# ndming/GS-2M

Measured on AMD Instinct MI355X. Metric: train views/s (fwd+bwd raster) at 1M Gaussians 1080p, higher is better.
Workload: dtype f32; 1 GPU; BASELINE configs[2] (c3): 1000000 synthetic Gaussians (SH deg 3), 1 camera 1920x1080 per GPU, feature_count=9, fwd+bwd at the op boundary; gaussians=1000000, visible=844909, num_rendered=2709460, width=1920, height=1080, feature_count=9, parallelism=view-parallel x1, views_per_rank=1

## Files before the change

gs-2m_amd/csrc/api.hip:

```cpp
#include "common.h"
#include <atomic>
#include <mutex>
#include <chrono>
#include <dlfcn.h>

#define HIP_TRY(expr)                          \
    do {                                       \
        hipError_t e_ = (expr);                \
        if (e_ != hipSuccess) return GS2M_ERR_HIP; \
    } while (0)

namespace {

uint32_t higher_msb(uint32_t n) {
    uint32_t msb = sizeof(n) * 4;
    uint32_t step = msb;
    while (step > 1) {
        step /= 2;
        if (n >> msb) msb += step; else msb -= step;
    }
    if (n >> msb) msb++;
    return msb;
}

constexpr int kLandSlots = 64, kLandWords = 16;
struct LandRing {
    uint32_t* host = nullptr;
    uint32_t* dev = nullptr;
    std::atomic<uint32_t> next{0};
    std::atomic<uint32_t> gen[kLandSlots];
};
LandRing g_land[64];
std::mutex g_land_mutex;
thread_local uint64_t t_last_token = 0;
thread_local long long t_rows_hint = -1;
thread_local long long t_units_hint = -1, t_units_from_token = -1;

static_assert(GS2M_NUM_STAGES == 10, "stage table");
enum Stage { ST_PREPROCESS = 0, ST_UNUSED1, ST_SCAN, ST_EMIT, ST_TILE_SORT, ST_LISTS, ST_BLEND_FWD, ST_UNUSED7,
             ST_BLEND_BWD, ST_GAUSSIAN_BWD, ST_COUNT };
constexpr int kMaxRecords = 8192;
struct Prof {
    std::atomic<int> mode{0};
    int n = 0;
    hipEvent_t ev[kMaxRecords][2];
    int stage[kMaxRecords];
    int created = 0;
    int every = 1;
    int seen3 = 0;
};
Prof g_prof;
std::mutex g_prof_mutex;
std::atomic<int> g_reference_binning{0};
std::atomic<int> g_spin_wait{1};
std::atomic<int> g_debug{0};
std::atomic<int> g_markers{0};

const char* const kStageNames[ST_COUNT] = {"preprocess", "-", "scan", "emit", "tile_sort", "depth_order+quad_lists", "blend_fwd", "-", "blend_bwd", "gaussian_bwd"};

struct Roctx {
    int (*push)(const char*) = nullptr;
    int (*pop)() = nullptr;
    bool tried = false;
    void load() {
        if (tried) return;
        tried = true;
        void* h = dlopen("libroctx64.so", RTLD_NOW | RTLD_GLOBAL);
        if (!h) h = dlopen("libroctx64.so.4", RTLD_NOW | RTLD_GLOBAL);
        if (!h) return;
        push = (int (*)(const char*))dlsym(h, "roctxRangePushA");
        pop = (int (*)())dlsym(h, "roctxRangePop");
    }
};
Roctx g_roctx;

struct StageTimer {
    hipStream_t s;
    int slot = -1;
    int stage;
    int* failed;
    bool marked = false;
    StageTimer(int stage_, hipStream_t s_, int* failed_ = nullptr) : s(s_), stage(stage_), failed(failed_) {
        if (g_markers.load(std::memory_order_relaxed)) {
            g_roctx.load();
            if (g_roctx.push) { g_roctx.push(kStageNames[stage]); marked = true; }
        }
        const bool blend = stage == ST_BLEND_FWD || stage == ST_BLEND_BWD;
        if (g_prof.mode.load(std::memory_order_relaxed) == 0) return;
        {
            std::lock_guard<std::mutex> lock(g_prof_mutex);
            if (g_prof.mode == 0 || (g_prof.mode == 1 && !blend) || (g_prof.mode == 3 && stage != ST_BLEND_BWD) || g_prof.n >= kMaxRecords) return;
            if (g_prof.mode == 3 && (g_prof.seen3++ % g_prof.every) != 0) return;
            slot = g_prof.n++;
            if (slot >= g_prof.created) {
                (void)hipEventCreate(&g_prof.ev[slot][0]);
                (void)hipEventCreate(&g_prof.ev[slot][1]);
                g_prof.created = slot + 1;
            }
            g_prof.stage[slot] = stage;
        }
        (void)hipEventRecord(g_prof.ev[slot][0], s);
    }
    ~StageTimer() {
        if (slot >= 0) (void)hipEventRecord(g_prof.ev[slot][1], s);
        if (failed && g_debug.load(std::memory_order_relaxed) && *failed == 0) {
            hipError_t e = hipGetLastError();
            if (e == hipSuccess) e = hipStreamSynchronize(s);
            if (e != hipSuccess) *failed = stage + 1;
        }
        if (marked && g_roctx.pop) g_roctx.pop();
    }
};
#define DEBUG_CHECK()                                        \
    do {                                                     \
        if (failed_stage) return GS2M_ERR_STAGE(failed_stage - 1); \
    } while (0)

}

extern "C" {

char* gs2m_prealloc_alloc(size_t bytes, void* user) {
    gs2m_prealloc* p = static_cast<gs2m_prealloc*>(user);
    if (!p) return nullptr;
    p->requested = bytes;
    if (p->ptr && bytes <= p->capacity) return p->ptr;
    p->used_fallback = 1;
    return p->fallback ? p->fallback(bytes, p->fallback_user) : nullptr;
}

const char* gs2m_version(void) { return "gs2m_raster 0.5 (gfx950, round 5)"; }

static int forward_impl(gs2m_alloc_fn geometry_alloc, void* geometry_user, gs2m_alloc_fn binning_alloc,
                        void* binning_user, gs2m_alloc_fn image_alloc, void* image_user, int P, int D, int M,
                        const float* background, int width, int height, const float* means3D, const float* shs, const float* shs_rest,
                        const float* colors_precomp, const float* opacities, const float* scales, float scale_modifier,
                        const float* rotations, const float* cov3D_precomp, const float* features,
                        const float* viewmatrix, const float* projmatrix, const float* cam_pos, float tan_fovx,
                        float tan_fovy, int prefiltered, int feature_count, float* out_color, int* out_radii,
                        int* out_observe, float* out_buffer, void* stream_) {
    hipStream_t s = (hipStream_t)stream_;
    const int reference_binning = g_reference_binning.load(), spin_wait = g_spin_wait.load();
    int failed_stage = 0;
    if (P < 0 || width <= 0 || height <= 0 || feature_count < 0 || feature_count > GS2M_NUM_FEATURES) return GS2M_ERR_INVALID_ARG;
    if (!geometry_alloc || !binning_alloc || !image_alloc || !out_color || !out_buffer || !background) return GS2M_ERR_INVALID_ARG;
    if (P > 0 && (!means3D || !opacities || !out_radii || !out_observe || !viewmatrix || !projmatrix)) return GS2M_ERR_INVALID_ARG;
    if (P > 0 && ((shs == nullptr) == (colors_precomp == nullptr))) return GS2M_ERR_INVALID_ARG;
    if (P > 0 && (((scales == nullptr) || (rotations == nullptr)) == (cov3D_precomp == nullptr))) return GS2M_ERR_INVALID_ARG;
    if (P > 0 && shs && (D < 0 || D > 3 || M < (D + 1) * (D + 1) || !cam_pos)) return GS2M_ERR_INVALID_ARG;
    if (shs_rest && (!shs || M != 16 || (((uintptr_t)shs_rest) & 15))) return GS2M_ERR_UNSUPPORTED;
    if (P > 0 && feature_count > 0 && !features) return GS2M_ERR_INVALID_ARG;
    if (width > 16 * 65535 || height > 16 * 65535) return GS2M_ERR_UNSUPPORTED;
    if ((size_t)((width + GS2M_TILE - 1) / GS2M_TILE) * (size_t)((height + GS2M_TILE - 1) / GS2M_TILE) > ((size_t)1 << 28)) return GS2M_ERR_UNSUPPORTED;
    if (P >= (1 << GS2M_GID_BITS)) return GS2M_ERR_UNSUPPORTED;

    const int tiles_x = (width + GS2M_TILE - 1) / GS2M_TILE, tiles_y = (height + GS2M_TILE - 1) / GS2M_TILE;
    const size_t tiles = (size_t)tiles_x * tiles_y, N = (size_t)width * height;
    const float focal_y = height / (2.0f * tan_fovy);
    const float focal_x = width / (2.0f * tan_fovx);

    const size_t Pn = P > 0 ? (size_t)P : 1;
    GeomState gsz = gs2m_carve_geom(nullptr, Pn);
    char* gbase = geometry_alloc(gsz.total_bytes, geometry_user);
    if (!gbase) return GS2M_ERR_ALLOC;
    GeomState g = gs2m_carve_geom(gbase, Pn);

    ImageState isz = gs2m_carve_image(nullptr, N, tiles);
    char* ibase = image_alloc(isz.total_bytes, image_user);
    if (!ibase) return GS2M_ERR_ALLOC;
    ImageState im = gs2m_carve_image(ibase, N, tiles);

    int dev_id = 0;
    HIP_TRY(hipGetDevice(&dev_id));
    if (dev_id < 0 || dev_id >= 64) return GS2M_ERR_UNSUPPORTED;
    LandRing& ring = g_land[dev_id];
    if (!ring.host) {
        std::lock_guard<std::mutex> lock(g_land_mutex);
        if (!ring.host) {
            uint32_t* h = nullptr;
            HIP_TRY(hipHostMalloc((void**)&h, kLandSlots * kLandWords * sizeof(uint32_t), hipHostMallocMapped | hipHostMallocPortable));
            HIP_TRY(hipHostGetDevicePointer((void**)&ring.dev, h, 0));
            for (int k = 0; k < kLandSlots; k++) ring.gen[k] = 0;
            ring.host = h;
        }
    }
    const uint32_t seq = ring.next.fetch_add(1), slot = seq % kLandSlots;
    const uint32_t generation = ring.gen[slot].fetch_add(1) + 1;
    volatile uint32_t* land = ring.host + slot * kLandWords;
    uint32_t* land_dev = ring.dev + slot * kLandWords;
    land[GS2M_LAND_R] = 0xFFFFFFFFu;
    land[GS2M_LAND_HUNITS] = 0xFFFFFFFFu;
    land[GS2M_LAND_PREFILTERED] = 0u;
    land[GS2M_LAND_ROWS] = 0u;
    t_last_token = ((uint64_t)(dev_id + 1) << 40) | ((uint64_t)(generation & 0xFFFFFFFFu) << 8) | slot;

    int R = 0;
    uint32_t U = 0, crowded = GS2M_CROWDED_WAVE;
    if (P > 0) {
        {
            StageTimer t(ST_PREPROCESS, s, &failed_stage);
            ZeroJobs zj = {{g.tile_hist, nullptr, nullptr}, {(size_t)GS2M_HIST_COPIES * GS2M_HIST_COPY_WORDS, 0, 0}};
            gs2m_launch_preprocess(P, D, M, means3D, scales, scale_modifier, rotations, opacities, shs, shs_rest, cov3D_precomp,
                                   colors_precomp, features, viewmatrix, projmatrix, cam_pos, width, height, tan_fovx,
                                   tan_fovy, focal_x, focal_y, tiles_x, tiles_y, out_radii, out_observe, g,
                                   reference_binning ? 0 : 1, zj, s);
        }
        if (prefiltered) gs2m_launch_prefiltered_check(P, means3D, viewmatrix, land_dev + GS2M_LAND_PREFILTERED, s);
        {
            StageTimer t(ST_SCAN, s, &failed_stage);
            gs2m_launch_blockscan(P, g, land_dev, s);
        }
        HIP_TRY(hipGetLastError());
        DEBUG_CHECK();
        if (spin_wait) {
            const auto t0 = std::chrono::steady_clock::now();
            uint32_t spins = 0;
            while (land[GS2M_LAND_R] == 0xFFFFFFFFu || land[GS2M_LAND_HUNITS] == 0xFFFFFFFFu) {
                __builtin_ia32_pause();
                if ((++spins & 0xFFFFu) == 0u && std::chrono::steady_clock::now() - t0 > std::chrono::seconds(2)) break;
            }
        }
        if (land[GS2M_LAND_R] == 0xFFFFFFFFu || land[GS2M_LAND_HUNITS] == 0xFFFFFFFFu) HIP_TRY(hipStreamSynchronize(s));
        if (prefiltered && land[GS2M_LAND_PREFILTERED] != 0u) {
            HIP_TRY(hipStreamSynchronize(s));
            return GS2M_ERR_PREFILTERED;
        }
        if (land[GS2M_LAND_R] >= (1u << 29)) return GS2M_ERR_UNSUPPORTED;
        R = (int)land[GS2M_LAND_R];
        U = land[GS2M_LAND_HUNITS];
        if ((size_t)U * 4 * GS2M_UNIT > (size_t)6 * (size_t)R + 65536) {
            crowded = GS2M_CROWDED_OFF;
            land[GS2M_LAND_R] = 0xFFFFFFFFu;
            land[GS2M_LAND_HUNITS] = 0xFFFFFFFFu;
            gs2m_launch_recount_heavy(P, g, s);
            gs2m_launch_blockscan(P, g, land_dev, s);
            HIP_TRY(hipGetLastError());
            HIP_TRY(hipStreamSynchronize(s));
            if (land[GS2M_LAND_R] != (uint32_t)R) return GS2M_ERR_STAGE(ST_SCAN);
            U = land[GS2M_LAND_HUNITS];
        }
        if (U >= (1u << 22)) return GS2M_ERR_UNSUPPORTED;
    }

    const int tile_bits = (int)higher_msb((uint32_t)tiles);
    const size_t Rn = R > 0 ? (size_t)R : 1;
    const size_t btemp = gs2m_binning_temp_bytes(Rn, tile_bits);
    BinningState bsz = gs2m_carve_binning(nullptr, Rn, btemp, U);
    char* bbase = binning_alloc(bsz.total_bytes, binning_user);
    if (!bbase) return GS2M_ERR_ALLOC;
    BinningState b = gs2m_carve_binning(bbase, Rn, btemp, U);

    if (R > 0) {
        {
            StageTimer t(ST_EMIT, s, &failed_stage);
            ZeroJobs zj = {{nullptr, im.ranges_raw, nullptr}, {0, tiles * 2, 0}};
            gs2m_radix_zero_region(b.temp, (size_t)R, tile_bits, &zj.p[0], &zj.words[0]);
            gs2m_launch_emit(P, width, height, tiles_x, tile_bits, g, b, U, crowded, land_dev, zj, s);
        }
        if (g_debug.load(std::memory_order_relaxed)) {
            uint32_t total = 0;
            HIP_TRY(hipStreamSynchronize(s));
            HIP_TRY(hipMemcpy(&total, g.counters, sizeof(total), hipMemcpyDeviceToHost));
            if (total != (uint32_t)R) return GS2M_ERR_STAGE(ST_EMIT);
        }
        {
            StageTimer t(ST_TILE_SORT, s, &failed_stage);
            HIP_TRY(gs2m_radix_sort_pairs(b.temp, b.temp_bytes, b.keys_unsorted, nullptr, b.sort_keyA, b.sort_valA, b.tile_keys, b.slot_sorted,
                                          (size_t)R, tile_bits, true, s, im.ranges_raw, g.tile_hist));
        }
    } else {
        HIP_TRY(gs2m_zero_async(im.ranges_raw, tiles * 2 * sizeof(uint32_t), s));
        land[GS2M_LAND_ROWS] = 1u;
        if (land[GS2M_LAND_HUNITS] == 0xFFFFFFFFu) land[GS2M_LAND_HUNITS] = 0u;
    }
    DEBUG_CHECK();
    {
        StageTimer t(ST_LISTS, s, &failed_stage);
        gs2m_launch_tile_sort(tiles, tiles_x, tiles_y, (size_t)(R > 0 ? R : 0), b, im, g, s);
    }
    {
        StageTimer t(ST_BLEND_FWD, s, &failed_stage);
        gs2m_launch_blend_fwd_q(width, height, tiles_x, tiles_y, feature_count, background, g, b, im, out_color, out_buffer, out_observe, s);
    }
    DEBUG_CHECK();
    HIP_TRY(hipGetLastError());
    return R;
}

static int backward_impl(int P, int D, int M, int R, const float* background, int width, int height,
                         const float* means3D, const float* shs, const float* shs_rest, const float* colors_precomp, const float* scales,
                         float scale_modifier, const float* rotations, const float* cov3D_precomp,
                         const float* features, const float* viewmatrix, const float* projmatrix, const float* campos,
                         float tan_fovx, float tan_fovy, const int* radii, const float* buffer, char* geom_buffer,
                         char* binning_buffer, char* image_buffer, int feature_count, const float* grad_colors,
                         const float* grad_buffer, float* dL_dmeans2D, float* dL_dconics, float* dL_dopacities,
                         float* dL_dcolors, float* dL_dmeans3D, float* dL_dcov3D, float* dL_dshs, float* dL_dshs_rest, float* dL_dscales,
                         float* dL_drots, float* dL_dfeatures, gs2m_alloc_fn scratch_alloc, void* scratch_user,
                         void* stream_) {
    (void)buffer; (void)features;
    hipStream_t s = (hipStream_t)stream_;
    int failed_stage = 0;
    if (P == 0) return GS2M_OK;
    if (P >= (1 << GS2M_GID_BITS)) return GS2M_ERR_UNSUPPORTED;
    if (P < 0 || R < 0 || width <= 0 || height <= 0 || feature_count < 0 || feature_count > GS2M_NUM_FEATURES) return GS2M_ERR_INVALID_ARG;
    if (!geom_buffer || !binning_buffer || !image_buffer || !scratch_alloc || !grad_colors || !radii) return GS2M_ERR_INVALID_ARG;
    if (feature_count > 0 && !grad_buffer) return GS2M_ERR_INVALID_ARG;
    if (!dL_dmeans2D || !dL_dopacities || !dL_dmeans3D || !dL_dscales || !dL_drots || !dL_dfeatures) return GS2M_ERR_INVALID_ARG;
    if ((colors_precomp && !dL_dcolors) || (cov3D_precomp && !dL_dcov3D)) return GS2M_ERR_INVALID_ARG;
    if (shs_rest && (M != 16 || ((dL_dshs == nullptr) != (dL_dshs_rest == nullptr)) || ((((uintptr_t)shs_rest) | ((uintptr_t)dL_dshs_rest)) & 15))) return GS2M_ERR_UNSUPPORTED;

    const int tiles_x = (width + GS2M_TILE - 1) / GS2M_TILE, tiles_y = (height + GS2M_TILE - 1) / GS2M_TILE;
    const size_t tiles = (size_t)tiles_x * tiles_y, N = (size_t)width * height;
    const size_t Rn = R > 0 ? (size_t)R : 1;
    GeomState g = gs2m_carve_geom(geom_buffer, (size_t)P);
    BinningState b = gs2m_carve_binning(binning_buffer, Rn, gs2m_binning_temp_bytes(Rn, (int)higher_msb((uint32_t)tiles)), 0);
    ImageState im = gs2m_carve_image(image_buffer, N, tiles);

    const int rowf = gs2m_row_floats(feature_count);
    const long long hint = t_rows_hint;
    long long units = hint >= 0 ? t_units_hint : -1;
    t_rows_hint = -1;
    t_units_hint = -1;
    size_t nrows = 0;
    if (hint >= 0 && (size_t)hint <= Rn * 10 + 256) {
        nrows = (size_t)hint;
    } else if (R > 0) {
        uint32_t c[2] = {0u, 0u};
        HIP_TRY(hipStreamSynchronize(s));
        HIP_TRY(hipMemcpy(c, g.counters + GS2M_CNT_ROWS, sizeof(c), hipMemcpyDeviceToHost));
        nrows = c[0];
        units = c[1];
    }
    const size_t rows_bytes = gs2m_align_up((nrows > 0 ? nrows : 1) * (size_t)rowf * sizeof(float));
    char* sbase = scratch_alloc(rows_bytes + 2 * GS2M_ALIGN, scratch_user);
    if (!sbase) return GS2M_ERR_ALLOC;
    float* rows = (float*)gs2m_align_up((size_t)(uintptr_t)sbase);

    if (R > 0) {
        StageTimer t(ST_BLEND_BWD, s, &failed_stage);
        gs2m_launch_blend_bwd_q(width, height, tiles_x, tiles_y, feature_count, background, g, b, im, grad_colors,
                                grad_buffer, rows, s);
    }
    DEBUG_CHECK();
    {
        StageTimer tg(ST_GAUSSIAN_BWD, s, &failed_stage);
        if (R > 0) gs2m_launch_heavy_reduce(rows, rowf, b, g, units, s);
        gs2m_launch_gaussian_bwd(P, D, M, means3D, shs, shs_rest, colors_precomp, scales, scale_modifier, rotations, cov3D_precomp,
                                 viewmatrix, projmatrix, campos, width, height, tan_fovx, tan_fovy, radii, feature_count, g,
                                 rows, rowf, R > 0, dL_dmeans2D, dL_dconics, dL_dopacities, dL_dcolors, dL_dmeans3D,
                                 dL_dcov3D, dL_dshs, dL_dshs_rest, dL_dscales, dL_drots, dL_dfeatures, s);
    }
    DEBUG_CHECK();
    HIP_TRY(hipGetLastError());
    return GS2M_OK;
}

int gs2m_raster_forward(gs2m_alloc_fn geometry_alloc, void* geometry_user, gs2m_alloc_fn binning_alloc,
                        void* binning_user, gs2m_alloc_fn image_alloc, void* image_user, int P, int D, int M,
                        const float* background, int width, int height, const float* means3D, const float* shs,
                        const float* colors_precomp, const float* opacities, const float* scales, float scale_modifier,
                        const float* rotations, const float* cov3D_precomp, const float* features,
                        const float* viewmatrix, const float* projmatrix, const float* cam_pos, float tan_fovx,
                        float tan_fovy, int prefiltered, int feature_count, float* out_color, int* out_radii,
                        int* out_observe, float* out_buffer, void* stream_) {
    return forward_impl(geometry_alloc, geometry_user, binning_alloc, binning_user, image_alloc, image_user, P, D, M, background, width, height, means3D, shs, nullptr, colors_precomp, opacities, scales, scale_modifier, rotations, cov3D_precomp, features, viewmatrix, projmatrix, cam_pos, tan_fovx, tan_fovy, prefiltered, feature_count, out_color, out_radii, out_observe, out_buffer, stream_);
}

int gs2m_raster_forward_split_sh(gs2m_alloc_fn geometry_alloc, void* geometry_user, gs2m_alloc_fn binning_alloc,
                        void* binning_user, gs2m_alloc_fn image_alloc, void* image_user, int P, int D, int M,
                        const float* background, int width, int height, const float* means3D, const float* sh_dc, const float* sh_rest,
                        const float* colors_precomp, const float* opacities, const float* scales, float scale_modifier,
                        const float* rotations, const float* cov3D_precomp, const float* features,
                        const float* viewmatrix, const float* projmatrix, const float* cam_pos, float tan_fovx,
                        float tan_fovy, int prefiltered, int feature_count, float* out_color, int* out_radii,
                        int* out_observe, float* out_buffer, void* stream_) {
    if (!sh_dc || !sh_rest) return GS2M_ERR_INVALID_ARG;
    return forward_impl(geometry_alloc, geometry_user, binning_alloc, binning_user, image_alloc, image_user, P, D, M, background, width, height, means3D, sh_dc, sh_rest, colors_precomp, opacities, scales, scale_modifier, rotations, cov3D_precomp, features, viewmatrix, projmatrix, cam_pos, tan_fovx, tan_fovy, prefiltered, feature_count, out_color, out_radii, out_observe, out_buffer, stream_);
}

int gs2m_raster_backward(int P, int D, int M, int R, const float* background, int width, int height,
                         const float* means3D, const float* shs, const float* colors_precomp, const float* scales,
                         float scale_modifier, const float* rotations, const float* cov3D_precomp,
                         const float* features, const float* viewmatrix, const float* projmatrix, const float* campos,
                         float tan_fovx, float tan_fovy, const int* radii, const float* buffer, char* geom_buffer,
                         char* binning_buffer, char* image_buffer, int feature_count, const float* grad_colors,
                         const float* grad_buffer, float* dL_dmeans2D, float* dL_dconics, float* dL_dopacities,
                         float* dL_dcolors, float* dL_dmeans3D, float* dL_dcov3D, float* dL_dshs, float* dL_dscales,
                         float* dL_drots, float* dL_dfeatures, gs2m_alloc_fn scratch_alloc, void* scratch_user,
                         void* stream_) {
    return backward_impl(P, D, M, R, background, width, height, means3D, shs, nullptr, colors_precomp, scales, scale_modifier, rotations, cov3D_precomp, features, viewmatrix, projmatrix, campos, tan_fovx, tan_fovy, radii, buffer, geom_buffer, binning_buffer, image_buffer, feature_count, grad_colors, grad_buffer, dL_dmeans2D, dL_dconics, dL_dopacities, dL_dcolors, dL_dmeans3D, dL_dcov3D, dL_dshs, nullptr, dL_dscales, dL_drots, dL_dfeatures, scratch_alloc, scratch_user, stream_);
}

int gs2m_raster_backward_split_sh(int P, int D, int M, int R, const float* background, int width, int height,
                         const float* means3D, const float* sh_dc, const float* sh_rest, const float* colors_precomp, const float* scales,
                         float scale_modifier, const float* rotations, const float* cov3D_precomp,
                         const float* features, const float* viewmatrix, const float* projmatrix, const float* campos,
                         float tan_fovx, float tan_fovy, const int* radii, const float* buffer, char* geom_buffer,
                         char* binning_buffer, char* image_buffer, int feature_count, const float* grad_colors,
                         const float* grad_buffer, float* dL_dmeans2D, float* dL_dconics, float* dL_dopacities,
                         float* dL_dcolors, float* dL_dmeans3D, float* dL_dcov3D, float* dL_dsh_dc, float* dL_dsh_rest, float* dL_dscales,
                         float* dL_drots, float* dL_dfeatures, gs2m_alloc_fn scratch_alloc, void* scratch_user,
                         void* stream_) {
    if (!sh_dc || !sh_rest) return GS2M_ERR_INVALID_ARG;
    return backward_impl(P, D, M, R, background, width, height, means3D, sh_dc, sh_rest, colors_precomp, scales, scale_modifier, rotations, cov3D_precomp, features, viewmatrix, projmatrix, campos, tan_fovx, tan_fovy, radii, buffer, geom_buffer, binning_buffer, image_buffer, feature_count, grad_colors, grad_buffer, dL_dmeans2D, dL_dconics, dL_dopacities, dL_dcolors, dL_dmeans3D, dL_dcov3D, dL_dsh_dc, dL_dsh_rest, dL_dscales, dL_drots, dL_dfeatures, scratch_alloc, scratch_user, stream_);
}

int gs2m_raster_mark_visible(int P, const float* means3D, const float* viewmatrix, const float* projmatrix,
                             uint8_t* present, void* stream_) {
    (void)projmatrix;
    if (P < 0) return GS2M_ERR_INVALID_ARG;
    if (P == 0) return GS2M_OK;
    if (!means3D || !viewmatrix || !present) return GS2M_ERR_INVALID_ARG;
    gs2m_launch_mark_visible(P, means3D, viewmatrix, present, (hipStream_t)stream_);
    HIP_TRY(hipGetLastError());
    return GS2M_OK;
}

int gs2m_set_reference_binning(int on) {
    g_reference_binning = on ? 1 : 0;
    return GS2M_OK;
}

int gs2m_set_tile_sort_policy(int policy) {
    if (policy < 0 || policy > 3) return GS2M_ERR_INVALID_ARG;
    gs2m_set_tile_sort_policy_impl(policy);
    return GS2M_OK;
}

int gs2m_set_debug(int on) {
    g_debug = on ? 1 : 0;
    return GS2M_OK;
}

int gs2m_set_markers(int on) {
    g_markers = on ? 1 : 0;
    if (on) {
        g_roctx.load();
        if (!g_roctx.push || !g_roctx.pop) return GS2M_ERR_UNSUPPORTED;
    }
    return GS2M_OK;
}

const char* gs2m_stage_name(int stage) { return stage >= 0 && stage < ST_COUNT ? kStageNames[stage] : "?"; }

int gs2m_set_spin_wait(int on) {
    g_spin_wait = on ? 1 : 0;
    return GS2M_OK;
}

int gs2m_profile_mode(int mode) {
    if (mode < 0 || mode > 3) return GS2M_ERR_INVALID_ARG;
    std::lock_guard<std::mutex> lock(g_prof_mutex);
    g_prof.mode = mode;
    g_prof.n = 0;
    g_prof.seen3 = 0;
    return GS2M_OK;
}

int gs2m_profile_sampling(int every) {
    if (every < 1) return GS2M_ERR_INVALID_ARG;
    std::lock_guard<std::mutex> lock(g_prof_mutex);
    g_prof.every = every;
    return GS2M_OK;
}

int gs2m_profile_collect(float* stage_ms, int* stage_count, int n_stages) {
    if (!stage_ms || !stage_count || n_stages < GS2M_NUM_STAGES) return GS2M_ERR_INVALID_ARG;
    std::lock_guard<std::mutex> lock(g_prof_mutex);
    for (int i = 0; i < n_stages; i++) { stage_ms[i] = 0.f; stage_count[i] = 0; }
    for (int r = 0; r < g_prof.n; r++) {
        float ms = 0.f;
        HIP_TRY(hipEventSynchronize(g_prof.ev[r][1]));
        HIP_TRY(hipEventElapsedTime(&ms, g_prof.ev[r][0], g_prof.ev[r][1]));
        stage_ms[g_prof.stage[r]] += ms;
        stage_count[g_prof.stage[r]] += 1;
    }
    g_prof.n = 0;
    return GS2M_OK;
}

int gs2m_debug_layout(int P, int R, int width, int height, gs2m_layout* out) {
    if (!out || P < 0 || R < 0 || width <= 0 || height <= 0) return GS2M_ERR_INVALID_ARG;
    const int tiles_x = (width + GS2M_TILE - 1) / GS2M_TILE, tiles_y = (height + GS2M_TILE - 1) / GS2M_TILE;
    const size_t tiles = (size_t)tiles_x * tiles_y, N = (size_t)width * height;
    const size_t Pn = P > 0 ? (size_t)P : 1, Rn = R > 0 ? (size_t)R : 1;
    GeomState g = gs2m_carve_geom(nullptr, Pn);
    BinningState b = gs2m_carve_binning(nullptr, Rn, gs2m_binning_temp_bytes(Rn, (int)higher_msb((uint32_t)tiles)), 0);
    ImageState im = gs2m_carve_image(nullptr, N, tiles);
    out->geom_bytes = g.total_bytes;
    out->rec = (uint64_t)(uintptr_t)g.rec;
    out->tiles_touched = (uint64_t)(uintptr_t)g.tiles_touched;
    out->depth_key = (uint64_t)(uintptr_t)g.depth_key;
    out->rect = (uint64_t)(uintptr_t)g.rect;
    out->gauss_rows = (uint64_t)(uintptr_t)g.gauss_rows;
    out->clamped = (uint64_t)(uintptr_t)g.clamped;
    out->wave_rowbase = (uint64_t)(uintptr_t)g.wave_rowbase;
    out->counters = (uint64_t)(uintptr_t)g.counters;
    out->binning_bytes = b.total_bytes;
    out->point_list = (uint64_t)(uintptr_t)b.point_list;
    out->tile_keys = (uint64_t)(uintptr_t)b.tile_keys;
    out->qlist = (uint64_t)(uintptr_t)b.qlist;
    out->qrow = (uint64_t)(uintptr_t)b.qrow;
    out->image_bytes = im.total_bytes;
    out->final_T = (uint64_t)(uintptr_t)im.final_T;
    out->n_contrib = (uint64_t)(uintptr_t)im.n_contrib;
    out->ranges = (uint64_t)(uintptr_t)im.ranges;
    out->qcount = (uint64_t)(uintptr_t)im.qcount;
    return GS2M_OK;
}

unsigned long long gs2m_raster_forward_token(void) { return (unsigned long long)t_last_token; }

long long gs2m_raster_dense_rows(unsigned long long token) {
    if (token == 0ull) return -1;
    const int dev = (int)(token >> 40) - 1;
    const uint32_t slot = (uint32_t)(token & 0xFFull), generation = (uint32_t)((token >> 8) & 0xFFFFFFFFull);
    if (dev < 0 || dev >= 64 || slot >= (uint32_t)kLandSlots || !g_land[dev].host) return -1;
    LandRing& ring = g_land[dev];
    volatile uint32_t* land = ring.host + slot * kLandWords;
    const auto t0 = std::chrono::steady_clock::now();
    uint32_t spins = 0;
    for (;;) {
        if (ring.gen[slot].load() != generation) return -1;
        const uint32_t v = land[GS2M_LAND_ROWS];
        if (v != 0u) {
            t_units_from_token = (long long)land[GS2M_LAND_HUNITS];
            return ring.gen[slot].load() == generation ? (long long)v - 1 : -1;
        }
        __builtin_ia32_pause();
        if ((++spins & 0xFFFFu) == 0u && std::chrono::steady_clock::now() - t0 > std::chrono::seconds(2)) return -1;
    }
}

int gs2m_raster_backward_rows_hint(long long dense_rows) {
    t_rows_hint = dense_rows;
    t_units_hint = dense_rows >= 0 ? t_units_from_token : -1;
    t_units_from_token = -1;
    return GS2M_OK;
}

int gs2m_debug_tile_sort(int tiles, const unsigned* ranges_raw, unsigned* ranges, const unsigned* slot_sorted, const unsigned* e_rec,
                         const unsigned* wave_rowbase, unsigned* point_list, unsigned* row_tmp, unsigned* qlist,
                         unsigned* qrow, unsigned* qcount, void* stream_) {
    if (tiles < 0 || !ranges_raw || !ranges || !slot_sorted || !e_rec || !wave_rowbase || !point_list || !row_tmp || !qlist || !qrow || !qcount) return GS2M_ERR_INVALID_ARG;
    BinningState b = {};
    b.slot_sorted = const_cast<uint32_t*>(slot_sorted); b.e_rec = reinterpret_cast<uint4*>(const_cast<unsigned*>(e_rec));
    b.point_list = point_list; b.sort_valA = row_tmp; b.qlist = reinterpret_cast<uint2*>(qlist); b.qrow = qrow;
    ImageState im = {};
    im.ranges_raw = const_cast<uint32_t*>(ranges_raw);
    im.ranges = reinterpret_cast<uint2*>(ranges);
    im.qcount = qcount;
    GeomState g = {};
    g.wave_rowbase = const_cast<uint32_t*>(wave_rowbase);
    static uint32_t* dbg_counters[64] = {nullptr};
    int dev = 0;
    HIP_TRY(hipGetDevice(&dev));
    if (dev < 0 || dev >= 64) return GS2M_ERR_UNSUPPORTED;
    if (dbg_counters[dev] == nullptr) HIP_TRY(hipMalloc(&dbg_counters[dev], 64 * sizeof(uint32_t)));
    HIP_TRY(hipMemsetAsync(dbg_counters[dev], 0, 64 * sizeof(uint32_t), (hipStream_t)stream_));
    g.counters = dbg_counters[dev];
    gs2m_launch_tile_sort((size_t)tiles, tiles, 1, SIZE_MAX, b, im, g, (hipStream_t)stream_);
    HIP_TRY(hipGetLastError());
    return GS2M_OK;
}

int gs2m_debug_radix_temp_bytes(long long n, int total_bits, unsigned long long* bytes) {
    if (n < 0 || !bytes) return GS2M_ERR_INVALID_ARG;
    *bytes = (unsigned long long)gs2m_radix_temp_bytes((size_t)n, total_bits);
    return GS2M_OK;
}

int gs2m_debug_radix_plan(int total_bits, int* npass, int* bits4, int* shift4) {
    if (!npass || !bits4 || !shift4) return GS2M_ERR_INVALID_ARG;
    gs2m_radix_plan(total_bits, npass, bits4, shift4);
    return GS2M_OK;
}

int gs2m_debug_radix_sort(long long n, int total_bits, const unsigned* kin, const unsigned* vin, unsigned* kA, unsigned* vA, unsigned* kB,
                          unsigned* vB, void* temp, unsigned long long temp_bytes, int prezeroed, unsigned* range_raw, const unsigned* ext_hist,
                          void* stream_) {
    if (n < 0 || (n > 0 && (!kin || !kA || !vA || !kB || !vB || !temp))) return GS2M_ERR_INVALID_ARG;
    const hipError_t e = gs2m_radix_sort_pairs(temp, (size_t)temp_bytes, kin, vin, kA, vA, kB, vB, (size_t)n, total_bits, prezeroed != 0,
                                               (hipStream_t)stream_, range_raw, ext_hist);
    return e == hipErrorInvalidValue ? GS2M_ERR_INVALID_ARG : gs2m_status(e);
}

int gs2m_debug_block_scans(long long n_blocks, const unsigned* block_tt, const unsigned* block_hu, unsigned* block_pref, unsigned* block_hupref,
                           long long n_waves, const unsigned* wave_rows, unsigned* wave_rowbase, unsigned* counters, unsigned* landing_out,
                           void* stream_) {
    if (n_blocks < 1 || n_blocks > 0x7FFFFFFF / 256 || n_waves < 1 || n_waves > 0x7FFFFFFF / 64) return GS2M_ERR_INVALID_ARG;
    if (!block_tt || !block_hu || !block_pref || !block_hupref || !wave_rows || !wave_rowbase || !counters || !landing_out) return GS2M_ERR_INVALID_ARG;
    if ((uintptr_t)landing_out & 7) return GS2M_ERR_INVALID_ARG;
    GeomState g = {};
    g.block_tt = const_cast<uint32_t*>(block_tt); g.block_hu = const_cast<uint32_t*>(block_hu);
    g.block_pref = block_pref; g.block_hupref = block_hupref;
    g.wave_rows = const_cast<uint32_t*>(wave_rows); g.wave_rowbase = wave_rowbase;
    g.counters = counters;
    gs2m_launch_blockscan((int)(n_blocks * 256), g, landing_out, (hipStream_t)stream_);
    gs2m_launch_rowscan((int)(n_waves * 64), g, landing_out, (hipStream_t)stream_);
    HIP_TRY(hipGetLastError());
    return GS2M_OK;
}

int gs2m_debug_blend_forward(int W, int H, int fc, const float* bg, const unsigned* ranges, const unsigned* qlist, const unsigned* qcount,
                             const float* rec, float* out_color, float* out_buffer, float* final_T, unsigned* n_contrib, int* observe,
                             unsigned* qlast, void* stream_) {
    if (W < 1 || H < 1 || fc < 0 || fc > GS2M_NUM_FEATURES) return GS2M_ERR_INVALID_ARG;
    if (!bg || !ranges || !qlist || !qcount || !rec || !out_color || !out_buffer || !final_T || !n_contrib || !observe || !qlast) return GS2M_ERR_INVALID_ARG;
    GeomState g = {};
    g.rec = reinterpret_cast<float4*>(const_cast<float*>(rec));
    BinningState b = {};
    b.qlist = reinterpret_cast<uint2*>(const_cast<unsigned*>(qlist));
    ImageState im = {};
    im.ranges = reinterpret_cast<uint2*>(const_cast<unsigned*>(ranges));
    im.qcount = const_cast<uint32_t*>(qcount);
    im.final_T = final_T; im.n_contrib = n_contrib; im.qlast = qlast;
    gs2m_launch_blend_fwd_q(W, H, (W + GS2M_TILE - 1) / GS2M_TILE, (H + GS2M_TILE - 1) / GS2M_TILE, fc, bg, g, b, im, out_color, out_buffer, observe,
                            (hipStream_t)stream_);
    HIP_TRY(hipGetLastError());
    return GS2M_OK;
}

int gs2m_debug_blend_backward(int W, int H, int fc, const float* bg, const unsigned* ranges, const unsigned* qlist, const unsigned* qcount,
                              const unsigned* qrow, const unsigned* qlast, const float* rec, const float* final_T, const unsigned* n_contrib,
                              const float* grad_color, const float* grad_buffer, float* rows, void* stream_) {
    if (W < 1 || H < 1 || fc < 0 || fc > GS2M_NUM_FEATURES) return GS2M_ERR_INVALID_ARG;
    if (!bg || !ranges || !qlist || !qcount || !qrow || !qlast || !rec || !final_T || !n_contrib || !grad_color || !grad_buffer || !rows) return GS2M_ERR_INVALID_ARG;
    GeomState g = {};
    g.rec = reinterpret_cast<float4*>(const_cast<float*>(rec));
    BinningState b = {};
    b.qlist = reinterpret_cast<uint2*>(const_cast<unsigned*>(qlist));
    b.qrow = const_cast<uint32_t*>(qrow);
    ImageState im = {};
    im.ranges = reinterpret_cast<uint2*>(const_cast<unsigned*>(ranges));
    im.qcount = const_cast<uint32_t*>(qcount);
    im.qlast = const_cast<uint32_t*>(qlast);
    im.final_T = const_cast<float*>(final_T); im.n_contrib = const_cast<uint32_t*>(n_contrib);
    gs2m_launch_blend_bwd_q(W, H, (W + GS2M_TILE - 1) / GS2M_TILE, (H + GS2M_TILE - 1) / GS2M_TILE, fc, bg, g, b, im, grad_color, grad_buffer, rows,
                            (hipStream_t)stream_);
    HIP_TRY(hipGetLastError());
    return GS2M_OK;
}

int gs2m_debug_row_floats(int fc) {
    if (fc < 0 || fc > GS2M_NUM_FEATURES) return GS2M_ERR_INVALID_ARG;
    return gs2m_row_floats(fc);
}

}
```

gs-2m_amd/csrc/binning.hip:

```cpp
#include "common.h"

GeomState gs2m_carve_geom(char* base, size_t P) {
    GeomState g;
    size_t off = base ? (gs2m_align_up((size_t)(uintptr_t)base) - (size_t)(uintptr_t)base) : 0;
    auto take = [&](size_t bytes) {
        char* p = (char*)((uintptr_t)base + off);
        off = gs2m_align_up(off + bytes);
        return p;
    };
    const size_t nb = (P + 255) / 256 + 1, nw = (P + 63) / 64 + 1;
    g.rec = (float4*)take(P * REC_Q * sizeof(float4));
    g.tiles_touched = (uint32_t*)take(P * 4);
    g.rect = (uint2*)take(P * sizeof(uint2));
    g.depth_key = (uint32_t*)take(P * 4);
    g.clamped = (uint8_t*)take(P);
    g.sh_dir = (float*)take(P * 9 * sizeof(float));
    g.counters = (uint32_t*)take(64 * 4);
    g.gauss_rows = (uint32_t*)take(P * 4);
    g.block_tt = (uint32_t*)take(nb * 4);
    g.block_pref = (uint32_t*)take(nb * 4);
    g.block_hu = (uint32_t*)take(nb * 4);
    g.block_hupref = (uint32_t*)take(nb * 4);
    g.wave_rows = (uint32_t*)take(nw * 4);
    g.wave_rowbase = (uint32_t*)take(nw * 4);
    g.tile_hist = (uint32_t*)take(GS2M_HIST_COPIES * GS2M_HIST_COPY_WORDS * 4);
    g.total_bytes = off + GS2M_ALIGN;
    return g;
}

BinningState gs2m_carve_binning(char* base, size_t R, size_t temp_bytes, size_t heavy_units) {
    BinningState b;
    size_t off = base ? (gs2m_align_up((size_t)(uintptr_t)base) - (size_t)(uintptr_t)base) : 0;
    auto take = [&](size_t bytes) {
        char* p = (char*)((uintptr_t)base + off);
        off = gs2m_align_up(off + bytes);
        return p;
    };
    b.keys_unsorted = (uint32_t*)take(R * 4);
    b.e_rec = (uint4*)take(R * sizeof(uint4));
    b.sort_keyA = (uint32_t*)take(R * 4);
    b.sort_valA = (uint32_t*)take(R * 4);
    b.tile_keys = (uint32_t*)take(R * 4);
    b.slot_sorted = (uint32_t*)take(R * 4);
    b.point_list = (uint32_t*)take(R * 4);
    b.qlist = (uint2*)take(R * 4 * sizeof(uint2));
    b.qrow = (uint32_t*)take(R * 4 * 4);
    b.temp = take(temp_bytes);
    b.temp_bytes = temp_bytes;
    b.hrec = (HeavyUnit*)take(heavy_units * sizeof(HeavyUnit));
    b.total_bytes = off + GS2M_ALIGN;
    return b;
}

size_t gs2m_binning_temp_bytes(size_t R, int tile_bits) { return gs2m_align_up(gs2m_radix_temp_bytes(R, tile_bits)) + GS2M_ALIGN; }

ImageState gs2m_carve_image(char* base, size_t N, size_t tiles) {
    ImageState im;
    size_t off = base ? (gs2m_align_up((size_t)(uintptr_t)base) - (size_t)(uintptr_t)base) : 0;
    auto take = [&](size_t bytes) {
        char* p = (char*)((uintptr_t)base + off);
        off = gs2m_align_up(off + bytes);
        return p;
    };
    im.final_T = (float*)take(N * 4);
    im.n_contrib = (uint32_t*)take(N * 4);
    im.ranges = (uint2*)take(tiles * sizeof(uint2));
    im.ranges_raw = (uint32_t*)take(tiles * 2 * sizeof(uint32_t));
    im.qcount = (uint32_t*)take(tiles * 4 * sizeof(uint32_t));
    im.qlast = (uint32_t*)take(tiles * 4 * sizeof(uint32_t));
    im.total_bytes = off + GS2M_ALIGN;
    return im;
}

namespace {

__device__ __forceinline__ void publish(uint32_t* landing, int word, uint32_t v) {
    __hip_atomic_store(landing + word, v, __ATOMIC_RELAXED, __HIP_MEMORY_SCOPE_SYSTEM);
}

__device__ __forceinline__ unsigned long long block_sum_u64(unsigned long long v, unsigned long long* s_part ) {
    const int lane = threadIdx.x & 63, wave = threadIdx.x >> 6, nw = blockDim.x >> 6;
#pragma unroll
    for (int d = 32; d > 0; d >>= 1) v += __shfl_xor(v, d, 64);
    gs2m_sync();
    if (lane == 0) s_part[wave] = v;
    gs2m_sync();
    unsigned long long t = 0;
    for (int w = 0; w < nw; w++) t += s_part[w];
    return t;
}

template <typename F>
__device__ __forceinline__ unsigned long long scan_1024_per_block(const uint32_t* __restrict__ in, size_t n, uint32_t* s_w ,
                                                                  unsigned long long* s_part , F emit) {
    const size_t first = (size_t)blockIdx.x * 1024;
    unsigned long long before = 0;
    for (size_t base = 0; base < first; base += 16 * 1024) {
        uint32_t v[16];
#pragma unroll
        for (int k = 0; k < 16; k++) {
            const size_t i = base + (size_t)k * 1024 + threadIdx.x;
            v[k] = i < first ? in[i] : 0u;
        }
#pragma unroll
        for (int k = 0; k < 16; k++) before += v[k];
    }
    const size_t i = first + threadIdx.x;
    const uint32_t mine = i < n ? in[i] : 0u;
    before = block_sum_u64(before, s_part);
    const int lane = threadIdx.x & 63, wave = threadIdx.x >> 6;
    const uint32_t incl = wave_inclusive_scan_u32(mine, lane);
    if (lane == 63) s_w[wave] = incl;
    gs2m_sync();
    uint32_t run = incl - mine, total = 0;
    for (int w = 0; w < 16; w++) {
        if (w < wave) run += s_w[w];
        total += s_w[w];
    }
    if (i < n) emit(i, (uint32_t)before + run, mine);
    return before + total;
}

template <typename F>
__device__ __forceinline__ void scan2_1024_per_block(const uint32_t* __restrict__ in0, const uint32_t* __restrict__ in1, size_t n, uint32_t* s_w ,
                                                     unsigned long long* s_part , F emit, unsigned long long& total0, unsigned long long& total1) {
    const size_t first = (size_t)blockIdx.x * 1024;
    unsigned long long b0 = 0, b1 = 0;
    for (size_t base = 0; base < first; base += 8 * 1024) {
        uint32_t v[8], w[8];
#pragma unroll
        for (int k = 0; k < 8; k++) {
            const size_t i = base + (size_t)k * 1024 + threadIdx.x;
            v[k] = i < first ? in0[i] : 0u;
            w[k] = i < first ? in1[i] : 0u;
        }
#pragma unroll
        for (int k = 0; k < 8; k++) { b0 += v[k]; b1 += w[k]; }
    }
    const size_t i = first + threadIdx.x;
    const uint32_t m0 = i < n ? in0[i] : 0u, m1 = i < n ? in1[i] : 0u;
    const int lane = threadIdx.x & 63, wave = threadIdx.x >> 6;
#pragma unroll
    for (int d = 32; d > 0; d >>= 1) { b0 += __shfl_xor(b0, d, 64); b1 += __shfl_xor(b1, d, 64); }
    const uint32_t i0 = wave_inclusive_scan_u32(m0, lane), i1 = wave_inclusive_scan_u32(m1, lane);
    if (lane == 0) { s_part[wave] = b0; s_part[16 + wave] = b1; }
    if (lane == 63) { s_w[wave] = i0; s_w[16 + wave] = i1; }
    gs2m_sync();
    unsigned long long f0 = 0, f1 = 0;
    uint32_t r0 = i0 - m0, r1 = i1 - m1, t0 = 0, t1 = 0;
    for (int w = 0; w < 16; w++) {
        f0 += s_part[w]; f1 += s_part[16 + w];
        if (w < wave) { r0 += s_w[w]; r1 += s_w[16 + w]; }
        t0 += s_w[w]; t1 += s_w[16 + w];
    }
    if (i < n) emit(i, (uint32_t)f0 + r0, (uint32_t)f1 + r1);
    total0 = f0 + t0;
    total1 = f1 + t1;
}

__global__ void __launch_bounds__(1024) blockscan_kernel(const uint32_t* __restrict__ block_tt, const uint32_t* __restrict__ block_hu, size_t nblocks,
                                                         uint32_t* __restrict__ block_pref, uint32_t* __restrict__ block_hupref,
                                                         uint32_t* __restrict__ counters, uint32_t* landing) {
    __shared__ uint32_t s_w[32];
    __shared__ unsigned long long s_part[32];
    unsigned long long t = 0, u = 0;
    scan2_1024_per_block(block_tt, block_hu, nblocks, s_w, s_part, [&](size_t b, uint32_t e0, uint32_t e1) { block_pref[b] = e0; block_hupref[b] = e1; }, t, u);
    if (blockIdx.x == gridDim.x - 1 && threadIdx.x == 0) {
        const uint32_t r32 = t > 0xFFFFFFFEull ? 0xFFFFFFFEu : (uint32_t)t, u32 = u > 0xFFFFFFFEull ? 0xFFFFFFFEu : (uint32_t)u;
        __hip_atomic_store(reinterpret_cast<unsigned long long*>(landing + GS2M_LAND_R), (unsigned long long)r32 | ((unsigned long long)u32 << 32),
                           __ATOMIC_RELAXED, __HIP_MEMORY_SCOPE_SYSTEM);
        counters[1] = r32;
        counters[GS2M_CNT_HUNITS] = u32;
        counters[GS2M_CNT_SPAN_MID] = 0u;
        counters[GS2M_CNT_SPAN_LONG] = 0u;
    }
}

__global__ void __launch_bounds__(1024) rowscan_kernel(const uint32_t* __restrict__ wave_rows, size_t nwaves, uint32_t* __restrict__ wave_rowbase,
                                                       uint32_t* __restrict__ counters, uint32_t* landing) {
    __shared__ uint32_t s_w[16];
    __shared__ unsigned long long s_part[16];
    const uint32_t heavy_rows = 4u * GS2M_UNIT * counters[GS2M_CNT_HUNITS];
    const unsigned long long total = heavy_rows + scan_1024_per_block(wave_rows, nwaves, s_w, s_part, [&](size_t w, uint32_t excl, uint32_t) { wave_rowbase[w] = heavy_rows + excl; });
    if (blockIdx.x == gridDim.x - 1 && threadIdx.x == 0) {
        counters[GS2M_CNT_ROWS] = (uint32_t)total;
        publish(landing, GS2M_LAND_ROWS, (uint32_t)total + 1u);
    }
}


__device__ __forceinline__ uint2 expand_instance(uint32_t rmin, uint32_t rwid, uint32_t t, const float4 a , const float2 ct ,
                                                 int W, int H, int tiles_x) {
    const uint32_t ry = t / rwid, rx = t - ry * rwid;
    const uint32_t tx = (rmin & 0xFFFFu) + rx, ty = (rmin >> 16) + ry;
    const int px0 = (int)tx * GS2M_TILE, py0 = (int)ty * GS2M_TILE;
    uint32_t mask = gs2m_reaches_quads(a.x, a.y, a.z, a.w, ct.x, ct.y, (float)px0, (float)py0);
    if (px0 + 8 >= W) mask &= 0x5u;
    if (py0 + 8 >= H) mask &= 0x3u;
    return make_uint2(ty * (uint32_t)tiles_x + tx, mask);
}

__global__ void __launch_bounds__(256) emit_kernel(int P, int W, int H, int tiles_x, const uint2* __restrict__ rect,
                                                   const uint32_t* __restrict__ block_pref, const uint32_t* __restrict__ block_hupref,
                                                   const float4* __restrict__ rec,
                                                   const uint32_t* __restrict__ depth_key, uint32_t* __restrict__ keys_out, uint4* __restrict__ e_rec,
                                                   HeavyUnit* __restrict__ hrec,
                                                   uint32_t* __restrict__ gauss_rows, uint32_t* __restrict__ wave_rows,
                                                   uint32_t* __restrict__ counters, uint32_t* __restrict__ tile_hist, int npass, int4 hbits,
                                                   int4 hshift, uint32_t crowded, ZeroJobs zero) {
    __shared__ uint32_t s_th[4][256];
    __shared__ uint32_t s_pref[4][GS2M_WAVE];
    __shared__ uint32_t s_rmin[4][GS2M_WAVE];
    __shared__ uint32_t s_rw[4][GS2M_WAVE];
    __shared__ uint32_t s_off[4][GS2M_WAVE];
    __shared__ uint32_t s_depth[4][GS2M_WAVE];
    __shared__ float4 s_geo[4][GS2M_WAVE];
    __shared__ float2 s_ct[4][GS2M_WAVE];
    __shared__ uint32_t s_rc[4][GS2M_WAVE];
    __shared__ uint32_t s_wtot[4], s_whu[4];
    const int i = blockIdx.x * 256 + threadIdx.x;
    const int wave = threadIdx.x >> 6, lane = threadIdx.x & 63;
    gs2m_zero_jobs(zero, (size_t)i, (size_t)gridDim.x * 256);
#pragma unroll
    for (int p = 0; p < 4; p++) s_th[p][threadIdx.x] = 0u;
    const int hb[4] = {hbits.x, hbits.y, hbits.z, hbits.w}, hs[4] = {hshift.x, hshift.y, hshift.z, hshift.w};
    uint32_t cnt = 0, rmin = 0, rw = 1;
    if (i < P) {
        const uint2 r = rect[i];
        rmin = r.x;
        rw = r.y & 0xFFFFu;
        cnt = rw * (r.y >> 16);
        if (rw == 0u) rw = 1u;
    }
    const bool heavy = gs2m_heavy(cnt, crowded);
    const uint32_t hu = heavy ? (cnt + GS2M_UNIT - 1u) / GS2M_UNIT : 0u;
    const uint32_t incl_all = wave_inclusive_scan_u32(cnt, lane), incl_hu = wave_inclusive_scan_u32(hu, lane);
    if (lane == 63) { s_wtot[wave] = incl_all; s_whu[wave] = incl_hu; }
    const uint32_t lcnt = heavy ? 0u : cnt;
    if (lcnt > 0) {
        const float4* r = rec + (size_t)i * REC_Q;
        s_geo[wave][lane] = r[REC_GEO0];
        s_ct[wave][lane] = make_float2(r[REC_GEO1].x, r[REC_BIN].w);
        s_depth[wave][lane] = depth_key[i];
    }
    const uint32_t incl = wave_inclusive_scan_u32(lcnt, lane);
    const uint32_t total = __shfl(incl, 63, 64);
    s_pref[wave][lane] = incl - lcnt;
    s_rmin[wave][lane] = rmin;
    s_rw[wave][lane] = rw;
    s_rc[wave][lane] = 0u;
    gs2m_sync();
    uint32_t off = block_pref[blockIdx.x], ustart = block_hupref[blockIdx.x];
#pragma unroll
    for (int w = 0; w < 4; w++)
        if (w < wave) { off += s_wtot[w]; ustart += s_whu[w]; }
    off += incl_all - cnt;
    ustart += incl_hu - hu;
    s_off[wave][lane] = off;
    if (blockIdx.x == gridDim.x - 1 && threadIdx.x == 255) counters[0] = off + cnt;
    if (heavy) {
        gauss_rows[i] = GS2M_ROWS_BIG | ustart;
        for (uint32_t j = 0; j < hu; j++) {
            hrec[ustart + j].gid = (uint32_t)i;
            hrec[ustart + j].off = off;
        }
    }
    const uint32_t gid0 = (uint32_t)blockIdx.x * 256u;
    uint32_t rows_run = 0;
    for (uint32_t k = 0; k < total; k += GS2M_WAVE) {
        const uint32_t j = k + lane;
        uint32_t pc = 0, slot = 0, mask = 0;
        int lo = 0;
        if (j < total) {
#pragma unroll
            for (int step = 32; step > 0; step >>= 1)
                if (s_pref[wave][lo + step] <= j) lo += step;
            const uint32_t t = j - s_pref[wave][lo];
            slot = s_off[wave][lo] + t;
            const uint2 km = expand_instance(s_rmin[wave][lo], s_rw[wave][lo], t, s_geo[wave][lo], s_ct[wave][lo], W, H, tiles_x);
            mask = km.y;
            keys_out[slot] = km.x;
            for (int p = 0; p < npass; p++) atomicAdd(&s_th[p][(km.x >> hs[p]) & ((1u << hb[p]) - 1u)], 1u);
            pc = (uint32_t)__popc(mask);
            if (pc) atomicAdd(&s_rc[wave][lo], pc);
        }
        const uint32_t pin = wave_inclusive_scan_u32(pc, lane);
        if (j < total) e_rec[slot] = make_uint4((gid0 + (uint32_t)(wave * GS2M_WAVE + lo)) | (mask << GS2M_GID_BITS), rows_run + pin - pc, s_depth[wave][lo], 0u);
        rows_run += __shfl(pin, 63, 64);
    }
    if (i < P && !heavy) gauss_rows[i] = s_rc[wave][lane];
    const size_t wave_id = (size_t)blockIdx.x * 4 + wave;
    if (lane == 0 && (size_t)wave_id * GS2M_WAVE < (size_t)P) wave_rows[wave_id] = rows_run;
    gs2m_sync();
    uint32_t* dst = tile_hist + (blockIdx.x & (GS2M_HIST_COPIES - 1)) * GS2M_HIST_COPY_WORDS;
    for (int p = 0; p < npass; p++) {
        const uint32_t c = s_th[p][threadIdx.x];
        if (c) atomicAdd(&dst[p * 256 + threadIdx.x], c);
    }
}

__global__ void __launch_bounds__(256) recount_heavy_kernel(int P, const uint2* __restrict__ rect, uint32_t* __restrict__ block_hu) {
    __shared__ uint32_t s_hu[4];
    const int i = blockIdx.x * 256 + threadIdx.x;
    uint32_t cnt = 0;
    if (i < P) {
        const uint2 r = rect[i];
        cnt = (r.y & 0xFFFFu) * (r.y >> 16);
    }
    uint32_t hu = gs2m_heavy(cnt, GS2M_CROWDED_OFF) ? (cnt + GS2M_UNIT - 1u) / GS2M_UNIT : 0u;
#pragma unroll
    for (int d = 32; d > 0; d >>= 1) hu += (uint32_t)__shfl_xor((int)hu, d, 64);
    if ((threadIdx.x & 63) == 0) s_hu[threadIdx.x >> 6] = hu;
    gs2m_sync();
    if (threadIdx.x == 0) block_hu[blockIdx.x] = s_hu[0] + s_hu[1] + s_hu[2] + s_hu[3];
}

__global__ void __launch_bounds__(256) emit_heavy_kernel(uint32_t units, int W, int H, int tiles_x, const uint2* __restrict__ rect, const float4* __restrict__ rec,
                                                         const uint32_t* __restrict__ depth_key, const uint32_t* __restrict__ gauss_rows,
                                                         uint32_t* __restrict__ keys_out, uint4* __restrict__ e_rec, HeavyUnit* __restrict__ hrec,
                                                         uint32_t* __restrict__ tile_hist, int npass, int4 hbits, int4 hshift) {
    __shared__ uint32_t s_th[4][256];
#pragma unroll
    for (int p = 0; p < 4; p++) s_th[p][threadIdx.x] = 0u;
    gs2m_sync();
    const int hb[4] = {hbits.x, hbits.y, hbits.z, hbits.w}, hs[4] = {hshift.x, hshift.y, hshift.z, hshift.w};
    const int wave = threadIdx.x >> 6, lane = threadIdx.x & 63;
    const uint32_t u = blockIdx.x * 4u + (uint32_t)wave;
    if (u < units) {
        const uint32_t gid = hrec[u].gid, off = hrec[u].off;
        const uint32_t ustart = gauss_rows[gid] & ~GS2M_ROWS_BIG;
        const uint2 r = rect[gid];
        const uint32_t rw = r.y & 0xFFFFu, cnt = rw * (r.y >> 16);
        const float4* rq = rec + (size_t)gid * REC_Q;
        const float4 geo = rq[REC_GEO0];
        const float2 ct = make_float2(rq[REC_GEO1].x, rq[REC_BIN].w);
        const uint32_t dk = depth_key[gid];
        const uint32_t t = (u - ustart) * GS2M_UNIT + (uint32_t)lane;
        uint32_t pc = 0;
        if (t < cnt) {
            const uint2 km = expand_instance(r.x, rw, t, geo, ct, W, H, tiles_x);
            keys_out[off + t] = km.x;
            for (int p = 0; p < npass; p++) atomicAdd(&s_th[p][(km.x >> hs[p]) & ((1u << hb[p]) - 1u)], 1u);
            e_rec[off + t] = make_uint4(gid | (km.y << GS2M_GID_BITS), GS2M_ROWS_BIG | (4u * (u * GS2M_UNIT + (uint32_t)lane)), dk, 0u);
            pc = (uint32_t)__popc(km.y);
        }
        hrec[u].pop[lane] = (uint8_t)pc;
    }
    gs2m_sync();
    uint32_t* dst = tile_hist + (blockIdx.x & (GS2M_HIST_COPIES - 1)) * GS2M_HIST_COPY_WORDS;
    for (int p = 0; p < npass; p++) {
        const uint32_t c = s_th[p][threadIdx.x];
        if (c) atomicAdd(&dst[p * 256 + threadIdx.x], c);
    }
}

}

void gs2m_launch_blockscan(int P, const GeomState& g, uint32_t* landing, hipStream_t s) {
    const size_t nb = (size_t)(P + 255) / 256;
    blockscan_kernel<<<(unsigned)((nb + 1023) / 1024 > 0 ? (nb + 1023) / 1024 : 1), 1024, 0, s>>>(g.block_tt, g.block_hu, nb, g.block_pref, g.block_hupref, g.counters,
                                                                                                  landing);
}

void gs2m_launch_recount_heavy(int P, const GeomState& g, hipStream_t s) {
    recount_heavy_kernel<<<(P + 255) / 256, 256, 0, s>>>(P, g.rect, g.block_hu);
}

void gs2m_launch_emit(int P, int W, int H, int tiles_x, int tile_bits, const GeomState& g, const BinningState& b, uint32_t heavy_units, uint32_t crowded,
                      uint32_t* landing, const ZeroJobs& zero, hipStream_t s) {
    int npass = 0, bits[4], shift[4];
    gs2m_radix_plan(tile_bits, &npass, bits, shift);
    const int4 hbits = make_int4(bits[0], bits[1], bits[2], bits[3]), hshift = make_int4(shift[0], shift[1], shift[2], shift[3]);
    emit_kernel<<<(P + 255) / 256, 256, 0, s>>>(P, W, H, tiles_x, g.rect, g.block_pref, g.block_hupref, g.rec, g.depth_key, b.keys_unsorted, b.e_rec, b.hrec,
                                                g.gauss_rows, g.wave_rows, g.counters, g.tile_hist, npass, hbits, hshift, crowded, zero);
    if (heavy_units > 0u)
        emit_heavy_kernel<<<(heavy_units + 3u) / 4u, 256, 0, s>>>(heavy_units, W, H, tiles_x, g.rect, g.rec, g.depth_key, g.gauss_rows, b.keys_unsorted, b.e_rec,
                                                                  b.hrec, g.tile_hist, npass, hbits, hshift);
    gs2m_launch_rowscan(P, g, landing, s);
}

void gs2m_launch_rowscan(int P, const GeomState& g, uint32_t* landing, hipStream_t s) {
    const size_t nw = (size_t)(P + 63) / 64;
    rowscan_kernel<<<(unsigned)((nw + 1023) / 1024 > 0 ? (nw + 1023) / 1024 : 1), 1024, 0, s>>>(g.wave_rows, nw, g.wave_rowbase, g.counters, landing);
}

__global__ void zero_kernel(uint32_t* __restrict__ p, size_t words) {
    const size_t i = (size_t)blockIdx.x * blockDim.x + threadIdx.x;
    const size_t head = (4 - (((uintptr_t)p >> 2) & 3)) & 3;
    const size_t quads = words > head ? (words - head) >> 2 : 0;
    if (i < quads) reinterpret_cast<uint4*>(p + head)[i] = make_uint4(0u, 0u, 0u, 0u);
    if (i < head && i < words) p[i] = 0u;
    const size_t tail = head + 4 * quads;
    if (i < words - min(words, tail)) p[tail + i] = 0u;
}
hipError_t gs2m_zero_async(void* p, size_t bytes, hipStream_t s) {
    if (bytes == 0) return hipSuccess;
    if ((bytes & 3) || ((uintptr_t)p & 3)) return hipMemsetAsync(p, 0, bytes, s);
    const size_t words = bytes >> 2, threads = (words >> 2) + 4;
    zero_kernel<<<(unsigned)((threads + 255) / 256), 256, 0, s>>>((uint32_t*)p, words);
    return hipGetLastError();
}
```

gs-2m_amd/csrc/common.h:

```cpp
#pragma once
#include <hip/hip_runtime.h>
#include <stdint.h>
#include <stddef.h>
#include "../../include/gs2m_raster.h"

typedef float gs2m_v4f __attribute__((ext_vector_type(4)));
template <typename T> __device__ __forceinline__ T gs2m_ldnt(const T* p) { return __builtin_nontemporal_load(p); }
__device__ __forceinline__ float4 gs2m_ldnt(const float4* p) {
    const gs2m_v4f t = __builtin_nontemporal_load(reinterpret_cast<const gs2m_v4f*>(p));
    return make_float4(t.x, t.y, t.z, t.w);
}
template <typename T> __device__ __forceinline__ void gs2m_stnt(T* p, T v) { __builtin_nontemporal_store(v, p); }
__device__ __forceinline__ void gs2m_stnt(float4* p, float4 v) {
    const gs2m_v4f t = {v.x, v.y, v.z, v.w};
    __builtin_nontemporal_store(t, reinterpret_cast<gs2m_v4f*>(p));
}

#define GS2M_ALIGN 256
#define GS2M_WAVE 64

#define REC_Q 8
#define REC_GEO0 0
#define REC_GEO1 1
#define REC_BIN 2
#define REC_CH 3
#define REC_AUX 7
#define GS2M_GID_BITS 28
#define GS2M_GID_MASK 0x0FFFFFFFu
#define GS2M_HEAVY_TILES 40u
#define GS2M_HEAVY_TILES_CROWDED 8u
#define GS2M_CROWDED_WAVE 320u
#define GS2M_ROWS_BIG 0x80000000u
#define GS2M_UNIT 64u
struct HeavyUnit {
    uint32_t gid;
    uint32_t off;
    uint32_t pad[2];
    uint8_t pop[GS2M_UNIT];
};

#define ROW_GEOM 8
#define ROW_COL 8
#define ROW_FEAT 11

static inline size_t gs2m_align_up(size_t x, size_t a = GS2M_ALIGN) { return (x + a - 1) & ~(a - 1); }
static inline int gs2m_status(hipError_t e) { return e == hipSuccess ? GS2M_OK : GS2M_ERR_HIP; }

struct GeomState {
    float4* rec;
    uint32_t* tiles_touched;
    uint2* rect;
    uint32_t* depth_key;
    uint8_t* clamped;
    float* sh_dir;
    uint32_t* counters;
    uint32_t* gauss_rows;
    uint32_t* block_tt;
    uint32_t* block_pref;
    uint32_t* block_hu;
    uint32_t* block_hupref;
    uint32_t* wave_rows;
    uint32_t* wave_rowbase;
    uint32_t* tile_hist;
    size_t total_bytes;
};
struct BinningState {
    uint32_t* keys_unsorted;
    uint4* e_rec;
    uint32_t* sort_keyA;
    uint32_t* sort_valA;
    uint32_t* tile_keys;
    uint32_t* slot_sorted;
    uint32_t* point_list;
    uint2* qlist;
    uint32_t* qrow;
    char* temp;
    size_t temp_bytes;
    HeavyUnit* hrec;
    size_t total_bytes;
};
struct ImageState {
    float* final_T;
    uint32_t* n_contrib;
    uint2* ranges;
    uint32_t* ranges_raw;
    uint32_t* qcount;
    uint32_t* qlast;
    size_t total_bytes;
};

struct ZeroJobs {
    uint32_t* p[3];
    size_t words[3];
};
#ifdef __HIPCC__
__device__ __forceinline__ void gs2m_zero_jobs(const ZeroJobs& z, size_t thread, size_t threads) {
#pragma unroll
    for (int k = 0; k < 3; k++)
        for (size_t i = thread; i < z.words[k]; i += threads) z.p[k][i] = 0u;
}
#endif

#ifdef __HIPCC__
__device__ __forceinline__ void gs2m_stage_sh(const float* __restrict__ shs, const float* __restrict__ rest, int P,
                                              float* __restrict__ s_sh) {
    const int tid = threadIdx.x;
    if (rest == nullptr) {
        const size_t base4 = (size_t)blockIdx.x * 256 * 12, lim4 = (size_t)P * 12;
        const float4* g4 = reinterpret_cast<const float4*>(shs);
        float4 t[12];
#pragma unroll
        for (int i = 0; i < 12; i++) {
            const size_t k = base4 + tid + 256 * i;
            t[i] = k < lim4 ? gs2m_ldnt(g4 + k) : make_float4(0.f, 0.f, 0.f, 0.f);
        }
#pragma unroll
        for (int i = 0; i < 12; i++) {
            const int e = 4 * (tid + 256 * i);
            const int row = e / 48, col = e - row * 48;
            float* d = s_sh + row * 49 + col;
            d[0] = t[i].x; d[1] = t[i].y; d[2] = t[i].z; d[3] = t[i].w;
        }
    } else {
        const size_t dbase = (size_t)blockIdx.x * 768, dlim = (size_t)P * 3;
#pragma unroll
        for (int i = 0; i < 3; i++) {
            const int e = tid + 256 * i;
            const float v = dbase + e < dlim ? shs[dbase + e] : 0.f;
            s_sh[(e / 3) * 49 + (e % 3)] = v;
        }
        const size_t rbase = (size_t)blockIdx.x * 11520, rlim = (size_t)P * 45;
        const bool full = rbase + 11520 <= rlim;
        float4 t[12];
        if (full) {
            const float4* g4 = reinterpret_cast<const float4*>(rest + rbase);
#pragma unroll
            for (int i = 0; i < 11; i++) t[i] = gs2m_ldnt(g4 + tid + 256 * i);
            t[11] = tid < 64 ? gs2m_ldnt(g4 + tid + 2816) : make_float4(0.f, 0.f, 0.f, 0.f);
        } else {
#pragma unroll
            for (int i = 0; i < 12; i++) {
                const int k4 = tid + 256 * i;
                const size_t ge = rbase + 4 * (size_t)k4;
                t[i] = make_float4(0.f, 0.f, 0.f, 0.f);
                if (k4 < 2880) {
                    if (ge + 3 < rlim) {
                        t[i] = *reinterpret_cast<const float4*>(rest + ge);
                    } else {
                        if (ge < rlim) t[i].x = rest[ge];
                        if (ge + 1 < rlim) t[i].y = rest[ge + 1];
                        if (ge + 2 < rlim) t[i].z = rest[ge + 2];
                    }
                }
            }
        }
        int row = (4 * tid) / 45, col = 4 * tid - 45 * row;
#pragma unroll
        for (int i = 0; i < 12; i++) {
            if (i < 11 || tid < 64) {
                const float v[4] = {t[i].x, t[i].y, t[i].z, t[i].w};
                int a = row * 49 + 3 + col, left = 45 - col;
#pragma unroll
                for (int c = 0; c < 4; c++) s_sh[a + c + (c >= left ? 4 : 0)] = v[c];
            }
            row += 22; col += 34;
            if (col >= 45) { col -= 45; row += 1; }
        }
    }
}
#endif

GeomState gs2m_carve_geom(char* base, size_t P);
BinningState gs2m_carve_binning(char* base, size_t R, size_t temp_bytes, size_t heavy_units);
size_t gs2m_binning_temp_bytes(size_t R, int tile_bits);
ImageState gs2m_carve_image(char* base, size_t N, size_t tiles);

size_t gs2m_radix_temp_bytes(size_t n, int total_bits);
hipError_t gs2m_radix_sort_pairs(void* temp, size_t temp_bytes, const uint32_t* kin, const uint32_t* vin, uint32_t* kA,
                                 uint32_t* vA, uint32_t* kB, uint32_t* vB, size_t n, int total_bits, bool prezeroed, hipStream_t s,
                                 uint32_t* range_raw = nullptr, const uint32_t* ext_hist = nullptr);
#define GS2M_HIST_COPIES 8
#define GS2M_HIST_COPY_WORDS 1024
void gs2m_radix_plan(int total_bits, int* npass, int bits[4], int shift[4]);
void gs2m_radix_zero_region(void* temp, size_t n, int total_bits, uint32_t** ptr, size_t* words);

#define GS2M_LAND_R 0
#define GS2M_LAND_HUNITS 1
#define GS2M_LAND_PREFILTERED 2
#define GS2M_LAND_ROWS 3
#define GS2M_CNT_ROWS 2
#define GS2M_CNT_HUNITS 3
#define GS2M_CNT_SPAN_MID 4
#define GS2M_CNT_SPAN_LONG 5

void gs2m_launch_preprocess(int P, int D, int M, const float* means3D, const float* scales, float scale_modifier,
                            const float* rotations, const float* opacities, const float* shs, const float* shs_rest,
                            const float* cov3D_precomp, const float* colors_precomp, const float* features,
                            const float* viewmatrix, const float* projmatrix, const float* cam_pos, int W, int H,
                            float tan_fovx, float tan_fovy, float focal_x, float focal_y, int tiles_x, int tiles_y,
                            int* radii, int* observe_zero, const GeomState& g, int shrink, const ZeroJobs& zero, hipStream_t s);
void gs2m_launch_blockscan(int P, const GeomState& g, uint32_t* landing, hipStream_t s);
void gs2m_launch_rowscan(int P, const GeomState& g, uint32_t* landing, hipStream_t s);
void gs2m_launch_emit(int P, int W, int H, int tiles_x, int tile_bits, const GeomState& g, const BinningState& b, uint32_t heavy_units,
                      uint32_t crowded, uint32_t* landing, const ZeroJobs& zero, hipStream_t s);
void gs2m_launch_recount_heavy(int P, const GeomState& g, hipStream_t s);
void gs2m_launch_heavy_reduce(float* rows, int rowf, const BinningState& b, const GeomState& g, long long heavy_units, hipStream_t s);
void gs2m_set_tile_sort_policy_impl(int policy);
void gs2m_launch_tile_sort(size_t tiles, int tiles_x, int tiles_y, size_t R, const BinningState& b, const ImageState& im, const GeomState& g, hipStream_t s);
hipError_t gs2m_zero_async(void* p, size_t bytes, hipStream_t s);

void gs2m_launch_blend_fwd_q(int W, int H, int tiles_x, int tiles_y, int fc, const float* bg, const GeomState& g,
                             const BinningState& b, const ImageState& im, float* out_color, float* out_buffer,
                             int* out_observe, hipStream_t s);
void gs2m_launch_blend_bwd_q(int W, int H, int tiles_x, int tiles_y, int fc, const float* bg, const GeomState& g,
                             const BinningState& b, const ImageState& im, const float* grad_color,
                             const float* grad_buffer, float* rows, hipStream_t s);
int gs2m_row_floats(int fc);
void gs2m_launch_gaussian_bwd(int P, int D, int M, const float* means3D, const float* shs, const float* shs_rest,
                              const float* colors_precomp,
                              const float* scales, float scale_modifier, const float* rotations,
                              const float* cov3D_precomp, const float* viewmatrix, const float* projmatrix,
                              const float* campos, int W, int H, float tan_fovx, float tan_fovy, const int* radii,
                              int fc, const GeomState& g, const float* rows, int rowf, bool have_rows,
                              float* dL_dmeans2D, float* dL_dconics, float* dL_dopacities, float* dL_dcolors,
                              float* dL_dmeans3D, float* dL_dcov3D, float* dL_dshs, float* dL_dshs_rest, float* dL_dscales,
                              float* dL_drots, float* dL_dfeatures, hipStream_t s);
void gs2m_launch_prefiltered_check(int P, const float* means3D, const float* viewmatrix, uint32_t* flag, hipStream_t s);
void gs2m_launch_mark_visible(int P, const float* means3D, const float* viewmatrix, uint8_t* present, hipStream_t s);

#ifdef __HIPCC__
__device__ __forceinline__ float u2f(uint32_t u) { return __uint_as_float(u); }
__device__ __forceinline__ uint32_t f2u(float f) { return __float_as_uint(f); }

#define DPP_QUAD_PERM(a, b, c, d) ((a) | ((b) << 2) | ((c) << 4) | ((d) << 6))
#define DPP_ROW_HALF_MIRROR 0x141
#define DPP_ROW_MIRROR 0x140

__device__ __forceinline__ void gs2m_sync() {
    asm volatile("s_waitcnt lgkmcnt(0)" ::: "memory");
    __syncthreads();
}
__device__ __forceinline__ int gs2m_sync_or(bool pred) {
    asm volatile("s_waitcnt lgkmcnt(0)" ::: "memory");
    return __syncthreads_or(pred);
}

#define GS2M_CROWDED_OFF 0xFFFFFFFFu
__device__ __forceinline__ bool gs2m_heavy(uint32_t cnt, uint32_t crowded) {
    uint32_t light = cnt < GS2M_HEAVY_TILES ? cnt : 0u;
#pragma unroll
    for (int d = 32; d > 0; d >>= 1) light += (uint32_t)__shfl_xor((int)light, d, 64);
    return cnt >= (light > crowded ? GS2M_HEAVY_TILES_CROWDED : GS2M_HEAVY_TILES) && cnt < (1u << 29);
}

template <typename T>
__device__ __forceinline__ T gs2m_wave_inclusive_scan(T v, int lane) {
#pragma unroll
    for (int d = 1; d < 64; d <<= 1) {
        const T t = __shfl_up(v, d, 64);
        if (lane >= d) v += t;
    }
    return v;
}
__device__ __forceinline__ uint32_t wave_inclusive_scan_u32(uint32_t v, int lane) { return gs2m_wave_inclusive_scan(v, lane); }

template <typename T>
__device__ __forceinline__ T gs2m_wg_exclusive_scan(T v, T* s_w, T* total) {
    const int lane = threadIdx.x & 63, w = threadIdx.x >> 6;
    const T inc = gs2m_wave_inclusive_scan(v, lane);
    if (lane == 63) s_w[w] = inc;
    __syncthreads();
    T off = 0, tot = 0;
#pragma unroll
    for (int k = 0; k < 4; k++) {
        const T x = s_w[k];
        off += k < w ? x : T(0);
        tot += x;
    }
    __syncthreads();
    *total = tot;
    return off + inc - v;
}

#define GS2M_LOG2E 1.4426950408889634f
__device__ __forceinline__ float gs2m_power(float dx, float dy, float A, float B, float C) {
    const float t1 = (A * dx) * dx;
    const float t2 = (C * dy) * dy;
    const float t3 = (B * dx) * dy;
    return (-0.5f * (t1 + t2)) - t3;
}
__device__ __forceinline__ uint32_t gs2m_reaches_quads(float gx, float gy, float A, float B, float C, float t2, float x0, float y0) {
    const float b2 = B + B;
    const float nhrC = -0.5f * __builtin_amdgcn_rcpf(C), nhrA = -0.5f * __builtin_amdgcn_rcpf(A);
    float xl[4], yl[4], blx[4], bly[4], basex[4], basey[4], mx[4], my[4];
#pragma unroll
    for (int i = 0; i < 4; i++) {
        const float o = (float)((i >> 1) * 8 + (i & 1) * 7);
        xl[i] = (x0 + o) - gx; yl[i] = (y0 + o) - gy;
        blx[i] = b2 * xl[i]; bly[i] = b2 * yl[i];
        basex[i] = (A * xl[i]) * xl[i]; basey[i] = (C * yl[i]) * yl[i];
        mx[i] = blx[i] * nhrC;
        my[i] = bly[i] * nhrA;
    }
    uint32_t mask = 0;
#pragma unroll
    for (int q = 0; q < 4; q++) {
        const int qx = q & 1, qy = q >> 1;
        const float lx = xl[2 * qx], ux = xl[2 * qx + 1], ly = yl[2 * qy], uy = yl[2 * qy + 1];
        const bool inside = lx <= 0.f && ux >= 0.f && ly <= 0.f && uy >= 0.f;
        float qe[2];
#pragma unroll
        for (int e = 0; e < 2; e++) {
            const int i = 2 * qx + e;
            const float fm = __builtin_amdgcn_fmed3f(mx[i], ly, uy);
            qe[e] = __builtin_fmaf(__builtin_fmaf(C, fm, blx[i]), fm, basex[i]);
        }
        const float qv = fminf(qe[0], qe[1]);
#pragma unroll
        for (int e = 0; e < 2; e++) {
            const int k = 2 * qy + e;
            const float fm = __builtin_amdgcn_fmed3f(my[k], lx, ux);
            qe[e] = __builtin_fmaf(__builtin_fmaf(A, fm, bly[k]), fm, basey[k]);
        }
        const float qmin = fminf(qv, fminf(qe[0], qe[1]));
        const bool hit = !(t2 < 3.0e38f) || inside || qmin <= __builtin_fmaf(1.0e-3f, fabsf(qmin), t2);
        mask |= hit ? (1u << q) : 0u;
    }
    return mask;
}

__device__ __forceinline__ float gs2m_exp(float x) { return __builtin_amdgcn_exp2f(x * GS2M_LOG2E); }
#endif
```

gs-2m_amd/csrc/radix_sort.hip:

```cpp
#include "common.h"
#include <stdlib.h>
#include <atomic>

static std::atomic<int> g_sort_tickets{0};
extern "C" int gs2m_set_sort_tickets(int on) {
    g_sort_tickets = on ? 1 : 0;
    return GS2M_OK;
}

namespace {
constexpr int RS_LB2_WIN = 16;
constexpr int RS_THREADS = 256;
constexpr int RS_ITEMS = 16;
constexpr int RS_TILE = RS_THREADS * RS_ITEMS;
constexpr int RS_MAXPASS = 4;
int resident_tiles() {
    static int cached[64] = {0};
    int dev = 0;
    if (hipGetDevice(&dev) != hipSuccess || dev < 0 || dev >= 64) return 0;
    if (cached[dev] == 0) {
        int cus = 0;
        cached[dev] = hipDeviceGetAttribute(&cus, hipDeviceAttributeMultiprocessorCount, dev) == hipSuccess && cus > 0 ? 4 * cus : -1;
    }
    return cached[dev] > 0 ? cached[dev] : 0;
}
constexpr uint32_t FLAG_AGG = 1u << 30, FLAG_PFX = 2u << 30, VAL_MASK = (1u << 30) - 1;

struct SortPlan {
    int npass;
    int bits[RS_MAXPASS];
    int shift[RS_MAXPASS];
};

SortPlan make_plan(int total_bits) {
    SortPlan p;
    if (total_bits < 1) total_bits = 1;
    p.npass = total_bits <= 16 ? 2 : 4;
    const int per = (total_bits + p.npass - 1) / p.npass;
    int s = 0;
    for (int i = 0; i < p.npass; i++) {
        int b = total_bits - s;
        if (b > per) b = per;
        if (b < 0) b = 0;
        p.bits[i] = b;
        p.shift[i] = s;
        s += b;
    }
    return p;
}

constexpr int RS_HIST_WGS = 512;
constexpr int RS_HIST_REP = 16;
__global__ void __launch_bounds__(RS_THREADS) rs_hist_kernel(const uint32_t* __restrict__ keys, uint32_t n, int npass,
                                                             int4 bits, int4 shift, uint32_t* __restrict__ ghist, int tiles,
                                                             int workers) {
    __shared__ uint32_t s_h[RS_MAXPASS][256][RS_HIST_REP];
    const int tid = threadIdx.x, lane = tid & 63;
    for (int i = tid; i < RS_MAXPASS * 256 * RS_HIST_REP; i += RS_THREADS) (&s_h[0][0][0])[i] = 0;
    gs2m_sync();
    const int b[4] = {bits.x, bits.y, bits.z, bits.w}, sh[4] = {shift.x, shift.y, shift.z, shift.w};
    const int rep = lane & (RS_HIST_REP - 1);
    for (int tile = blockIdx.x; tile < tiles; tile += workers) {
        const uint32_t base = (uint32_t)tile * RS_TILE;
        uint32_t key[RS_ITEMS];
#pragma unroll
        for (int k = 0; k < RS_ITEMS; k++) {
            const uint32_t i = base + k * RS_THREADS + tid;
            key[k] = i < n ? keys[i] : 0u;
        }
#pragma unroll
        for (int k = 0; k < RS_ITEMS; k++) {
            const uint32_t i = base + k * RS_THREADS + tid;
            if (i < n)
                for (int p = 0; p < npass; p++) atomicAdd(&s_h[p][(key[k] >> sh[p]) & ((1u << b[p]) - 1u)][rep], 1u);
        }
    }
    gs2m_sync();
    for (int p = 0; p < npass; p++) {
        const uint4* r4 = reinterpret_cast<const uint4*>(&s_h[p][tid][0]);
        uint32_t c = 0;
#pragma unroll
        for (int q = 0; q < RS_HIST_REP / 4; q++) {
            const uint4 v = r4[q];
            c += v.x + v.y + v.z + v.w;
        }
        if (c) atomicAdd(&ghist[p * 256 + tid], c);
    }
}

template <int BITS>
__global__ void __launch_bounds__(RS_THREADS) rs_onesweep_kernel(
    const uint32_t* __restrict__ keys_in, const uint32_t* __restrict__ vals_in, uint32_t* __restrict__ keys_out,
    uint32_t* __restrict__ vals_out, uint32_t n, int shift, const uint32_t* __restrict__ ghist, uint32_t* ticket,
    uint32_t* status , uint32_t* range_raw, int hist_copies ) {
    constexpr int BINS = 1 << BITS;
    __shared__ uint32_t s_cnt[4][BINS];
    __shared__ uint32_t s_gbase[256];
    __shared__ uint32_t s_w[2][4];
    __shared__ uint32_t s_tile;
    __shared__ uint32_t s_key[RS_TILE], s_val[RS_TILE];
    const int tid = threadIdx.x, wave = tid >> 6, lane = tid & 63;
    if (tid == 0) s_tile = ticket != nullptr ? atomicAdd(ticket, 1u) : blockIdx.x;
    for (int i = tid; i < 4 * BINS; i += RS_THREADS) (&s_cnt[0][0])[i] = 0;
    gs2m_sync();
    const uint32_t tile = s_tile;
    const uint32_t tile_base = tile * RS_TILE;
    const uint32_t tile_count = min((uint32_t)RS_TILE, n - tile_base);
    const uint32_t segbase = tile_base + wave * (64 * RS_ITEMS);

    uint32_t key[RS_ITEMS], val[RS_ITEMS], rank[RS_ITEMS];
#pragma unroll
    for (int k = 0; k < RS_ITEMS; k++) {
        const uint32_t i = segbase + k * 64 + lane;
        key[k] = i < n ? keys_in[i] : 0xFFFFFFFFu;
        val[k] = i < n ? (vals_in ? vals_in[i] : i) : 0u;
    }
    const unsigned long long lt = (1ull << lane) - 1ull;
    [[maybe_unused]] uint32_t run0 = 0;
#pragma unroll
    for (int k = 0; k < RS_ITEMS; k++) {
        const bool valid = segbase + k * 64 + lane < n;
        const uint32_t d = (key[k] >> shift) & (BINS - 1);
        unsigned long long peers = __builtin_amdgcn_ballot_w64(valid);
#pragma unroll
        for (int b = 0; b < BITS; b++) {
            const bool bit = (d >> b) & 1u;
            const unsigned long long bal = __builtin_amdgcn_ballot_w64(bit);
            peers &= bit ? bal : ~bal;
        }
        const unsigned long long below = peers & lt;
        if constexpr (BITS == 0) {
            rank[k] = run0 + (uint32_t)__popcll(below);
            run0 += (uint32_t)__popcll(peers);
        } else {
            const uint32_t old = s_cnt[wave][d];
            rank[k] = old + (uint32_t)__popcll(below);
            if (valid && below == 0ull) s_cnt[wave][d] = old + (uint32_t)__popcll(peers);
        }
    }
    if (BITS == 0 && lane == 0) s_cnt[wave][0] = run0;
    gs2m_sync();

    uint32_t tot = 0, c0 = 0, c1 = 0, c2 = 0, gh = 0;
    if (tid < BINS) {
        c0 = s_cnt[0][tid]; c1 = s_cnt[1][tid]; c2 = s_cnt[2][tid];
        tot = c0 + c1 + c2 + s_cnt[3][tid];
        for (int c = 0; c < hist_copies; c++) gh += ghist[c * GS2M_HIST_COPY_WORDS + tid];
    }
    const uint32_t inclA = wave_inclusive_scan_u32(tot, lane), inclB = wave_inclusive_scan_u32(gh, lane);
    if (lane == 63) {
        s_w[0][wave] = inclA;
        s_w[1][wave] = inclB;
    }
    gs2m_sync();
    uint32_t tile_excl = inclA - tot, digit_base = inclB - gh;
#pragma unroll
    for (int w = 0; w < 4; w++)
        if (w < wave) {
            tile_excl += s_w[0][w];
            digit_base += s_w[1][w];
        }
    if (tid < BINS) {
        __hip_atomic_store(status + (size_t)tile * 256 + tid, FLAG_AGG | tot, __ATOMIC_RELAXED, __HIP_MEMORY_SCOPE_AGENT);
        s_cnt[0][tid] = tile_excl;
        s_cnt[1][tid] = tile_excl + c0;
        s_cnt[2][tid] = tile_excl + c0 + c1;
        s_cnt[3][tid] = tile_excl + c0 + c1 + c2;
    }
    gs2m_sync();
#pragma unroll
    for (int k = 0; k < RS_ITEMS; k++) {
        if (segbase + k * 64 + lane < n) {
            const uint32_t d = (key[k] >> shift) & (BINS - 1);
            const uint32_t lp = s_cnt[wave][d] + rank[k];
            s_key[lp] = key[k];
            s_val[lp] = val[k];
        }
    }
    if (tid < BINS) {
        const uint32_t grp = tile >> 5, r = tile & 31u;
        uint32_t* const lvl2 = status + (size_t)gridDim.x * 256;
        const bool leader = r == 31u;
        uint32_t insum = 0;
#pragma unroll
        for (int h = 0; h < 2; h++) {
            uint32_t w[16];
#pragma unroll
            for (int k = 0; k < 16; k++) {
                const uint32_t back = (uint32_t)(16 * h + k) + 1u;
                w[k] = back <= r ? __hip_atomic_load(status + (size_t)(tile - back) * 256 + tid, __ATOMIC_RELAXED, __HIP_MEMORY_SCOPE_AGENT) : FLAG_AGG;
            }
#pragma unroll
            for (int k = 0; k < 16; k++) {
                const uint32_t back = (uint32_t)(16 * h + k) + 1u;
                while ((w[k] & ~VAL_MASK) == 0u) {
                    __builtin_amdgcn_s_sleep(1);
                    w[k] = __hip_atomic_load(status + (size_t)(tile - back) * 256 + tid, __ATOMIC_RELAXED, __HIP_MEMORY_SCOPE_AGENT);
                }
                insum += w[k] & VAL_MASK;
            }
        }
        uint32_t* const my2 = lvl2 + (size_t)grp * 256 + tid;
        const uint32_t gagg = insum + tot;
        if (leader) __hip_atomic_store(my2, (grp == 0 ? FLAG_PFX : FLAG_AGG) | gagg, __ATOMIC_RELAXED, __HIP_MEMORY_SCOPE_AGENT);
        uint32_t excl2 = 0;
        {
            int p = (int)grp - 1;
            bool found = p < 0;
            while (!found) {
                uint32_t w[RS_LB2_WIN];
#pragma unroll
                for (int k = 0; k < RS_LB2_WIN; k++)
                    w[k] = p - k >= 0 ? __hip_atomic_load(lvl2 + (size_t)(p - k) * 256 + tid, __ATOMIC_RELAXED, __HIP_MEMORY_SCOPE_AGENT)
                                      : FLAG_PFX;
                bool stalled = false;
#pragma unroll
                for (int k = 0; k < RS_LB2_WIN; k++) {
                    const uint32_t f = w[k] & ~VAL_MASK;
                    if (!found && !stalled) {
                        if (f == 0u) {
                            stalled = true;
                        } else {
                            excl2 += w[k] & VAL_MASK;
                            p--;
                            found = f == FLAG_PFX;
                        }
                    }
                }
                if (stalled) __builtin_amdgcn_s_sleep(1);
            }
        }
        if (leader && grp > 0) __hip_atomic_store(my2, FLAG_PFX | (excl2 + gagg), __ATOMIC_RELAXED, __HIP_MEMORY_SCOPE_AGENT);
        const uint32_t excl = excl2 + insum;
        s_gbase[tid] = digit_base + excl - tile_excl;
    }
    gs2m_sync();
#pragma unroll
    for (int k = 0; k < RS_ITEMS; k++) {
        const uint32_t i = k * RS_THREADS + tid;
        if (i < tile_count) {
            const uint32_t kk = s_key[i];
            const uint32_t pos = s_gbase[(kk >> shift) & (BINS - 1)] + i;
            keys_out[pos] = kk;
            vals_out[pos] = s_val[i];
            if (range_raw != nullptr) {
                if (i == 0 || s_key[i - 1] != kk) atomicMax(&range_raw[2 * kk], ~pos);
                if (i + 1 == tile_count || s_key[i + 1] != kk) atomicMax(&range_raw[2 * kk + 1], pos + 1u);
            }
        }
    }
}

template <int BITS>
void launch_pass(const uint32_t* ki, const uint32_t* vi, uint32_t* ko, uint32_t* vo, uint32_t n, int shift,
                 const uint32_t* ghist, uint32_t* ticket, uint32_t* status, int tiles, hipStream_t s, uint32_t* range_raw, int hist_copies) {
    static const bool env_tickets = getenv("GS2M_SORT_TICKETS") && atoi(getenv("GS2M_SORT_TICKETS")) != 0;
    const bool force_tickets = env_tickets || g_sort_tickets.load(std::memory_order_relaxed) != 0;
    rs_onesweep_kernel<BITS><<<tiles, RS_THREADS, 0, s>>>(ki, vi, ko, vo, n, shift, ghist,
                                                          (!force_tickets && tiles <= resident_tiles()) ? nullptr : ticket, status, range_raw, hist_copies);
}

}

void gs2m_radix_plan(int total_bits, int* npass, int bits[4], int shift[4]) {
    const SortPlan p = make_plan(total_bits);
    *npass = p.npass;
    for (int i = 0; i < RS_MAXPASS; i++) { bits[i] = i < p.npass ? p.bits[i] : 0; shift[i] = i < p.npass ? p.shift[i] : 0; }
}

static size_t status_rows(size_t tiles) { return tiles + (tiles + 31) / 32; }
size_t gs2m_radix_temp_bytes(size_t n, int total_bits) {
    const SortPlan p = make_plan(total_bits);
    const size_t tiles = (n + RS_TILE - 1) / RS_TILE;
    return gs2m_align_up(RS_MAXPASS * 256 * 4) + GS2M_ALIGN + (size_t)p.npass * status_rows(tiles) * 256 * 4 + 2 * GS2M_ALIGN;
}

void gs2m_radix_zero_region(void* temp, size_t n, int total_bits, uint32_t** ptr, size_t* words) {
    const SortPlan p = make_plan(total_bits);
    const size_t tiles = (n + RS_TILE - 1) / RS_TILE;
    *ptr = (uint32_t*)gs2m_align_up((size_t)(uintptr_t)temp);
    *words = (gs2m_align_up(RS_MAXPASS * 256 * 4) + GS2M_ALIGN + (size_t)p.npass * status_rows(tiles) * 256 * 4) / 4;
}

hipError_t gs2m_radix_sort_pairs(void* temp, size_t temp_bytes, const uint32_t* kin, const uint32_t* vin, uint32_t* kA,
                                 uint32_t* vA, uint32_t* kB, uint32_t* vB, size_t n, int total_bits, bool prezeroed, hipStream_t s,
                                 uint32_t* range_raw, const uint32_t* ext_hist) {
    if (n == 0) return hipSuccess;
    if (n > (size_t)VAL_MASK) return hipErrorInvalidValue;
    const SortPlan p = make_plan(total_bits);
    const int tiles = (int)((n + RS_TILE - 1) / RS_TILE);
    if (temp_bytes < gs2m_radix_temp_bytes(n, total_bits)) return hipErrorInvalidValue;
    char* base = (char*)gs2m_align_up((size_t)(uintptr_t)temp);
    uint32_t* ghist = (uint32_t*)base;
    uint32_t* tickets = (uint32_t*)(base + gs2m_align_up(RS_MAXPASS * 256 * 4));
    uint32_t* status = (uint32_t*)(base + gs2m_align_up(RS_MAXPASS * 256 * 4) + GS2M_ALIGN);
    const size_t zero_bytes = gs2m_align_up(RS_MAXPASS * 256 * 4) + GS2M_ALIGN + (size_t)p.npass * status_rows((size_t)tiles) * 256 * 4;
    hipError_t e = prezeroed ? hipSuccess : gs2m_zero_async(base, zero_bytes, s);
    if (e != hipSuccess) return e;
    const int workers = tiles < RS_HIST_WGS ? tiles : RS_HIST_WGS;
    if (ext_hist == nullptr)
        rs_hist_kernel<<<workers, RS_THREADS, 0, s>>>(kin, (uint32_t)n, p.npass, make_int4(p.bits[0], p.bits[1], p.bits[2], p.bits[3]),
                                                      make_int4(p.shift[0], p.shift[1], p.shift[2], p.shift[3]), ghist, tiles, workers);
    const uint32_t *ki = kin, *vi = vin;
    for (int i = 0; i < p.npass; i++) {
        uint32_t* ko = (i & 1) ? kB : kA;
        uint32_t* vo = (i & 1) ? vB : vA;
        uint32_t* st = status + (size_t)i * status_rows((size_t)tiles) * 256;
        const uint32_t* gh = (ext_hist ? ext_hist : ghist) + i * 256;
        const int hc = ext_hist ? GS2M_HIST_COPIES : 1;
        uint32_t* const rr = i == p.npass - 1 ? range_raw : nullptr;
        switch (p.bits[i]) {
#define RS_CASE(B) case B: launch_pass<B>(ki, vi, ko, vo, (uint32_t)n, p.shift[i], gh, tickets + i, st, tiles, s, rr, hc); break;
            RS_CASE(0) RS_CASE(1) RS_CASE(2) RS_CASE(3) RS_CASE(4) RS_CASE(5) RS_CASE(6) RS_CASE(7) RS_CASE(8)
#undef RS_CASE
            default: return hipErrorInvalidValue;
        }
        ki = ko;
        vi = vo;
    }
    return hipGetLastError();
}
```

gs-2m_amd/csrc/tile_sort.hip:

```cpp
#include "common.h"
#include <atomic>
#include <cstdlib>
#include <type_traits>

namespace {

template <int CTRL, int ROW_MASK = 0xF, int BANK_MASK = 0xF>
__device__ __forceinline__ uint32_t dpp_u32(uint32_t old, uint32_t v) {
    return (uint32_t)__builtin_amdgcn_update_dpp((int)old, (int)v, CTRL, ROW_MASK, BANK_MASK, false);
}
template <int CTRL>
__device__ __forceinline__ uint32_t dpp_perm(uint32_t v) {
    return (uint32_t)__builtin_amdgcn_update_dpp(0, (int)v, CTRL, 0xF, 0xF, true);
}
template <int B>
__device__ __forceinline__ uint32_t lane_xor(uint32_t v, int lane) {
    if constexpr (B == 0) return dpp_perm<DPP_QUAD_PERM(1, 0, 3, 2)>(v);
    else if constexpr (B == 1) return dpp_perm<DPP_QUAD_PERM(2, 3, 0, 1)>(v);
    else if constexpr (B == 2) {
        const uint32_t t = dpp_u32<0x104 , 0xF, 0x5>(v, v);
        return dpp_u32<0x114 , 0xF, 0xA>(t, v);
    } else if constexpr (B == 3) return dpp_perm<0x128 >(v);
    else return (uint32_t)__builtin_amdgcn_ds_bpermute((lane ^ (1 << B)) << 2, (int)v);
}
template <int T>
__device__ __forceinline__ uint32_t lane_flip(uint32_t v, int lane) {
    if constexpr (T == 1) return dpp_perm<DPP_QUAD_PERM(1, 0, 3, 2)>(v);
    else if constexpr (T == 2) return dpp_perm<DPP_QUAD_PERM(3, 2, 1, 0)>(v);
    else if constexpr (T == 3) return dpp_perm<DPP_ROW_HALF_MIRROR>(v);
    else if constexpr (T == 4) return dpp_perm<DPP_ROW_MIRROR>(v);
    else return (uint32_t)__builtin_amdgcn_ds_bpermute((lane ^ ((1 << T) - 1)) << 2, (int)v);
}

template <int I, int N, typename F>
__device__ __forceinline__ void static_for(F&& f) {
    if constexpr (I < N) {
        f(std::integral_constant<int, I>{});
        static_for<I + 1, N>(f);
    }
}
template <int E, int a, int b>
__device__ __forceinline__ void ce(uint32_t (&k)[E], uint32_t (&x)[E]) {
    const bool sw = k[b] < k[a];
    const uint32_t mn = min(k[a], k[b]), mx = max(k[a], k[b]);
    const uint32_t xa = sw ? x[b] : x[a], xb = sw ? x[a] : x[b];
    k[a] = mn; k[b] = mx; x[a] = xa; x[b] = xb;
}
template <int E, int KB>
__device__ __forceinline__ void inlane_flip(uint32_t (&k)[E], uint32_t (&x)[E]) {
    static_for<0, E>([&](auto ec) {
        constexpr int e = decltype(ec)::value;
        if constexpr (((e >> (KB - 1)) & 1) == 0) ce<E, e, (e ^ ((1 << KB) - 1))>(k, x);
    });
}
template <int E, int JB>
__device__ __forceinline__ void inlane_xor(uint32_t (&k)[E], uint32_t (&x)[E]) {
    static_for<0, E>([&](auto ec) {
        constexpr int e = decltype(ec)::value;
        if constexpr (((e >> JB) & 1) == 0) ce<E, e, (e | (1 << JB))>(k, x);
    });
}
template <int E, int T>
__device__ __forceinline__ void cross_flip(uint32_t (&k)[E], uint32_t (&x)[E], int lane) {
    const bool lower = ((lane >> (T - 1)) & 1) == 0;
    uint32_t nk[E], nx[E];
#pragma unroll
    for (int e = 0; e < E; e++) {
        const uint32_t ok = lane_flip<T>(k[E - 1 - e], lane), ox = lane_flip<T>(x[E - 1 - e], lane);
        const uint32_t mn = min(k[e], ok), mx = max(k[e], ok);
        nk[e] = lower ? mn : mx;
        nx[e] = nk[e] == k[e] ? x[e] : ox;
    }
#pragma unroll
    for (int e = 0; e < E; e++) { k[e] = nk[e]; x[e] = nx[e]; }
}
template <int E, int B>
__device__ __forceinline__ void cross_xor(uint32_t (&k)[E], uint32_t (&x)[E], int lane) {
    const bool lower = ((lane >> B) & 1) == 0;
#pragma unroll
    for (int e = 0; e < E; e++) {
        const uint32_t ok = lane_xor<B>(k[e], lane), ox = lane_xor<B>(x[e], lane);
        const uint32_t mn = min(k[e], ok), mx = max(k[e], ok);
        const uint32_t nk = lower ? mn : mx;
        x[e] = nk == k[e] ? x[e] : ox;
        k[e] = nk;
    }
}
template <int E, int LE, int JB>
__device__ __forceinline__ void xor_steps(uint32_t (&k)[E], uint32_t (&x)[E], int lane) {
    if constexpr (JB >= 0) {
        if constexpr (JB >= LE) cross_xor<E, JB - LE>(k, x, lane);
        else inlane_xor<E, JB>(k, x);
        xor_steps<E, LE, JB - 1>(k, x, lane);
    }
}
template <int E, int LE, int KB>
__device__ __forceinline__ void levels(uint32_t (&k)[E], uint32_t (&x)[E], int lane, uint32_t n) {
    if constexpr (KB <= LE + 6) {
        if (n > (1u << (KB - 1))) {
            if constexpr (KB <= LE) inlane_flip<E, KB>(k, x);
            else cross_flip<E, KB - LE>(k, x, lane);
            xor_steps<E, LE, KB - 2>(k, x, lane);
        }
        levels<E, LE, KB + 1>(k, x, lane, n);
    }
}

__device__ __forceinline__ int skew(int p) { return p + (p >> 5); }

template <int E>
__device__ __forceinline__ void tie_positions(const uint32_t (&key)[E], const uint32_t (&idx)[E], uint32_t (&pos)[E], const int t, const uint32_t n,
                                              const uint32_t* s_k, const uint32_t* s_i) {
#pragma unroll
    for (int e = 0; e < E; e++) {
        const uint32_t i = (uint32_t)(t * E + e);
        pos[e] = i;
        if (i >= n) continue;
        const uint32_t K = key[e], X = idx[e];
        uint32_t a = i, cnt = 0;
        for (uint32_t j = i; j > 0u;) {
            j--;
            if (s_k[skew((int)j)] != K) break;
            a = j;
            cnt += s_i[skew((int)j)] < X ? 1u : 0u;
        }
        for (uint32_t j = i + 1u; j < n; j++) {
            if (s_k[skew((int)j)] != K) break;
            cnt += s_i[skew((int)j)] < X ? 1u : 0u;
        }
        pos[e] = a + cnt;
    }
}

template <int E, int LE>
__device__ __forceinline__ void sort_tile_wave(const int tile, const uint32_t start, const uint32_t n, const uint32_t* __restrict__ slot_sorted,
                                               const uint4* __restrict__ e_rec, const uint32_t* __restrict__ wave_rowbase,
                                               uint32_t* __restrict__ point_list, uint2* __restrict__ qlist, uint32_t* __restrict__ qrow,
                                               uint32_t* __restrict__ qcount, uint32_t* s_v, uint32_t* s_r, const int lane) {
    uint32_t key[E], idx[E], rb[E];
    static_for<0, E / 8>([&](auto bc) {
        constexpr int e0 = 8 * decltype(bc)::value;
        uint32_t slot[8];
#pragma unroll
        for (int e = 0; e < 8; e++) {
            const uint32_t p = (uint32_t)((e0 + e) * GS2M_WAVE + lane);
            slot[e] = p < n ? slot_sorted[start + p] : 0u;
        }
        uint4 rc[8];
#pragma unroll
        for (int e = 0; e < 8; e++) rc[e] = (uint32_t)((e0 + e) * GS2M_WAVE + lane) < n ? e_rec[slot[e]] : make_uint4(0u, 0u, 0xFFFFFFFFu, 0u);
        static_for<0, 8>([&](auto ec) {
            constexpr int e = decltype(ec)::value;
            const uint32_t p = (uint32_t)((e0 + e) * GS2M_WAVE + lane);
            key[e0 + e] = rc[e].z;
            idx[e0 + e] = p;
            s_v[skew((int)p)] = rc[e].x;
            s_r[skew((int)p)] = rc[e].y & ~GS2M_ROWS_BIG;
            rb[e0 + e] = p < n && (rc[e].y & GS2M_ROWS_BIG) == 0u ? wave_rowbase[(rc[e].x & GS2M_GID_MASK) >> 6] : 0u;
        });
        asm volatile("" ::: "memory");
    });
    levels<E, LE, 1>(key, idx, lane, 0xFFFFFFFFu);
#pragma unroll
    for (int e = 0; e < E; e++) s_r[skew(e * GS2M_WAVE + lane)] += rb[e];
    asm volatile("s_waitcnt lgkmcnt(0)" ::: "memory");
    uint32_t sv[E], sr[E];
    auto pick_up = [&]() {
#pragma unroll
        for (int e = 0; e < E; e++) {
            const bool real = (uint32_t)(lane * E + e) < n;
            sv[e] = real ? s_v[skew((int)idx[e])] : 0u;
            sr[e] = real ? s_r[skew((int)idx[e])] : 0u;
        }
        asm volatile("s_waitcnt lgkmcnt(0)" ::: "memory");
    };
    auto park = [&]() {
#pragma unroll
        for (int e = 0; e < E; e++) {
            s_v[skew(lane * E + e)] = sv[e];
            s_r[skew(lane * E + e)] = sr[e];
        }
    };
    pick_up();
    bool tie = false;
#pragma unroll
    for (int e = 0; e + 1 < E; e++) tie |= (uint32_t)(lane * E + e + 1) < n && key[e] == key[e + 1];
    {
        const uint32_t nxt = (uint32_t)__shfl_down((int)key[0], 1, 64);
        tie |= lane < 63 && (uint32_t)(lane * E + E) < n && key[E - 1] == nxt;
    }
    if (__builtin_amdgcn_ballot_w64(tie) != 0ull) {
#pragma unroll
        for (int e = 0; e < E; e++) {
            s_v[skew(lane * E + e)] = key[e];
            s_r[skew(lane * E + e)] = idx[e];
        }
        asm volatile("s_waitcnt lgkmcnt(0)" ::: "memory");
        uint32_t pos[E];
        tie_positions<E>(key, idx, pos, lane, n, s_v, s_r);
        asm volatile("s_waitcnt lgkmcnt(0)" ::: "memory");
#pragma unroll
        for (int e = 0; e < E; e++) {
            s_v[skew((int)pos[e])] = sv[e];
            s_r[skew((int)pos[e])] = sr[e];
        }
    } else {
        park();
    }
    asm volatile("s_waitcnt lgkmcnt(0)" ::: "memory");
    uint2* out = qlist + (size_t)4 * start;
    uint32_t* orow = qrow + (size_t)4 * start;
    uint32_t run[4] = {0u, 0u, 0u, 0u};
    const unsigned long long lt = lane == 0 ? 0ull : (~0ull >> (64 - lane));
    for (uint32_t base = 0; base < n; base += GS2M_WAVE) {
        const uint32_t k = base + (uint32_t)lane;
        uint32_t v = 0, r = 0;
        if (k < n) {
            v = s_v[skew((int)k)];
            r = s_r[skew((int)k)];
            point_list[start + k] = v;
        }
        const uint32_t mask = v >> GS2M_GID_BITS;
#pragma unroll
        for (int q = 0; q < 4; q++) {
            const bool hit = ((mask >> q) & 1u) != 0u;
            const unsigned long long m = __builtin_amdgcn_ballot_w64(hit);
            if (hit) {
                const size_t o = (size_t)q * n + run[q] + (uint32_t)__popcll(m & lt);
                out[o] = make_uint2(v, k);
                orow[o] = r + (uint32_t)__popc(mask & ((1u << q) - 1u));
            }
            run[q] += (uint32_t)__popcll(m);
        }
    }
    if (lane < 4) qcount[tile * 4 + lane] = lane == 0 ? run[0] : (lane == 1 ? run[1] : (lane == 2 ? run[2] : run[3]));
    asm volatile("s_waitcnt lgkmcnt(0)" ::: "memory");
}

#ifndef GS2M_TS_SUPER_LOG
#define GS2M_TS_SUPER_LOG 2
#endif
__device__ __forceinline__ int tile_of_block(int b, int tiles_x, int tiles_y) {
    constexpr int L = GS2M_TS_SUPER_LOG, SIDE = 1 << L, PER = SIDE * SIDE;
    const int xcd = b & 7, j = b >> 3, sub = j & (PER - 1);
    const int stx = (tiles_x + SIDE - 1) >> L, nsuper = stx * ((tiles_y + SIDE - 1) >> L);
    const int S = (j >> (2 * L)) * 8 + xcd;
    if (S >= nsuper) return -1;
    const int tx = SIDE * (S % stx) + (sub & (SIDE - 1)), ty = SIDE * (S / stx) + (sub >> L);
    if (tx >= tiles_x || ty >= tiles_y) return -1;
    return ty * tiles_x + tx;
}
__host__ __device__ inline unsigned tile_grid(int tiles_x, int tiles_y) {
    constexpr int L = GS2M_TS_SUPER_LOG, SIDE = 1 << L;
    const size_t nsuper = (size_t)((tiles_x + SIDE - 1) >> L) * ((tiles_y + SIDE - 1) >> L);
    return (unsigned)(((nsuper + 7) / 8) * 8 * SIDE * SIDE);
}

__device__ __forceinline__ uint2 tile_range(const uint32_t* __restrict__ ranges_raw, uint2* __restrict__ ranges, int tile, int lane) {
    const uint2 raw = reinterpret_cast<const uint2*>(ranges_raw)[tile];
    const uint2 range = raw.y != 0u ? make_uint2(~raw.x, raw.y) : make_uint2(0u, 0u);
    if (lane == 0) ranges[tile] = range;
    return range;
}

__global__ void __launch_bounds__(64) tile_sort_wave_kernel(const uint32_t* __restrict__ ranges_raw, uint2* __restrict__ ranges,
                                                            const uint32_t* __restrict__ slot_sorted, const uint4* __restrict__ e_rec,
                                                            const uint32_t* __restrict__ wave_rowbase,
                                                            uint32_t* __restrict__ point_list, uint2* __restrict__ qlist,
                                                            uint32_t* __restrict__ qrow, uint32_t* __restrict__ qcount, int tiles_x, int tiles_y,
                                                            uint32_t wave_max , uint32_t* __restrict__ counters) {
    constexpr int M = 64 * 8;
    __shared__ uint32_t s_v[M + M / 32], s_r[M + M / 32];
    const int lane = threadIdx.x;
    const int tile = tile_of_block(blockIdx.x, tiles_x, tiles_y);
    if (tile < 0) return;
    const uint2 range = tile_range(ranges_raw, ranges, tile, lane);
    const uint32_t n = range.y - range.x;
    if (n == 0u) {
        if (lane < 4) qcount[tile * 4 + lane] = 0u;
    } else if (n <= wave_max) {
        sort_tile_wave<8, 3>(tile, range.x, n, slot_sorted, e_rec, wave_rowbase, point_list, qlist, qrow, qcount, s_v, s_r, lane);
    } else if (lane == 0) {
        counters[n <= 1024u ? GS2M_CNT_SPAN_MID : GS2M_CNT_SPAN_LONG] = 1u;
    }
}

__global__ void __launch_bounds__(64) __attribute__((amdgpu_waves_per_eu(4, 8)))
tile_sort_wave16_kernel(const uint32_t* __restrict__ ranges_raw, const uint32_t* __restrict__ slot_sorted, const uint4* __restrict__ e_rec,
                        const uint32_t* __restrict__ wave_rowbase, uint32_t* __restrict__ point_list, uint2* __restrict__ qlist,
                        uint32_t* __restrict__ qrow, uint32_t* __restrict__ qcount, int tiles_x, int tiles_y, const uint32_t* __restrict__ counters) {
    constexpr int M16 = 64 * 16, W16 = M16 + M16 / 32;
    __shared__ uint32_t s_v[W16], s_r[W16];
    if (counters[GS2M_CNT_SPAN_MID] == 0u) return;
    const int lane = threadIdx.x;
    const int tile = tile_of_block(blockIdx.x, tiles_x, tiles_y);
    if (tile < 0) return;
    const uint2 raw = reinterpret_cast<const uint2*>(ranges_raw)[tile];
    const uint32_t start = ~raw.x, n = raw.y != 0u ? raw.y - start : 0u;
    if (n <= 512u || n > 1024u) return;
    sort_tile_wave<16, 4>(tile, start, n, slot_sorted, e_rec, wave_rowbase, point_list, qlist, qrow, qcount, s_v, s_r, lane);
}

template <int E>
__device__ __forceinline__ void cross_wave(uint32_t (&k)[E], uint32_t (&x)[E], const int tid, const int partner, const bool mirrored, const bool lower,
                                           uint32_t* s_x) {
    uint32_t ok[E], ox[E];
#pragma unroll
    for (int e = 0; e < E; e++) s_x[skew(tid * E + e)] = k[e];
    gs2m_sync();
#pragma unroll
    for (int e = 0; e < E; e++) ok[e] = s_x[skew(partner * E + (mirrored ? E - 1 - e : e))];
    gs2m_sync();
#pragma unroll
    for (int e = 0; e < E; e++) s_x[skew(tid * E + e)] = x[e];
    gs2m_sync();
#pragma unroll
    for (int e = 0; e < E; e++) ox[e] = s_x[skew(partner * E + (mirrored ? E - 1 - e : e))];
    gs2m_sync();
#pragma unroll
    for (int e = 0; e < E; e++) {
        const uint32_t mn = min(k[e], ok[e]), mx = max(k[e], ok[e]);
        const uint32_t nk = lower ? mn : mx;
        x[e] = nk == k[e] ? x[e] : ox[e];
        k[e] = nk;
    }
}
template <int E, int LE>
__device__ __forceinline__ void network_wg(uint32_t (&k)[E], uint32_t (&x)[E], const int tid, uint32_t* s_x) {
    const int lane = tid & 63, wave = tid >> 6;
    levels<E, LE, 1>(k, x, lane, 0xFFFFFFFFu);
    cross_wave<E>(k, x, tid, tid ^ 127, true, (wave & 1) == 0, s_x);
    xor_steps<E, LE, LE + 5>(k, x, lane);
    cross_wave<E>(k, x, tid, tid ^ 255, true, wave < 2, s_x);
    cross_wave<E>(k, x, tid, tid ^ 64, false, (wave & 1) == 0, s_x);
    xor_steps<E, LE, LE + 5>(k, x, lane);
}

constexpr int WG_MAX = 4096;
template <int E, int LE>
__device__ __forceinline__ void sort_tile_wg(const int tile, const uint32_t start, const uint32_t n, const uint32_t* __restrict__ slot_sorted,
                                             const uint4* __restrict__ e_rec, const uint32_t* __restrict__ wave_rowbase,
                                             uint32_t* __restrict__ point_list, uint2* __restrict__ qlist, uint32_t* __restrict__ qrow,
                                             uint32_t* __restrict__ qcount, uint32_t* s_v, uint32_t* s_r, uint32_t* s_x, const int tid,
                                             uint32_t* __restrict__ clk = nullptr) {
    const int lane = tid & 63, wave = tid >> 6;
#ifdef GS2M_TS_CLOCK
    const unsigned long long c0 = wall_clock64();
    int cphase = 0;
#define TS_CLK() do { if (tid == 0 && clk) clk[16 * tile + (cphase++)] = (uint32_t)(wall_clock64() - c0); } while (0)
#else
#define TS_CLK() do {} while (0)
#endif
    uint32_t key[E], idx[E], rb[E];
    constexpr int BATCH = E < 8 ? E : 8;
    static_for<0, E / BATCH>([&](auto bc) {
        constexpr int e0 = BATCH * decltype(bc)::value;
        uint32_t slot[BATCH];
#pragma unroll
        for (int e = 0; e < BATCH; e++) {
            const uint32_t p = (uint32_t)((e0 + e) * 256 + tid);
            slot[e] = p < n ? slot_sorted[start + p] : 0u;
        }
        uint4 rc[BATCH];
#pragma unroll
        for (int e = 0; e < BATCH; e++) rc[e] = (uint32_t)((e0 + e) * 256 + tid) < n ? e_rec[slot[e]] : make_uint4(0u, 0u, 0xFFFFFFFFu, 0u);
        static_for<0, BATCH>([&](auto ec) {
            constexpr int e = decltype(ec)::value;
            const uint32_t p = (uint32_t)((e0 + e) * 256 + tid);
            key[e0 + e] = rc[e].z;
            idx[e0 + e] = p;
            s_v[skew((int)p)] = rc[e].x;
            s_r[skew((int)p)] = rc[e].y & ~GS2M_ROWS_BIG;
            rb[e0 + e] = p < n && (rc[e].y & GS2M_ROWS_BIG) == 0u ? wave_rowbase[(rc[e].x & GS2M_GID_MASK) >> 6] : 0u;
        });
        asm volatile("" ::: "memory");
    });
    TS_CLK();
    network_wg<E, LE>(key, idx, tid, s_x);
    TS_CLK();
#pragma unroll
    for (int e = 0; e < E; e++) s_r[skew(e * 256 + tid)] += rb[e];
    uint32_t sv[E], sr[E];
    auto pick_up = [&]() {
#pragma unroll
        for (int e = 0; e < E; e++) {
            const bool real = (uint32_t)(tid * E + e) < n;
            sv[e] = real ? s_v[skew((int)idx[e])] : 0u;
            sr[e] = real ? s_r[skew((int)idx[e])] : 0u;
        }
    };
    auto park = [&]() {
#pragma unroll
        for (int e = 0; e < E; e++) {
            s_v[skew(tid * E + e)] = sv[e];
            s_r[skew(tid * E + e)] = sr[e];
        }
    };
    gs2m_sync();
    pick_up();
    bool tie = false;
#pragma unroll
    for (int e = 0; e + 1 < E; e++) tie |= (uint32_t)(tid * E + e + 1) < n && key[e] == key[e + 1];
    s_x[tid] = key[0];
    gs2m_sync();
    tie |= tid < 255 && (uint32_t)(tid * E + E) < n && key[E - 1] == s_x[tid + 1];
    if (gs2m_sync_or(tie) != 0) {
#pragma unroll
        for (int e = 0; e < E; e++) {
            s_v[skew(tid * E + e)] = key[e];
            s_r[skew(tid * E + e)] = idx[e];
        }
        gs2m_sync();
        uint32_t pos[E];
        tie_positions<E>(key, idx, pos, tid, n, s_v, s_r);
        gs2m_sync();
#pragma unroll
        for (int e = 0; e < E; e++) {
            s_v[skew((int)pos[e])] = sv[e];
            s_r[skew((int)pos[e])] = sr[e];
        }
    } else {
        park();
    }
    TS_CLK();
    gs2m_sync();
    TS_CLK();
    for (uint32_t k = (uint32_t)tid; k < n; k += 256) point_list[start + k] = s_v[skew((int)k)];
    const int q = wave;
    uint2* out = qlist + (size_t)4 * start + (size_t)q * n;
    uint32_t* orow = qrow + (size_t)4 * start + (size_t)q * n;
    uint32_t run = 0;
    const unsigned long long lt = lane == 0 ? 0ull : (~0ull >> (64 - lane));
    for (uint32_t base = 0; base < n; base += GS2M_WAVE) {
        const uint32_t k = base + (uint32_t)lane;
        uint32_t v = 0, r = 0;
        if (k < n) { v = s_v[skew((int)k)]; r = s_r[skew((int)k)]; }
        const uint32_t mask = v >> GS2M_GID_BITS;
        const bool hit = ((mask >> q) & 1u) != 0u;
        const unsigned long long m = __builtin_amdgcn_ballot_w64(hit);
        if (hit) {
            const uint32_t o = run + (uint32_t)__popcll(m & lt);
            out[o] = make_uint2(v, k);
            orow[o] = r + (uint32_t)__popc(mask & ((1u << q) - 1u));
        }
        run += (uint32_t)__popcll(m);
    }
    if (lane == 0) qcount[tile * 4 + q] = run;
    TS_CLK();
#ifdef GS2M_TS_CLOCK
    if (tid == 0 && clk) { clk[16 * tile + 14] = n; clk[16 * tile + 15] = (uint32_t)(c0 & 0xFFFFFFFFull); }
#endif
}

constexpr int BIG_CHUNK = 4096;
__device__ __forceinline__ void sort_tile_big(const int tile, const uint32_t start, const uint32_t n, const uint32_t* __restrict__ slot_sorted,
                                              const uint4* __restrict__ e_rec, const uint32_t* __restrict__ wave_rowbase, uint32_t* __restrict__ point_list,
                                              uint32_t* __restrict__ row_tmp ,
                                              uint2* __restrict__ qlist, uint32_t* __restrict__ qrow, uint32_t* __restrict__ qcount,
                                              uint32_t* s_x ) {
    const int tid = threadIdx.x, wave = tid >> 6, lane = tid & 63;
    uint32_t* const K = reinterpret_cast<uint32_t*>(qlist + (size_t)4 * start);
    uint32_t* const I = K + n;
    auto barrier = [&]() {
        __threadfence_block();
        gs2m_sync();
    };
    constexpr int E = 16, LE = 4;
    for (uint32_t base = 0; base < n; base += BIG_CHUNK) {
        uint32_t key[E], idx[E];
        static_for<0, E / 8>([&](auto bc) {
            constexpr int e0 = 8 * decltype(bc)::value;
            uint32_t slot[8];
#pragma unroll
            for (int e = 0; e < 8; e++) {
                const uint32_t p = base + (uint32_t)((e0 + e) * 256 + tid);
                slot[e] = p < n ? slot_sorted[start + p] : 0u;
            }
            static_for<0, 8>([&](auto ec) {
                constexpr int e = decltype(ec)::value;
                const uint32_t p = base + (uint32_t)((e0 + e) * 256 + tid);
                key[e0 + e] = p < n ? e_rec[slot[e]].z : 0xFFFFFFFFu;
                idx[e0 + e] = p;
            });
        });
        network_wg<E, LE>(key, idx, tid, s_x);
#pragma unroll
        for (int e = 0; e < E; e++) {
            const uint32_t i = base + (uint32_t)(tid * E + e);
            if (i < n) { K[i] = key[e]; I[i] = idx[e]; }
        }
    }
    barrier();
    auto cex = [&](uint32_t i, uint32_t p) {
        const uint32_t a = K[i], b = K[p];
        if (b < a) {
            const uint32_t xa = I[i], xb = I[p];
            K[i] = b; K[p] = a; I[i] = xb; I[p] = xa;
        }
    };
    for (int kb = 13; (1u << (kb - 1)) < n; kb++) {
        const uint32_t half = 1u << (kb - 1), mask = (1u << kb) - 1u;
        for (uint32_t q = tid;; q += 256) {
            const uint32_t i = ((q >> (kb - 1)) << kb) | (q & (half - 1u));
            if (i >= n) break;
            const uint32_t p = i ^ mask;
            if (p < n) cex(i, p);
        }
        barrier();
        for (int jb = kb - 2; jb >= 12; jb--) {
            const uint32_t j = 1u << jb;
            for (uint32_t q = tid;; q += 256) {
                const uint32_t i = ((q >> jb) << (jb + 1)) | (q & (j - 1u));
                if (i >= n) break;
                const uint32_t p = i | j;
                if (p < n) cex(i, p);
            }
            barrier();
        }
        for (uint32_t base = 0; base < n; base += BIG_CHUNK) {
            uint32_t key[E], idx[E];
#pragma unroll
            for (int e = 0; e < E; e++) {
                const uint32_t i = base + (uint32_t)(tid * E + e);
                key[e] = i < n ? K[i] : 0xFFFFFFFFu;
                idx[e] = i < n ? I[i] : i;
            }
            cross_wave<E>(key, idx, tid, tid ^ 128, false, (wave & 2) == 0, s_x);
            cross_wave<E>(key, idx, tid, tid ^ 64, false, (wave & 1) == 0, s_x);
            xor_steps<E, LE, LE + 5>(key, idx, lane);
#pragma unroll
            for (int e = 0; e < E; e++) {
                const uint32_t i = base + (uint32_t)(tid * E + e);
                if (i < n) { K[i] = key[e]; I[i] = idx[e]; }
            }
        }
        barrier();
    }
    uint32_t* const I2 = I + n;
    for (uint32_t p = tid; p < n; p += 256) {
        const uint32_t Kp = K[p], X = I[p];
        uint32_t a = p, cnt = 0;
        for (uint32_t j = p; j > 0u;) {
            j--;
            if (K[j] != Kp) break;
            a = j;
            cnt += I[j] < X ? 1u : 0u;
        }
        for (uint32_t j = p + 1u; j < n; j++) {
            if (K[j] != Kp) break;
            cnt += I[j] < X ? 1u : 0u;
        }
        I2[a + cnt] = X;
    }
    barrier();
    for (uint32_t p = tid; p < n; p += 256) {
        const uint4 rc = e_rec[slot_sorted[start + I2[p]]];
        point_list[start + p] = rc.x;
        row_tmp[start + p] = (rc.y & GS2M_ROWS_BIG) != 0u ? (rc.y & ~GS2M_ROWS_BIG) : rc.y + wave_rowbase[(rc.x & GS2M_GID_MASK) >> 6];
    }
    barrier();
    const int q = wave;
    uint2* out = qlist + (size_t)4 * start + (size_t)q * n;
    uint32_t* orow = qrow + (size_t)4 * start + (size_t)q * n;
    uint32_t run = 0;
    const unsigned long long lt = lane == 0 ? 0ull : (~0ull >> (64 - lane));
    for (uint32_t base = 0; base < n; base += GS2M_WAVE) {
        const uint32_t k = base + (uint32_t)lane;
        uint32_t v = 0, r = 0;
        if (k < n) { v = point_list[start + k]; r = row_tmp[start + k]; }
        const uint32_t mask = v >> GS2M_GID_BITS;
        const bool hit = ((mask >> q) & 1u) != 0u;
        const unsigned long long m = __builtin_amdgcn_ballot_w64(hit);
        if (hit) {
            const uint32_t o = run + (uint32_t)__popcll(m & lt);
            out[o] = make_uint2(v, k);
            orow[o] = r + (uint32_t)__popc(mask & ((1u << q) - 1u));
        }
        run += (uint32_t)__popcll(m);
    }
    if (lane == 0) qcount[tile * 4 + q] = run;
}

#ifndef GS2M_TS_WG_OCC
#define GS2M_TS_WG_OCC 6
#endif
template <int MAXE>
struct WgCfg {
    static constexpr int kMax = 256 * MAXE, kWords = kMax + kMax / 32;
    static constexpr int kLds = 3 * kWords;
};
template <int MAXE>
__global__ void __launch_bounds__(256) __attribute__((amdgpu_waves_per_eu(MAXE >= 8 ? 3 : GS2M_TS_WG_OCC, 8)))
tile_sort_wg_kernel(const uint32_t* __restrict__ ranges_raw, uint2* __restrict__ ranges, const uint32_t* __restrict__ slot_sorted,
                    const uint4* __restrict__ e_rec, const uint32_t* __restrict__ wave_rowbase, uint32_t* __restrict__ point_list,
                    uint32_t* __restrict__ row_tmp, uint2* __restrict__ qlist, uint32_t* __restrict__ qrow, uint32_t* __restrict__ qcount,
                    int tiles_x, int tiles_y, uint32_t nblocks, uint32_t* __restrict__ counters, int take_mid) {
    constexpr int WORDS = WgCfg<MAXE>::kWords;
    __shared__ uint32_t s_all[WgCfg<MAXE>::kLds];
    if constexpr (MAXE >= 8) {
        if (counters[GS2M_CNT_SPAN_LONG] == 0u && !(take_mid && counters[GS2M_CNT_SPAN_MID] != 0u)) return;
    }
    uint32_t* const s_v = s_all, * const s_r = s_all + WORDS, * const s_x = s_all + 2 * WORDS;
    const int tid = threadIdx.x;
    for (uint32_t blk = blockIdx.x; blk < nblocks; blk += gridDim.x) {
        const int tile = tile_of_block((int)blk, tiles_x, tiles_y);
        if (tile < 0) continue;
        const uint2 raw = reinterpret_cast<const uint2*>(ranges_raw)[tile];
        const uint32_t start = raw.y != 0u ? ~raw.x : 0u, n = raw.y != 0u ? raw.y - start : 0u;
        if constexpr (MAXE < 8) {
            if (ranges != nullptr) {
                if (tid == 0) ranges[tile] = raw.y != 0u ? make_uint2(start, raw.y) : make_uint2(0u, 0u);
                if (n == 0u && tid < 4) qcount[tile * 4 + tid] = 0u;
            }
            if (n > 1024u && tid == 0) counters[GS2M_CNT_SPAN_LONG] = 1u;
            if (n == 0u || n > 1024u) continue;
            if (n <= 256u) sort_tile_wg<1, 0>(tile, start, n, slot_sorted, e_rec, wave_rowbase, point_list, qlist, qrow, qcount, s_v, s_r, s_x, tid, row_tmp);
            else if (n <= 512u) sort_tile_wg<2, 1>(tile, start, n, slot_sorted, e_rec, wave_rowbase, point_list, qlist, qrow, qcount, s_v, s_r, s_x, tid, row_tmp);
            else sort_tile_wg<4, 2>(tile, start, n, slot_sorted, e_rec, wave_rowbase, point_list, qlist, qrow, qcount, s_v, s_r, s_x, tid, row_tmp);
        } else {
            if (n <= 512u || (n <= 1024u && !take_mid)) continue;
            if (n <= 1024u) sort_tile_wg<4, 2>(tile, start, n, slot_sorted, e_rec, wave_rowbase, point_list, qlist, qrow, qcount, s_v, s_r, s_x, tid, row_tmp);
            else if (n <= 2048u) sort_tile_wg<8, 3>(tile, start, n, slot_sorted, e_rec, wave_rowbase, point_list, qlist, qrow, qcount, s_v, s_r, s_x, tid, row_tmp);
            else if (n <= (uint32_t)WG_MAX) sort_tile_wg<16, 4>(tile, start, n, slot_sorted, e_rec, wave_rowbase, point_list, qlist, qrow, qcount, s_v, s_r, s_x, tid, row_tmp);
            else sort_tile_big(tile, start, n, slot_sorted, e_rec, wave_rowbase, point_list, row_tmp, qlist, qrow, qcount, s_all);
        }
        gs2m_sync();
    }
}

}

static std::atomic<int> g_ts_policy{0};
void gs2m_set_tile_sort_policy_impl(int policy) { g_ts_policy = policy; }

void gs2m_launch_tile_sort(size_t tiles, int tiles_x, int tiles_y, size_t R , const BinningState& b, const ImageState& im,
                           const GeomState& g, hipStream_t s) {
    if (tiles == 0) return;
    const unsigned grid = tile_grid(tiles_x, tiles_y);
    static const int env_policy = getenv("GS2M_TS_POLICY") ? atoi(getenv("GS2M_TS_POLICY")) : 0;
    const int set_policy = g_ts_policy.load(std::memory_order_relaxed), policy = set_policy != 0 ? set_policy : env_policy;
    const bool waves = policy == 2 || policy == 3 || (policy == 0 && tiles >= 2560);
    const bool mid_own_kernel = policy != 3 && (R == SIZE_MAX || R > (size_t)400 * tiles);
    const unsigned wg_grid = grid < 2048u ? grid : 2048u;
    if (waves) {
        tile_sort_wave_kernel<<<grid, 64, 0, s>>>(im.ranges_raw, im.ranges, b.slot_sorted, b.e_rec, g.wave_rowbase, b.point_list, b.qlist, b.qrow, im.qcount,
                                                  tiles_x, tiles_y, 512u, g.counters);
        if (mid_own_kernel)
            tile_sort_wave16_kernel<<<grid, 64, 0, s>>>(im.ranges_raw, b.slot_sorted, b.e_rec, g.wave_rowbase, b.point_list, b.qlist, b.qrow, im.qcount, tiles_x, tiles_y, g.counters);
    } else {
        tile_sort_wg_kernel<4><<<wg_grid, 256, 0, s>>>(im.ranges_raw, im.ranges, b.slot_sorted, b.e_rec, g.wave_rowbase, b.point_list, b.sort_valA, b.qlist, b.qrow,
                                                       im.qcount, tiles_x, tiles_y, grid, g.counters, 0);
    }
    tile_sort_wg_kernel<16><<<wg_grid < 768u ? wg_grid : 768u , 256, 0, s>>>(im.ranges_raw, nullptr, b.slot_sorted, b.e_rec, g.wave_rowbase, b.point_list, b.sort_valA,
                                                                             b.qlist, b.qrow, im.qcount, tiles_x, tiles_y, grid, g.counters, waves && !mid_own_kernel ? 1 : 0);
}
```

gs-2m_amd/gs2m_native.py:

```python
import ctypes as C
import os
import subprocess

_HERE = os.path.dirname(os.path.abspath(__file__))
CSRC = os.path.join(_HERE, "csrc")
LIB_PATH = os.environ.get("GS2M_LIB", os.path.join(CSRC, "libgs2m_raster.so"))

ALLOC_FN = C.CFUNCTYPE(C.c_void_p, C.c_size_t, C.c_void_p)


class Prealloc(C.Structure):
    _fields_ = [("ptr", C.c_void_p), ("capacity", C.c_size_t), ("fallback", ALLOC_FN), ("fallback_user", C.c_void_p),
                ("used_fallback", C.c_int), ("requested", C.c_size_t)]


class Layout(C.Structure):
    _fields_ = [(n, C.c_uint64) for n in (
        "geom_bytes", "rec", "tiles_touched", "depth_key", "rect", "gauss_rows", "clamped", "wave_rowbase", "counters",
        "binning_bytes", "point_list", "tile_keys", "qlist", "qrow",
        "image_bytes", "final_T", "n_contrib", "ranges", "qcount")]


class STREAM(C.c_void_p):
    """`void* stream` as an entry point's LAST parameter: the function enqueues GPU work (call it through `launch`)."""


p, i, f, d, ll, ull, A, s = C.c_void_p, C.c_int, C.c_float, C.c_double, C.c_longlong, C.c_ulonglong, ALLOC_FN, STREAM
SIGNATURES = {
    "gs2m_raster_forward": (i, [A, p, A, p, A, p, i, i, i, p, i, i, p, p, p, p, p, f, p, p, p, p, p, p, f, f, i, i, p,
                                p, p, p, s]),
    "gs2m_raster_backward": (i, [i, i, i, i, p, i, i, p, p, p, p, f, p, p, p, p, p, p, f, f, p, p, p, p, p, i, p, p, p,
                                 p, p, p, p, p, p, p, p, p, A, p, s]),
    "gs2m_raster_mark_visible": (i, [i, p, p, p, p, s]),
    "gs2m_knn_dist2": (i, [i, p, p, A, p, s]),
    "gs2m_debug_layout": (i, [i, i, i, i, C.POINTER(Layout)]),
    "gs2m_set_reference_binning": (i, [i]),
    "gs2m_raster_forward_split_sh": (i, [A, p, A, p, A, p, i, i, i, p, i, i, p, p, p, p, p, p, f, p, p, p, p, p, p, f,
                                         f, i, i, p, p, p, p, s]),
    "gs2m_raster_backward_split_sh": (i, [i, i, i, i, p, i, i, p, p, p, p, p, f, p, p, p, p, p, p, f, f, p, p, p, p, p,
                                          i, p, p, p, p, p, p, p, p, p, p, p, p, p, A, p, s]),
    "gs2m_pack_features_forward": (i, [i, p, p, p, p, p, p, p, p, i, i, p, s]),
    "gs2m_pack_features_backward": (i, [i, p, p, p, p, p, i, i, p, p, p, p, p, p, s]),
    "gs2m_gbuffer_post_forward": (i, [i, i, p, p, p, i, p, p, p, s]),
    "gs2m_gbuffer_post_backward": (i, [i, i, p, p, p, i, p, p, p, s]),
    "gs2m_gbuffer_maps_backward": (i, [i, i, p, p, p, i, p, p, p, p, p, p, p, p, p, s]),
    "gs2m_sobel_normal_forward": (i, [i, i, p, p, p, p, f, f, f, f, p, s]),
    "gs2m_sobel_normal_backward": (i, [i, i, p, p, p, p, f, f, f, f, p, p, p, s]),
    "gs2m_activate_forward": (i, [i, p, p, p, p, p, p, p, p, p, p, p, p, s]),
    "gs2m_activate_backward": (i, [i, p, p, p, p, p, p, p, p, p, p, p, p, p, p, p, p, p, p, s]),
    "gs2m_set_spin_wait": (i, [i]),
    "gs2m_set_sort_tickets": (i, [i]),
    "gs2m_set_tile_sort_policy": (i, [i]),
    "gs2m_prealloc_alloc": (p, [C.c_size_t, p]),
    "gs2m_set_debug": (i, [i]),
    "gs2m_set_markers": (i, [i]),
    "gs2m_stage_name": (C.c_char_p, [i]),
    "gs2m_raster_forward_token": (ull, []),
    "gs2m_raster_dense_rows": (ll, [ull]),
    "gs2m_raster_backward_rows_hint": (i, [ll]),
    "gs2m_debug_tile_sort": (i, [i, p, p, p, p, p, p, p, p, p, p, s]),
    "gs2m_debug_radix_temp_bytes": (i, [ll, i, C.POINTER(ull)]),
    "gs2m_debug_radix_plan": (i, [i, C.POINTER(i), C.POINTER(i), C.POINTER(i)]),
    "gs2m_debug_radix_sort": (i, [ll, i, p, p, p, p, p, p, p, ull, i, p, p, s]),
    "gs2m_debug_block_scans": (i, [ll, p, p, p, p, ll, p, p, p, p, s]),
    "gs2m_debug_blend_forward": (i, [i, i, i, p, p, p, p, p, p, p, p, p, p, p, s]),
    "gs2m_debug_blend_backward": (i, [i, i, i, p, p, p, p, p, p, p, p, p, p, p, p, s]),
    "gs2m_debug_row_floats": (i, [i]),
    "gs2m_profile_mode": (i, [i]),
    "gs2m_profile_sampling": (i, [i]),
    "gs2m_profile_collect": (i, [C.POINTER(C.c_float), C.POINTER(C.c_int), i]),
    "gs2m_version": (C.c_char_p, []),
    "gs2m_texture_cube_forward": (i, [i, i, i, p, p, p, p, p, s]),
    "gs2m_texture_cube_backward": (i, [i, i, i, p, p, p, p, p, i, s]),
    "gs2m_texture_2d_clamp_forward": (i, [i, i, i, i, p, p, p, s]),
    "gs2m_texture_2d_clamp_backward": (i, [i, i, i, i, p, p, p, s]),
    "gs2m_diffuse_cubemap_forward": (i, [i, p, p, s]),
    "gs2m_diffuse_cubemap_backward": (i, [i, p, p, s]),
    "gs2m_cubemap_texel_table": (i, [i, p, s]),
    "gs2m_specular_cubemap_forward": (i, [i, f, f, p, p, p, s]),
    "gs2m_specular_cubemap_backward": (i, [i, f, f, p, p, p, s]),
    "gs2m_specular_cubemap_normalized_forward": (i, [i, f, f, p, p, p, p, s]),
    "gs2m_specular_cubemap_normalized_backward": (i, [i, f, f, p, p, p, p, p, s]),
    "gs2m_pbr_shade_forward": (i, [i, p, p, p, p, p, p, i, i, p, i, i, p, p, f, f, p, p, p, p, s]),
    "gs2m_pbr_shade_backward": (i, [i, p, p, p, p, p, p, i, i, p, i, i, p, p, f, f, p, p, p, p, p, i, s]),
    "gs2m_pbr_inputs_forward": (i, [i, i, p, p, p, p, p, f, f, p, p, p, p, s]),
    "gs2m_pbr_inputs_backward": (i, [i, i, p, p, p, s]),
    "gs2m_patch_ncc_forward": (i, [i, p, p, p, p, p, i, i, p, p, p, f, i, p, s]),
    "gs2m_patch_ncc_backward": (i, [i, p, p, p, p, p, i, i, p, p, p, f, i, p, p, p, s]),
    "gs2m_patch_ncc_roughness": (i, [i, p, p, p, p, p, i, i, p, p, p, f, i, p, p, p, s]),
    "gs2m_mvs_set_deterministic": (None, [i]),
    "gs2m_mvs_get_deterministic": (i, []),
    "gs2m_grid_sample_border_forward": (i, [i, i, i, i, p, p, p, s]),
    "gs2m_grid_sample_border_backward": (i, [i, i, i, i, p, p, p, p, p, s]),
    "gs2m_mv_geo_forward": (i, [i, i, i, i, p, p, p, p, p, p, p, p, p, p, f, p, p, p, s]),
    "gs2m_mv_geo_backward": (i, [i, i, i, i, p, p, p, p, p, p, p, p, p, p, f, p, p, p, p, p, p, s]),
    "gs2m_adam_step": (i, [i, p, d, d, d, s]),
    "gs2m_ssim_forward": (i, [i, i, i, i, f, f, p, p, p, p, p, p, s]),
    "gs2m_ssim_backward": (i, [i, i, i, i, p, p, p, p, p, p, p, s]),
    "gs2m_ssim_backward_uniform": (i, [i, i, i, i, p, p, p, f, f, p, p, p, p, s]),
    "gs2m_loss_workspace_bytes": (i, []),
    "gs2m_edge_gradient": (i, [i, i, p, p, p, p, s]),
    "gs2m_image_loss_forward": (i, [i, i, p, i, p, p, p, p, p, p, p, p, f, f, p, p, p, s]),
    "gs2m_image_loss_backward": (i, [i, i, p, i, p, p, p, p, p, p, p, f, f, p, p, p, p, p, s]),
    "gs2m_tv_loss_forward": (i, [i, i, i, p, p, p, i, f, p, p, s]),
    "gs2m_tv_loss_backward": (i, [i, i, i, p, p, p, i, f, p, p, s]),
    "gs2m_mv_geo_loss_forward": (i, [i, p, p, p, f, f, f, f, p, p, p, p, s]),
    "gs2m_mv_geo_loss_backward": (i, [i, p, p, p, f, f, f, f, p, p, p, p, s]),
    "gs2m_mv_take_forward": (i, [i, p, i, i, p, p, p, p, p, p, p, s]),
    "gs2m_mv_take_backward": (i, [i, p, i, i, p, p, p, p, s]),
    "gs2m_ncc_tail_forward": (i, [i, p, p, p, p, s]),
    "gs2m_ncc_tail_backward": (i, [i, p, p, p, p, p, s]),
    "gs2m_subset_thin": (i, [i, p, i, ull, p, i, p, p, s]),
    "gs2m_subset_remove": (i, [i, i, ull, p, p, s]),
    "gs2m_affine_mean": (i, [ll, p, f, f, p, p, s]),
    "gs2m_plane_loss_forward": (i, [i, p, i, p, f, p, p, s]),
    "gs2m_plane_loss_backward": (i, [i, p, i, p, f, p, p, p, s]),
    "gs2m_densification_stats": (i, [i, p, p, p, p, p, p, p, p, s]),
    "gs2m_tsdf_workspace_bytes": (i, [p, i, p, p]),
    "gs2m_tsdf_points_aabb": (i, [i, i, p, f, f, f, f, f, p, p, s]),
    "gs2m_tsdf_touch": (i, [p, f, f, i, i, p, f, f, f, f, f, p, i, p, p, p, p, p, p, s]),
    "gs2m_tsdf_integrate": (i, [f, f, i, i, p, p, f, f, f, f, f, p, i, p, p, p, p, p, s]),
    "gs2m_tsdf_mesh_count": (i, [p, i, p, p, p, p, p, p, s]),
    "gs2m_tsdf_mesh_emit": (i, [p, f, i, p, p, p, p, p, ll, ll, p, p, p, s]),
    "gs2m_tsdf_block_coords": (i, [i, p, p, s]),
    "gs2m_mesh_post_workspace_bytes": (i, [ll, ll, p, p]),
    "gs2m_mesh_cluster_triangles": (i, [ll, ll, p, p, p, p, p, s]),
    "gs2m_mesh_keep_clusters": (i, [ll, p, p, i, p, s]),
    "gs2m_mesh_compact": (i, [ll, ll, p, p, p, p, p, p, p, p, p, s]),
    "gs2m_eval_transform": (i, [ll, p, d, p, p, s]),
    "gs2m_eval_sample_workspace_bytes": (i, [ll, ll, p, p]),
    "gs2m_eval_sample_rows": (i, [ll, p, ll, p, d, p, p, s]),
    "gs2m_eval_sample_count": (i, [ll, ll, p, p, p, s]),
    "gs2m_eval_sample_emit": (i, [ll, p, ll, p, ll, p, p, ll, p, s]),
    "gs2m_eval_gather": (i, [ll, p, p, p, s]),
    "gs2m_eval_grid_bytes": (i, [ll, p, p]),
    "gs2m_eval_grid_build": (i, [ll, p, d, p, p, s]),
    "gs2m_eval_thin_workspace_bytes": (i, [ll, p]),
    "gs2m_eval_thin": (i, [ll, p, p, d, p, p, p, s]),
    "gs2m_eval_filter": (i, [ll, p, p, p, p, d, p, p, p, s]),
    "gs2m_eval_above_plane": (i, [ll, p, p, p, s]),
    "gs2m_eval_scan_workspace_bytes": (i, [ll, p]),
    "gs2m_eval_compact": (i, [ll, p, p, i, p, p, p, s]),
    "gs2m_eval_nearest": (i, [ll, p, ll, d, p, d, p, s]),
    "gs2m_eval_nearest_index": (i, [ll, p, ll, d, p, d, p, p, s]),
    "gs2m_eval_masked_mean": (i, [ll, p, d, p, p, p, s]),
    "gs2m_eval_dilate_bytes": (i, [i, i, i, p]),
    "gs2m_eval_dilate_disk": (i, [i, i, i, p, i, p, s]),
    "gs2m_eval_cull_flags": (i, [ll, p, i, p, i, i, p, i, i, p, s]),
    "gs2m_eval_cull_workspace_bytes": (i, [ll, ll, p]),
    "gs2m_eval_cull_triangles": (i, [ll, p, ll, p, p, p, p, s]),
    "gs2m_tnt_mesh_points": (i, [ll, p, ll, p, p, p, s]),
    "gs2m_tnt_transform": (i, [ll, p, p, p, s]),
    "gs2m_tnt_crop_flags": (i, [ll, p, i, d, d, i, p, p, s]),
    "gs2m_tnt_voxel_workspace_bytes": (i, [ll, p]),
    "gs2m_tnt_voxel_downsample": (i, [ll, p, d, p, p, p, s]),
    "gs2m_tnt_stride_gather": (i, [ll, p, ll, p, s]),
    "gs2m_tnt_icp_workspace_bytes": (i, [p]),
    "gs2m_tnt_icp_moments": (i, [ll, p, ll, p, p, p, p, p, s]),
    "gs2m_tnt_histogram": (i, [ll, p, i, p, p, s]),
}
del p, i, f, d, ll, ull, A, s
EXPORTS = tuple(SIGNATURES)

STAGES = ("preprocess", "unused1", "scan", "emit", "tile_sort", "lists", "blend_fwd", "unused7", "blend_bwd",
          "gaussian_bwd")

_lib = None


def build(jobs=8, force=False):
    cmd = ["make", "-C", CSRC, "-j", str(jobs)]
    if force:
        cmd.append("-B")
    subprocess.check_call(cmd, stdout=subprocess.DEVNULL)
    return LIB_PATH


def lib():
    global _lib
    if _lib is not None:
        return _lib
    if not os.path.exists(LIB_PATH):
        raise RuntimeError(
            f"gs2m: HIP extension not built: {LIB_PATH} is missing. Run `python -c 'import __graft_entry__ as g; "
            f"g.build()'` (needs hipcc, --offload-arch=gfx950). There is no CPU fallback.")
    L = C.CDLL(LIB_PATH)
    for name, (restype, argtypes) in SIGNATURES.items():
        fn = getattr(L, name)
        fn.restype, fn.argtypes = restype, argtypes
    _lib = L
    return L


ERRORS = {-1: "invalid argument", -2: "HIP runtime error", -3: "scratch allocation failed", -4: "unsupported size",
          -5: "Point culled! This point should have been prefiltered (prefiltered=True and a Gaussian has view z <= 0.2; the reference traps the device here, cuda_rasterizer/auxiliary.h:155-158)"}


class _NoGuard:
    def __enter__(self):
        return None

    def __exit__(self, *exc):
        return False


_NO_GUARD = _NoGuard()


def device_guard(device):
    import torch
    idx = device.index if hasattr(device, "index") else device
    if idx is None or idx == torch.cuda.current_device():
        return _NO_GUARD
    return torch.cuda.device(device)


def stream_ptr(device=None):
    import torch
    idx = None if device is None else (device.index if hasattr(device, "index") else device)
    if idx is None:
        idx = torch.cuda.current_device()
    return torch._C._cuda_getCurrentRawStream(idx)


def check(rc, what):
    if rc <= -100:
        raise RuntimeError(f"gs2m: {what} failed in stage `{lib().gs2m_stage_name(-100 - rc).decode()}` (debug mode)")
    if rc < 0:
        raise RuntimeError(f"gs2m: {what} failed: {ERRORS.get(rc, rc)}")
    return rc


def launch(name, device, *args):
    fn = getattr(lib(), name)
    if fn.argtypes[-1] is not STREAM:
        raise TypeError(f"gs2m: {name} takes no stream: call it as check(lib().{name}(...), ...)")
    with device_guard(device):
        return check(fn(*args, stream_ptr(device)), name)


def ptr(t):
    return None if t is None or t.numel() == 0 else t.data_ptr()


def f32(t, name, shape=None, *, who, optional=False):
    import torch
    if optional and (t is None or t.numel() == 0):
        return t
    if not isinstance(t, torch.Tensor) or not t.is_cuda:
        raise RuntimeError(f"{who}: `{name}` must be a CUDA tensor on a HIP device; there is no CPU path")
    if t.dtype != torch.float32:
        raise RuntimeError(f"{who}: `{name}` must be float32, got {t.dtype}")
    if shape is not None and tuple(t.shape) != tuple(shape):
        raise RuntimeError(f"{who}: `{name}` must have shape {tuple(shape)}, got {tuple(t.shape)}")
    return t.contiguous()


def set_debug(on):
    check(lib().gs2m_set_debug(int(bool(on))), "gs2m_set_debug")


def set_markers(on):
    check(lib().gs2m_set_markers(int(bool(on))), "gs2m_set_markers")


def reset_modes():
    L = lib()
    L.gs2m_set_reference_binning(0); L.gs2m_set_spin_wait(1); L.gs2m_set_debug(0); L.gs2m_set_sort_tickets(0); L.gs2m_set_tile_sort_policy(0)
    L.gs2m_set_markers(0); L.gs2m_profile_mode(0)


def debug_layout(P, R, W, H):
    lay = Layout()
    check(lib().gs2m_debug_layout(P, R, W, H, C.byref(lay)), "gs2m_debug_layout")
    return lay


def set_sort_tickets(on):
    check(lib().gs2m_set_sort_tickets(int(bool(on))), "gs2m_set_sort_tickets")


def set_tile_sort_policy(policy):
    check(lib().gs2m_set_tile_sort_policy(int(policy)), "gs2m_set_tile_sort_policy")


def set_spin_wait(on):
    check(lib().gs2m_set_spin_wait(int(bool(on))), "gs2m_set_spin_wait")


def profile_mode(mode, every=1):
    check(lib().gs2m_profile_sampling(int(every)), "gs2m_profile_sampling")
    check(lib().gs2m_profile_mode(int(mode)), "gs2m_profile_mode")


def profile_collect():
    n = len(STAGES)
    ms = (C.c_float * n)()
    cnt = (C.c_int * n)()
    check(lib().gs2m_profile_collect(ms, cnt, n), "gs2m_profile_collect")
    return {STAGES[k]: (float(ms[k]), int(cnt[k])) for k in range(n)}


def set_reference_binning(on):
    check(lib().gs2m_set_reference_binning(1 if on else 0), "gs2m_set_reference_binning")
```

include/gs2m_raster.h:

```cpp
#ifndef GS2M_RASTER_H
#define GS2M_RASTER_H

#include <stddef.h>
#include <stdint.h>

#ifdef __cplusplus
extern "C" {
#endif

#define GS2M_NUM_CHANNELS 3
#define GS2M_NUM_FEATURES 10
#define GS2M_TILE 16

#define GS2M_OK 0
#define GS2M_ERR_INVALID_ARG (-1)
#define GS2M_ERR_HIP (-2)
#define GS2M_ERR_ALLOC (-3)
#define GS2M_ERR_UNSUPPORTED (-4)
#define GS2M_ERR_PREFILTERED (-5)
#define GS2M_ERR_STAGE(st) (-100 - (st))

typedef char* (*gs2m_alloc_fn)(size_t bytes, void* user);

int gs2m_raster_forward(
    gs2m_alloc_fn geometry_alloc, void* geometry_user,
    gs2m_alloc_fn binning_alloc, void* binning_user,
    gs2m_alloc_fn image_alloc, void* image_user,
    int P, int D, int M,
    const float* background,
    int width, int height,
    const float* means3D,
    const float* shs,
    const float* colors_precomp,
    const float* opacities,
    const float* scales,
    float scale_modifier,
    const float* rotations,
    const float* cov3D_precomp,
    const float* features,
    const float* viewmatrix,
    const float* projmatrix,
    const float* cam_pos,
    float tan_fovx, float tan_fovy,
    int prefiltered,
    int feature_count,
    float* out_color,
    int* out_radii,
    int* out_observe,
    float* out_buffer,
    void* stream);

int gs2m_raster_backward(
    int P, int D, int M, int R,
    const float* background,
    int width, int height,
    const float* means3D,
    const float* shs,
    const float* colors_precomp,
    const float* scales,
    float scale_modifier,
    const float* rotations,
    const float* cov3D_precomp,
    const float* features,
    const float* viewmatrix,
    const float* projmatrix,
    const float* campos,
    float tan_fovx, float tan_fovy,
    const int* radii,
    const float* buffer,
    char* geom_buffer,
    char* binning_buffer,
    char* image_buffer,
    int feature_count,
    const float* grad_colors,
    const float* grad_buffer,
    float* dL_dmeans2D,
    float* dL_dconics,
    float* dL_dopacities,
    float* dL_dcolors,
    float* dL_dmeans3D,
    float* dL_dcov3D,
    float* dL_dshs,
    float* dL_dscales,
    float* dL_drots,
    float* dL_dfeatures,
    gs2m_alloc_fn scratch_alloc, void* scratch_user,
    void* stream);

int gs2m_raster_mark_visible(int P, const float* means3D, const float* viewmatrix,
                             const float* projmatrix, uint8_t* present, void* stream);

int gs2m_knn_dist2(int P, const float* points, float* mean_dists,
                   gs2m_alloc_fn scratch_alloc, void* scratch_user, void* stream);


typedef struct gs2m_layout {
    uint64_t geom_bytes;
    uint64_t rec;
    uint64_t tiles_touched;
    uint64_t depth_key;
    uint64_t rect;
    uint64_t gauss_rows;
    uint64_t clamped;
    uint64_t wave_rowbase;
    uint64_t counters;
    uint64_t binning_bytes;
    uint64_t point_list;
    uint64_t tile_keys;
    uint64_t qlist;
    uint64_t qrow;
    uint64_t image_bytes;
    uint64_t final_T;
    uint64_t n_contrib;
    uint64_t ranges;
    uint64_t qcount;
} gs2m_layout;

int gs2m_debug_layout(int P, int R, int width, int height, gs2m_layout* out);

int gs2m_set_reference_binning(int on);

int gs2m_raster_forward_split_sh(gs2m_alloc_fn geometry_alloc, void* geometry_user, gs2m_alloc_fn binning_alloc,
                        void* binning_user, gs2m_alloc_fn image_alloc, void* image_user, int P, int D, int M,
                        const float* background, int width, int height, const float* means3D, const float* sh_dc, const float* sh_rest,
                        const float* colors_precomp, const float* opacities, const float* scales, float scale_modifier,
                        const float* rotations, const float* cov3D_precomp, const float* features,
                        const float* viewmatrix, const float* projmatrix, const float* cam_pos, float tan_fovx,
                        float tan_fovy, int prefiltered, int feature_count, float* out_color, int* out_radii,
                        int* out_observe, float* out_buffer, void* stream_);
int gs2m_raster_backward_split_sh(int P, int D, int M, int R, const float* background, int width, int height,
                         const float* means3D, const float* sh_dc, const float* sh_rest, const float* colors_precomp, const float* scales,
                         float scale_modifier, const float* rotations, const float* cov3D_precomp,
                         const float* features, const float* viewmatrix, const float* projmatrix, const float* campos,
                         float tan_fovx, float tan_fovy, const int* radii, const float* buffer, char* geom_buffer,
                         char* binning_buffer, char* image_buffer, int feature_count, const float* grad_colors,
                         const float* grad_buffer, float* dL_dmeans2D, float* dL_dconics, float* dL_dopacities,
                         float* dL_dcolors, float* dL_dmeans3D, float* dL_dcov3D, float* dL_dsh_dc, float* dL_dsh_rest, float* dL_dscales,
                         float* dL_drots, float* dL_dfeatures, gs2m_alloc_fn scratch_alloc, void* scratch_user,
                         void* stream_);

int gs2m_pack_features_forward(int P, const float* xyz, const float* scales, const float* rotations, const float* albedo,
                               const float* roughness, const float* metallic, const float* campos, const float* view,
                               int z_depth, int blend_metallic, float* features, void* stream);
int gs2m_pack_features_backward(int P, const float* xyz, const float* scales, const float* rotations, const float* campos,
                                const float* view, int z_depth, int blend_metallic, const float* dL_dfeatures,
                                float* dL_dxyz, float* dL_drotations, float* dL_dalbedo, float* dL_droughness,
                                float* dL_dmetallic, void* stream);
int gs2m_gbuffer_post_forward(int width, int height, const float* buffer, const float* rays, const float* view, int z_depth,
                              uint8_t* normal_mask, float* local_normal_map, float* depth_map, void* stream);
int gs2m_gbuffer_post_backward(int width, int height, const float* buffer, const float* rays, const float* view,
                               int z_depth, const float* dL_dlocal_normal, const float* dL_ddepth, float* dL_dbuffer,
                               void* stream);

int gs2m_gbuffer_maps_backward(int width, int height, const float* buffer, const float* rays, const float* view,
                               int z_depth, const float* dL_dlocal_normal, const float* dL_ddepth, const float* dL_dalpha,
                               const float* dL_ddistance, const float* dL_dnormal, const float* dL_dalbedo,
                               const float* dL_droughness, const float* dL_dmetallic, float* dL_dbuffer, void* stream);

int gs2m_sobel_normal_forward(int width, int height, const float* depth, const float* alpha, const float* bg,
                              const float* view, float fx, float fy, float cx, float cy, float* sobel_map, void* stream);
int gs2m_sobel_normal_backward(int width, int height, const float* depth, const float* alpha, const float* bg,
                               const float* view, float fx, float fy, float cx, float cy, const float* dL_dsobel,
                               float* dL_ddepth, float* dL_dalpha, void* stream);

int gs2m_activate_forward(int P, const float* scaling, const float* rotation, const float* opacity, const float* albedo,
                          const float* roughness, const float* metallic, float* scales, float* rotations, float* opacities,
                          float* albedo_a, float* roughness_a, float* metallic_a, void* stream);
int gs2m_activate_backward(int P, const float* rotation, const float* scales, const float* opacities, const float* albedo_a,
                           const float* roughness_a, const float* metallic_a, const float* dL_dscales,
                           const float* dL_drotations, const float* dL_dopacities, const float* dL_dalbedo_a,
                           const float* dL_droughness_a, const float* dL_dmetallic_a, float* dL_dscaling, float* dL_drotation,
                           float* dL_dopacity, float* dL_dalbedo, float* dL_droughness, float* dL_dmetallic, void* stream);

int gs2m_set_spin_wait(int on);

int gs2m_set_sort_tickets(int on);

int gs2m_set_tile_sort_policy(int policy);

typedef struct gs2m_prealloc {
    char* ptr;
    size_t capacity;
    gs2m_alloc_fn fallback;
    void* fallback_user;
    int used_fallback;
    size_t requested;
} gs2m_prealloc;
char* gs2m_prealloc_alloc(size_t bytes, void* user);

int gs2m_set_debug(int on);
int gs2m_set_markers(int on);
const char* gs2m_stage_name(int stage);


unsigned long long gs2m_raster_forward_token(void);
long long gs2m_raster_dense_rows(unsigned long long token);
int gs2m_raster_backward_rows_hint(long long dense_rows);

int gs2m_debug_tile_sort(int tiles, const unsigned* ranges_raw, unsigned* ranges, const unsigned* slot_sorted, const unsigned* e_rec,
                         const unsigned* wave_rowbase, unsigned* point_list, unsigned* row_tmp,
                         unsigned* qlist, unsigned* qrow, unsigned* qcount, void* stream);

int gs2m_debug_radix_temp_bytes(long long n, int total_bits, unsigned long long* bytes);
int gs2m_debug_radix_plan(int total_bits, int* npass, int* bits4, int* shift4);
int gs2m_debug_radix_sort(long long n, int total_bits, const unsigned* kin, const unsigned* vin, unsigned* kA, unsigned* vA,
                          unsigned* kB, unsigned* vB, void* temp, unsigned long long temp_bytes, int prezeroed,
                          unsigned* range_raw, const unsigned* ext_hist, void* stream);
int gs2m_debug_block_scans(long long n_blocks, const unsigned* block_tt, const unsigned* block_hu, unsigned* block_pref,
                           unsigned* block_hupref, long long n_waves, const unsigned* wave_rows, unsigned* wave_rowbase,
                           unsigned* counters, unsigned* landing_out, void* stream);
int gs2m_debug_blend_forward(int W, int H, int fc, const float* bg, const unsigned* ranges, const unsigned* qlist,
                             const unsigned* qcount, const float* rec, float* out_color, float* out_buffer, float* final_T,
                             unsigned* n_contrib, int* observe, unsigned* qlast, void* stream);
int gs2m_debug_blend_backward(int W, int H, int fc, const float* bg, const unsigned* ranges, const unsigned* qlist,
                              const unsigned* qcount, const unsigned* qrow, const unsigned* qlast, const float* rec,
                              const float* final_T, const unsigned* n_contrib, const float* grad_color, const float* grad_buffer,
                              float* rows, void* stream);
int gs2m_debug_row_floats(int fc);

#define GS2M_NUM_STAGES 10
int gs2m_profile_mode(int mode);
int gs2m_profile_sampling(int every);
int gs2m_profile_collect(float* stage_ms, int* stage_count, int n_stages);

const char* gs2m_version(void);

#ifdef __cplusplus
}
#endif
#endif
```

Before: 855.8 views/s.

## Sort per-instance records directly as SoA payload instead of slot indices

```diff
diff --git a/gs-2m_amd/csrc/api.hip b/gs-2m_amd/csrc/api.hip
--- a/gs-2m_amd/csrc/api.hip
+++ b/gs-2m_amd/csrc/api.hip
@@ -3,6 +3,7 @@
 #include <mutex>
 #include <chrono>
 #include <dlfcn.h>
+#include <stdlib.h>
 
 #define HIP_TRY(expr)                          \
     do {                                       \
@@ -265,8 +266,8 @@
         }
         {
             StageTimer t(ST_TILE_SORT, s, &failed_stage);
-            HIP_TRY(gs2m_radix_sort_pairs(b.temp, b.temp_bytes, b.keys_unsorted, nullptr, b.sort_keyA, b.sort_valA, b.tile_keys, b.slot_sorted,
-                                          (size_t)R, tile_bits, true, s, im.ranges_raw, g.tile_hist));
+            HIP_TRY(gs2m_radix_sort_rec3(b.temp, b.temp_bytes, b.tile_keys, b.rec, b.sort_keyA, b.recA, b.tile_keys, b.rec,
+                                         (size_t)R, tile_bits, true, s, im.ranges_raw, g.tile_hist));
         }
     } else {
         HIP_TRY(gs2m_zero_async(im.ranges_raw, tiles * 2 * sizeof(uint32_t), s));
@@ -501,6 +502,9 @@
     out->tile_keys = (uint64_t)(uintptr_t)b.tile_keys;
     out->qlist = (uint64_t)(uintptr_t)b.qlist;
     out->qrow = (uint64_t)(uintptr_t)b.qrow;
+    out->rec_id = (uint64_t)(uintptr_t)b.rec[0];
+    out->rec_row = (uint64_t)(uintptr_t)b.rec[1];
+    out->rec_depth = (uint64_t)(uintptr_t)b.rec[2];
     out->image_bytes = im.total_bytes;
     out->final_T = (uint64_t)(uintptr_t)im.final_T;
     out->n_contrib = (uint64_t)(uintptr_t)im.n_contrib;
@@ -544,8 +548,7 @@
                          unsigned* qrow, unsigned* qcount, void* stream_) {
     if (tiles < 0 || !ranges_raw || !ranges || !slot_sorted || !e_rec || !wave_rowbase || !point_list || !row_tmp || !qlist || !qrow || !qcount) return GS2M_ERR_INVALID_ARG;
     BinningState b = {};
-    b.slot_sorted = const_cast<uint32_t*>(slot_sorted); b.e_rec = reinterpret_cast<uint4*>(const_cast<unsigned*>(e_rec));
-    b.point_list = point_list; b.sort_valA = row_tmp; b.qlist = reinterpret_cast<uint2*>(qlist); b.qrow = qrow;
+    b.point_list = point_list; b.sort_keyA = row_tmp; b.qlist = reinterpret_cast<uint2*>(qlist); b.qrow = qrow;
     ImageState im = {};
     im.ranges_raw = const_cast<uint32_t*>(ranges_raw);
     im.ranges = reinterpret_cast<uint2*>(ranges);
@@ -559,6 +562,27 @@
     if (dbg_counters[dev] == nullptr) HIP_TRY(hipMalloc(&dbg_counters[dev], 64 * sizeof(uint32_t)));
     HIP_TRY(hipMemsetAsync(dbg_counters[dev], 0, 64 * sizeof(uint32_t), (hipStream_t)stream_));
     g.counters = dbg_counters[dev];
+    static uint32_t* dbg_rec[64] = {nullptr};
+    static size_t dbg_rec_cap[64] = {0};
+    size_t n = 0;
+    if (tiles > 0) {
+        HIP_TRY(hipStreamSynchronize((hipStream_t)stream_));
+        uint32_t* host_raw = (uint32_t*)malloc((size_t)tiles * 2 * sizeof(uint32_t));
+        if (!host_raw) return GS2M_ERR_ALLOC;
+        const hipError_t ce = hipMemcpy(host_raw, ranges_raw, (size_t)tiles * 2 * sizeof(uint32_t), hipMemcpyDeviceToHost);
+        for (int t = 0; ce == hipSuccess && t < tiles; t++)
+            if ((size_t)host_raw[2 * t + 1] > n) n = host_raw[2 * t + 1];
+        free(host_raw);
+        HIP_TRY(ce);
+    }
+    const size_t per = gs2m_align_up((n > 0 ? n : 1) * sizeof(uint32_t));
+    if (dbg_rec_cap[dev] < 3 * per) {
+        if (dbg_rec[dev] != nullptr) { HIP_TRY(hipDeviceSynchronize()); HIP_TRY(hipFree(dbg_rec[dev])); dbg_rec[dev] = nullptr; dbg_rec_cap[dev] = 0; }
+        HIP_TRY(hipMalloc(&dbg_rec[dev], 3 * per));
+        dbg_rec_cap[dev] = 3 * per;
+    }
+    for (int w = 0; w < 3; w++) b.rec[w] = dbg_rec[dev] + (size_t)w * (per / sizeof(uint32_t));
+    gs2m_launch_gather_records(n, slot_sorted, reinterpret_cast<const uint4*>(e_rec), b.rec, (hipStream_t)stream_);
     gs2m_launch_tile_sort((size_t)tiles, tiles, 1, SIZE_MAX, b, im, g, (hipStream_t)stream_);
     HIP_TRY(hipGetLastError());
     return GS2M_OK;
@@ -582,6 +606,19 @@
     if (n < 0 || (n > 0 && (!kin || !kA || !vA || !kB || !vB || !temp))) return GS2M_ERR_INVALID_ARG;
     const hipError_t e = gs2m_radix_sort_pairs(temp, (size_t)temp_bytes, kin, vin, kA, vA, kB, vB, (size_t)n, total_bits, prezeroed != 0,
                                                (hipStream_t)stream_, range_raw, ext_hist);
+    return e == hipErrorInvalidValue ? GS2M_ERR_INVALID_ARG : gs2m_status(e);
+}
+
+int gs2m_debug_radix_sort_rec3(long long n, int total_bits, const unsigned* kin, const unsigned* vin, unsigned* kA, unsigned* vA, unsigned* kB,
+                               unsigned* vB, void* temp, unsigned long long temp_bytes, int prezeroed, unsigned* range_raw,
+                               const unsigned* ext_hist, void* stream_) {
+    if (n < 0 || (n > 0 && (!kin || !vin || !kA || !vA || !kB || !vB || !temp))) return GS2M_ERR_INVALID_ARG;
+    const size_t N = (size_t)n;
+    const uint32_t* const in3[3] = {vin, vin + N, vin + 2 * N};
+    uint32_t* const a3[3] = {vA, vA + N, vA + 2 * N};
+    uint32_t* const b3[3] = {vB, vB + N, vB + 2 * N};
+    const hipError_t e = gs2m_radix_sort_rec3(temp, (size_t)temp_bytes, kin, in3, kA, a3, kB, b3, N, total_bits, prezeroed != 0,
+                                              (hipStream_t)stream_, range_raw, ext_hist);
     return e == hipErrorInvalidValue ? GS2M_ERR_INVALID_ARG : gs2m_status(e);
 }
 
diff --git a/gs-2m_amd/csrc/binning.hip b/gs-2m_amd/csrc/binning.hip
--- a/gs-2m_amd/csrc/binning.hip
+++ b/gs-2m_amd/csrc/binning.hip
@@ -36,12 +36,10 @@
         off = gs2m_align_up(off + bytes);
         return p;
     };
-    b.keys_unsorted = (uint32_t*)take(R * 4);
-    b.e_rec = (uint4*)take(R * sizeof(uint4));
+    b.tile_keys = (uint32_t*)take(R * 4);
+    for (int w = 0; w < 3; w++) b.rec[w] = (uint32_t*)take(R * 4);
     b.sort_keyA = (uint32_t*)take(R * 4);
-    b.sort_valA = (uint32_t*)take(R * 4);
-    b.tile_keys = (uint32_t*)take(R * 4);
-    b.slot_sorted = (uint32_t*)take(R * 4);
+    for (int w = 0; w < 3; w++) b.recA[w] = (uint32_t*)take(R * 4);
     b.point_list = (uint32_t*)take(R * 4);
     b.qlist = (uint2*)take(R * 4 * sizeof(uint2));
     b.qrow = (uint32_t*)take(R * 4 * 4);
@@ -203,7 +201,8 @@
 __global__ void __launch_bounds__(256) emit_kernel(int P, int W, int H, int tiles_x, const uint2* __restrict__ rect,
                                                    const uint32_t* __restrict__ block_pref, const uint32_t* __restrict__ block_hupref,
                                                    const float4* __restrict__ rec,
-                                                   const uint32_t* __restrict__ depth_key, uint32_t* __restrict__ keys_out, uint4* __restrict__ e_rec,
+                                                   const uint32_t* __restrict__ depth_key, uint32_t* __restrict__ keys_out, uint32_t* __restrict__ rec_id,
+                                                   uint32_t* __restrict__ rec_row, uint32_t* __restrict__ rec_depth,
                                                    HeavyUnit* __restrict__ hrec,
                                                    uint32_t* __restrict__ gauss_rows, uint32_t* __restrict__ wave_rows,
                                                    uint32_t* __restrict__ counters, uint32_t* __restrict__ tile_hist, int npass, int4 hbits,
@@ -285,7 +284,11 @@
             if (pc) atomicAdd(&s_rc[wave][lo], pc);
         }
         const uint32_t pin = wave_inclusive_scan_u32(pc, lane);
-        if (j < total) e_rec[slot] = make_uint4((gid0 + (uint32_t)(wave * GS2M_WAVE + lo)) | (mask << GS2M_GID_BITS), rows_run + pin - pc, s_depth[wave][lo], 0u);
+        if (j < total) {
+            rec_id[slot] = (gid0 + (uint32_t)(wave * GS2M_WAVE + lo)) | (mask << GS2M_GID_BITS);
+            rec_row[slot] = rows_run + pin - pc;
+            rec_depth[slot] = s_depth[wave][lo];
+        }
         rows_run += __shfl(pin, 63, 64);
     }
     if (i < P && !heavy) gauss_rows[i] = s_rc[wave][lane];
@@ -317,7 +320,8 @@
 
 __global__ void __launch_bounds__(256) emit_heavy_kernel(uint32_t units, int W, int H, int tiles_x, const uint2* __restrict__ rect, const float4* __restrict__ rec,
                                                          const uint32_t* __restrict__ depth_key, const uint32_t* __restrict__ gauss_rows,
-                                                         uint32_t* __restrict__ keys_out, uint4* __restrict__ e_rec, HeavyUnit* __restrict__ hrec,
+                                                         uint32_t* __restrict__ keys_out, uint32_t* __restrict__ rec_id, uint32_t* __restrict__ rec_row,
+                                                         uint32_t* __restrict__ rec_depth, HeavyUnit* __restrict__ hrec,
                                                          uint32_t* __restrict__ tile_hist, int npass, int4 hbits, int4 hshift) {
     __shared__ uint32_t s_th[4][256];
 #pragma unroll
@@ -341,7 +345,9 @@
             const uint2 km = expand_instance(r.x, rw, t, geo, ct, W, H, tiles_x);
             keys_out[off + t] = km.x;
             for (int p = 0; p < npass; p++) atomicAdd(&s_th[p][(km.x >> hs[p]) & ((1u << hb[p]) - 1u)], 1u);
-            e_rec[off + t] = make_uint4(gid | (km.y << GS2M_GID_BITS), GS2M_ROWS_BIG | (4u * (u * GS2M_UNIT + (uint32_t)lane)), dk, 0u);
+            rec_id[off + t] = gid | (km.y << GS2M_GID_BITS);
+            rec_row[off + t] = GS2M_ROWS_BIG | (4u * (u * GS2M_UNIT + (uint32_t)lane));
+            rec_depth[off + t] = dk;
             pc = (uint32_t)__popc(km.y);
         }
         hrec[u].pop[lane] = (uint8_t)pc;
@@ -371,11 +377,11 @@
     int npass = 0, bits[4], shift[4];
     gs2m_radix_plan(tile_bits, &npass, bits, shift);
     const int4 hbits = make_int4(bits[0], bits[1], bits[2], bits[3]), hshift = make_int4(shift[0], shift[1], shift[2], shift[3]);
-    emit_kernel<<<(P + 255) / 256, 256, 0, s>>>(P, W, H, tiles_x, g.rect, g.block_pref, g.block_hupref, g.rec, g.depth_key, b.keys_unsorted, b.e_rec, b.hrec,
+    emit_kernel<<<(P + 255) / 256, 256, 0, s>>>(P, W, H, tiles_x, g.rect, g.block_pref, g.block_hupref, g.rec, g.depth_key, b.tile_keys, b.rec[0], b.rec[1], b.rec[2], b.hrec,
                                                 g.gauss_rows, g.wave_rows, g.counters, g.tile_hist, npass, hbits, hshift, crowded, zero);
     if (heavy_units > 0u)
-        emit_heavy_kernel<<<(heavy_units + 3u) / 4u, 256, 0, s>>>(heavy_units, W, H, tiles_x, g.rect, g.rec, g.depth_key, g.gauss_rows, b.keys_unsorted, b.e_rec,
-                                                                  b.hrec, g.tile_hist, npass, hbits, hshift);
+        emit_heavy_kernel<<<(heavy_units + 3u) / 4u, 256, 0, s>>>(heavy_units, W, H, tiles_x, g.rect, g.rec, g.depth_key, g.gauss_rows, b.tile_keys, b.rec[0], b.rec[1],
+                                                                  b.rec[2], b.hrec, g.tile_hist, npass, hbits, hshift);
     gs2m_launch_rowscan(P, g, landing, s);
 }
 
diff --git a/gs-2m_amd/csrc/common.h b/gs-2m_amd/csrc/common.h
--- a/gs-2m_amd/csrc/common.h
+++ b/gs-2m_amd/csrc/common.h
@@ -65,12 +65,10 @@
     size_t total_bytes;
 };
 struct BinningState {
-    uint32_t* keys_unsorted;
-    uint4* e_rec;
+    uint32_t* tile_keys;
+    uint32_t* rec[3];
     uint32_t* sort_keyA;
-    uint32_t* sort_valA;
-    uint32_t* tile_keys;
-    uint32_t* slot_sorted;
+    uint32_t* recA[3];
     uint32_t* point_list;
     uint2* qlist;
     uint32_t* qrow;
@@ -181,6 +179,9 @@
                                  uint32_t* range_raw = nullptr, const uint32_t* ext_hist = nullptr);
 #define GS2M_HIST_COPIES 8
 #define GS2M_HIST_COPY_WORDS 1024
+hipError_t gs2m_radix_sort_rec3(void* temp, size_t temp_bytes, const uint32_t* kin, const uint32_t* const vin[3], uint32_t* kA,
+                                uint32_t* const vA[3], uint32_t* kB, uint32_t* const vB[3], size_t n, int total_bits, bool prezeroed,
+                                hipStream_t s, uint32_t* range_raw = nullptr, const uint32_t* ext_hist = nullptr);
 void gs2m_radix_plan(int total_bits, int* npass, int bits[4], int shift[4]);
 void gs2m_radix_zero_region(void* temp, size_t n, int total_bits, uint32_t** ptr, size_t* words);
 
@@ -206,6 +207,7 @@
 void gs2m_launch_recount_heavy(int P, const GeomState& g, hipStream_t s);
 void gs2m_launch_heavy_reduce(float* rows, int rowf, const BinningState& b, const GeomState& g, long long heavy_units, hipStream_t s);
 void gs2m_set_tile_sort_policy_impl(int policy);
+void gs2m_launch_gather_records(size_t n, const uint32_t* slot_sorted, const uint4* e_rec, uint32_t* const rec[3], hipStream_t s);
 void gs2m_launch_tile_sort(size_t tiles, int tiles_x, int tiles_y, size_t R, const BinningState& b, const ImageState& im, const GeomState& g, hipStream_t s);
 hipError_t gs2m_zero_async(void* p, size_t bytes, hipStream_t s);
 
diff --git a/gs-2m_amd/csrc/radix_sort.hip b/gs-2m_amd/csrc/radix_sort.hip
--- a/gs-2m_amd/csrc/radix_sort.hip
+++ b/gs-2m_amd/csrc/radix_sort.hip
@@ -14,13 +14,13 @@
 constexpr int RS_ITEMS = 16;
 constexpr int RS_TILE = RS_THREADS * RS_ITEMS;
 constexpr int RS_MAXPASS = 4;
-int resident_tiles() {
+int compute_units() {
     static int cached[64] = {0};
     int dev = 0;
     if (hipGetDevice(&dev) != hipSuccess || dev < 0 || dev >= 64) return 0;
     if (cached[dev] == 0) {
         int cus = 0;
-        cached[dev] = hipDeviceGetAttribute(&cus, hipDeviceAttributeMultiprocessorCount, dev) == hipSuccess && cus > 0 ? 4 * cus : -1;
+        cached[dev] = hipDeviceGetAttribute(&cus, hipDeviceAttributeMultiprocessorCount, dev) == hipSuccess && cus > 0 ? cus : -1;
     }
     return cached[dev] > 0 ? cached[dev] : 0;
 }
@@ -88,10 +88,21 @@
     }
 }
 
-template <int BITS>
+struct PayU32 {
+    static constexpr int WORDS = 1, WG_PER_CU = 4;
+    using In = const uint32_t* __restrict__;
+    using Out = uint32_t* __restrict__;
+};
+struct PayRec3 {
+    static constexpr int WORDS = 3, WG_PER_CU = 3;
+    struct In { const uint32_t* w[3]; };
+    struct Out { uint32_t* w[3]; };
+};
+
+template <int BITS, typename PAY>
 __global__ void __launch_bounds__(RS_THREADS) rs_onesweep_kernel(
-    const uint32_t* __restrict__ keys_in, const uint32_t* __restrict__ vals_in, uint32_t* __restrict__ keys_out,
-    uint32_t* __restrict__ vals_out, uint32_t n, int shift, const uint32_t* __restrict__ ghist, uint32_t* ticket,
+    const uint32_t* __restrict__ keys_in, const typename PAY::In vals_in, uint32_t* __restrict__ keys_out,
+    const typename PAY::Out vals_out, uint32_t n, int shift, const uint32_t* __restrict__ ghist, uint32_t* ticket,
     uint32_t* status , uint32_t* range_raw, int hist_copies ) {
     constexpr int BINS = 1 << BITS;
     __shared__ uint32_t s_cnt[4][BINS];
@@ -108,12 +119,33 @@
     const uint32_t tile_count = min((uint32_t)RS_TILE, n - tile_base);
     const uint32_t segbase = tile_base + wave * (64 * RS_ITEMS);
 
+    constexpr bool REC = PAY::WORDS == 3;
     uint32_t key[RS_ITEMS], val[RS_ITEMS], rank[RS_ITEMS];
-#pragma unroll
-    for (int k = 0; k < RS_ITEMS; k++) {
-        const uint32_t i = segbase + k * 64 + lane;
-        key[k] = i < n ? keys_in[i] : 0xFFFFFFFFu;
-        val[k] = i < n ? (vals_in ? vals_in[i] : i) : 0u;
+    [[maybe_unused]] uint32_t val1[REC ? RS_ITEMS : 1], val2[REC ? RS_ITEMS : 1];
+    if constexpr (!REC) {
+#pragma unroll
+        for (int k = 0; k < RS_ITEMS; k++) {
+            const uint32_t i = segbase + k * 64 + lane;
+            key[k] = i < n ? keys_in[i] : 0xFFFFFFFFu;
+            val[k] = i < n ? (vals_in ? vals_in[i] : i) : 0u;
+        }
+    } else {
+#pragma unroll
+        for (int k = 0; k < RS_ITEMS; k++) {
+            const uint32_t i = segbase + k * 64 + lane;
+            key[k] = i < n ? keys_in[i] : 0xFFFFFFFFu;
+        }
+#pragma unroll
+        for (int k = 0; k < RS_ITEMS; k++) {
+            const uint32_t i = segbase + k * 64 + lane;
+            val[k] = i < n ? vals_in.w[0][i] : 0u;
+        }
+#pragma unroll
+        for (int k = 0; k < RS_ITEMS; k++) {
+            const uint32_t i = segbase + k * 64 + lane;
+            val1[k] = i < n ? vals_in.w[1][i] : 0u;
+            val2[k] = i < n ? vals_in.w[2][i] : 0u;
+        }
     }
     const unsigned long long lt = (1ull << lane) - 1ull;
     [[maybe_unused]] uint32_t run0 = 0;
@@ -175,6 +207,7 @@
             const uint32_t lp = s_cnt[wave][d] + rank[k];
             s_key[lp] = key[k];
             s_val[lp] = val[k];
+            if constexpr (REC) rank[k] = lp;
         }
     }
     if (tid < BINS) {
@@ -235,6 +268,7 @@
         s_gbase[tid] = digit_base + excl - tile_excl;
     }
     gs2m_sync();
+    [[maybe_unused]] uint32_t opos[REC ? RS_ITEMS : 1];
 #pragma unroll
     for (int k = 0; k < RS_ITEMS; k++) {
         const uint32_t i = k * RS_THREADS + tid;
@@ -242,22 +276,46 @@
             const uint32_t kk = s_key[i];
             const uint32_t pos = s_gbase[(kk >> shift) & (BINS - 1)] + i;
             keys_out[pos] = kk;
-            vals_out[pos] = s_val[i];
+            if constexpr (REC) {
+                vals_out.w[0][pos] = s_val[i];
+                opos[k] = pos;
+            } else {
+                vals_out[pos] = s_val[i];
+            }
             if (range_raw != nullptr) {
                 if (i == 0 || s_key[i - 1] != kk) atomicMax(&range_raw[2 * kk], ~pos);
                 if (i + 1 == tile_count || s_key[i + 1] != kk) atomicMax(&range_raw[2 * kk + 1], pos + 1u);
             }
         }
     }
-}
-
-template <int BITS>
-void launch_pass(const uint32_t* ki, const uint32_t* vi, uint32_t* ko, uint32_t* vo, uint32_t n, int shift,
+    if constexpr (REC) {
+        gs2m_sync();
+#pragma unroll
+        for (int k = 0; k < RS_ITEMS; k++) {
+            if (segbase + k * 64 + lane < n) {
+                s_key[rank[k]] = val1[k];
+                s_val[rank[k]] = val2[k];
+            }
+        }
+        gs2m_sync();
+#pragma unroll
+        for (int k = 0; k < RS_ITEMS; k++) {
+            const uint32_t i = k * RS_THREADS + tid;
+            if (i < tile_count) {
+                vals_out.w[1][opos[k]] = s_key[i];
+                vals_out.w[2][opos[k]] = s_val[i];
+            }
+        }
+    }
+}
+
+template <int BITS, typename PAY>
+void launch_pass(const uint32_t* ki, const typename PAY::In vi, uint32_t* ko, const typename PAY::Out vo, uint32_t n, int shift,
                  const uint32_t* ghist, uint32_t* ticket, uint32_t* status, int tiles, hipStream_t s, uint32_t* range_raw, int hist_copies) {
     static const bool env_tickets = getenv("GS2M_SORT_TICKETS") && atoi(getenv("GS2M_SORT_TICKETS")) != 0;
     const bool force_tickets = env_tickets || g_sort_tickets.load(std::memory_order_relaxed) != 0;
-    rs_onesweep_kernel<BITS><<<tiles, RS_THREADS, 0, s>>>(ki, vi, ko, vo, n, shift, ghist,
-                                                          (!force_tickets && tiles <= resident_tiles()) ? nullptr : ticket, status, range_raw, hist_copies);
+    rs_onesweep_kernel<BITS, PAY><<<tiles, RS_THREADS, 0, s>>>(ki, vi, ko, vo, n, shift, ghist,
+                                                          (!force_tickets && tiles <= PAY::WG_PER_CU * compute_units()) ? nullptr : ticket, status, range_raw, hist_copies);
 }
 
 }
@@ -282,9 +340,13 @@
     *words = (gs2m_align_up(RS_MAXPASS * 256 * 4) + GS2M_ALIGN + (size_t)p.npass * status_rows(tiles) * 256 * 4) / 4;
 }
 
-hipError_t gs2m_radix_sort_pairs(void* temp, size_t temp_bytes, const uint32_t* kin, const uint32_t* vin, uint32_t* kA,
-                                 uint32_t* vA, uint32_t* kB, uint32_t* vB, size_t n, int total_bits, bool prezeroed, hipStream_t s,
-                                 uint32_t* range_raw, const uint32_t* ext_hist) {
+namespace {
+PayU32::In pay_next(PayU32::Out o) { return o; }
+PayRec3::In pay_next(const PayRec3::Out& o) { return PayRec3::In{{o.w[0], o.w[1], o.w[2]}}; }
+
+template <typename PAY>
+hipError_t sort_impl(void* temp, size_t temp_bytes, const uint32_t* kin, typename PAY::In vin, uint32_t* kA, typename PAY::Out vA, uint32_t* kB,
+                     typename PAY::Out vB, size_t n, int total_bits, bool prezeroed, hipStream_t s, uint32_t* range_raw, const uint32_t* ext_hist) {
     if (n == 0) return hipSuccess;
     if (n > (size_t)VAL_MASK) return hipErrorInvalidValue;
     const SortPlan p = make_plan(total_bits);
@@ -301,22 +363,37 @@
     if (ext_hist == nullptr)
         rs_hist_kernel<<<workers, RS_THREADS, 0, s>>>(kin, (uint32_t)n, p.npass, make_int4(p.bits[0], p.bits[1], p.bits[2], p.bits[3]),
                                                       make_int4(p.shift[0], p.shift[1], p.shift[2], p.shift[3]), ghist, tiles, workers);
-    const uint32_t *ki = kin, *vi = vin;
+    const uint32_t* ki = kin;
+    typename PAY::In vi = vin;
     for (int i = 0; i < p.npass; i++) {
         uint32_t* ko = (i & 1) ? kB : kA;
-        uint32_t* vo = (i & 1) ? vB : vA;
+        const typename PAY::Out vo = (i & 1) ? vB : vA;
         uint32_t* st = status + (size_t)i * status_rows((size_t)tiles) * 256;
         const uint32_t* gh = (ext_hist ? ext_hist : ghist) + i * 256;
         const int hc = ext_hist ? GS2M_HIST_COPIES : 1;
         uint32_t* const rr = i == p.npass - 1 ? range_raw : nullptr;
         switch (p.bits[i]) {
-#define RS_CASE(B) case B: launch_pass<B>(ki, vi, ko, vo, (uint32_t)n, p.shift[i], gh, tickets + i, st, tiles, s, rr, hc); break;
+#define RS_CASE(B) case B: launch_pass<B, PAY>(ki, vi, ko, vo, (uint32_t)n, p.shift[i], gh, tickets + i, st, tiles, s, rr, hc); break;
             RS_CASE(0) RS_CASE(1) RS_CASE(2) RS_CASE(3) RS_CASE(4) RS_CASE(5) RS_CASE(6) RS_CASE(7) RS_CASE(8)
 #undef RS_CASE
             default: return hipErrorInvalidValue;
         }
         ki = ko;
-        vi = vo;
+        vi = pay_next(vo);
     }
     return hipGetLastError();
 }
+}
+
+hipError_t gs2m_radix_sort_pairs(void* temp, size_t temp_bytes, const uint32_t* kin, const uint32_t* vin, uint32_t* kA,
+                                 uint32_t* vA, uint32_t* kB, uint32_t* vB, size_t n, int total_bits, bool prezeroed, hipStream_t s,
+                                 uint32_t* range_raw, const uint32_t* ext_hist) {
+    return sort_impl<PayU32>(temp, temp_bytes, kin, vin, kA, vA, kB, vB, n, total_bits, prezeroed, s, range_raw, ext_hist);
+}
+
+hipError_t gs2m_radix_sort_rec3(void* temp, size_t temp_bytes, const uint32_t* kin, const uint32_t* const vin[3], uint32_t* kA,
+                                uint32_t* const vA[3], uint32_t* kB, uint32_t* const vB[3], size_t n, int total_bits, bool prezeroed,
+                                hipStream_t s, uint32_t* range_raw, const uint32_t* ext_hist) {
+    return sort_impl<PayRec3>(temp, temp_bytes, kin, PayRec3::In{{vin[0], vin[1], vin[2]}}, kA, PayRec3::Out{{vA[0], vA[1], vA[2]}}, kB,
+                              PayRec3::Out{{vB[0], vB[1], vB[2]}}, n, total_bits, prezeroed, s, range_raw, ext_hist);
+}
diff --git a/gs-2m_amd/csrc/tile_sort.hip b/gs-2m_amd/csrc/tile_sort.hip
--- a/gs-2m_amd/csrc/tile_sort.hip
+++ b/gs-2m_amd/csrc/tile_sort.hip
@@ -133,22 +133,20 @@
 }
 
 template <int E, int LE>
-__device__ __forceinline__ void sort_tile_wave(const int tile, const uint32_t start, const uint32_t n, const uint32_t* __restrict__ slot_sorted,
-                                               const uint4* __restrict__ e_rec, const uint32_t* __restrict__ wave_rowbase,
+__device__ __forceinline__ void sort_tile_wave(const int tile, const uint32_t start, const uint32_t n, const uint32_t* __restrict__ rec_id,
+                                               const uint32_t* __restrict__ rec_row, const uint32_t* __restrict__ rec_depth,
+                                               const uint32_t* __restrict__ wave_rowbase,
                                                uint32_t* __restrict__ point_list, uint2* __restrict__ qlist, uint32_t* __restrict__ qrow,
                                                uint32_t* __restrict__ qcount, uint32_t* s_v, uint32_t* s_r, const int lane) {
     uint32_t key[E], idx[E], rb[E];
     static_for<0, E / 8>([&](auto bc) {
         constexpr int e0 = 8 * decltype(bc)::value;
-        uint32_t slot[8];
+        uint3 rc[8];
 #pragma unroll
         for (int e = 0; e < 8; e++) {
             const uint32_t p = (uint32_t)((e0 + e) * GS2M_WAVE + lane);
-            slot[e] = p < n ? slot_sorted[start + p] : 0u;
-        }
-        uint4 rc[8];
-#pragma unroll
-        for (int e = 0; e < 8; e++) rc[e] = (uint32_t)((e0 + e) * GS2M_WAVE + lane) < n ? e_rec[slot[e]] : make_uint4(0u, 0u, 0xFFFFFFFFu, 0u);
+            rc[e] = p < n ? make_uint3(rec_id[start + p], rec_row[start + p], rec_depth[start + p]) : make_uint3(0u, 0u, 0xFFFFFFFFu);
+        }
         static_for<0, 8>([&](auto ec) {
             constexpr int e = decltype(ec)::value;
             const uint32_t p = (uint32_t)((e0 + e) * GS2M_WAVE + lane);
@@ -264,8 +262,8 @@
 }
 
 __global__ void __launch_bounds__(64) tile_sort_wave_kernel(const uint32_t* __restrict__ ranges_raw, uint2* __restrict__ ranges,
-                                                            const uint32_t* __restrict__ slot_sorted, const uint4* __restrict__ e_rec,
-                                                            const uint32_t* __restrict__ wave_rowbase,
+                                                            const uint32_t* __restrict__ rec_id, const uint32_t* __restrict__ rec_row,
+                                                            const uint32_t* __restrict__ rec_depth, const uint32_t* __restrict__ wave_rowbase,
                                                             uint32_t* __restrict__ point_list, uint2* __restrict__ qlist,
                                                             uint32_t* __restrict__ qrow, uint32_t* __restrict__ qcount, int tiles_x, int tiles_y,
                                                             uint32_t wave_max , uint32_t* __restrict__ counters) {
@@ -279,15 +277,15 @@
     if (n == 0u) {
         if (lane < 4) qcount[tile * 4 + lane] = 0u;
     } else if (n <= wave_max) {
-        sort_tile_wave<8, 3>(tile, range.x, n, slot_sorted, e_rec, wave_rowbase, point_list, qlist, qrow, qcount, s_v, s_r, lane);
+        sort_tile_wave<8, 3>(tile, range.x, n, rec_id, rec_row, rec_depth, wave_rowbase, point_list, qlist, qrow, qcount, s_v, s_r, lane);
     } else if (lane == 0) {
         counters[n <= 1024u ? GS2M_CNT_SPAN_MID : GS2M_CNT_SPAN_LONG] = 1u;
     }
 }
 
 __global__ void __launch_bounds__(64) __attribute__((amdgpu_waves_per_eu(4, 8)))
-tile_sort_wave16_kernel(const uint32_t* __restrict__ ranges_raw, const uint32_t* __restrict__ slot_sorted, const uint4* __restrict__ e_rec,
-                        const uint32_t* __restrict__ wave_rowbase, uint32_t* __restrict__ point_list, uint2* __restrict__ qlist,
+tile_sort_wave16_kernel(const uint32_t* __restrict__ ranges_raw, const uint32_t* __restrict__ rec_id, const uint32_t* __restrict__ rec_row,
+                        const uint32_t* __restrict__ rec_depth, const uint32_t* __restrict__ wave_rowbase, uint32_t* __restrict__ point_list, uint2* __restrict__ qlist,
                         uint32_t* __restrict__ qrow, uint32_t* __restrict__ qcount, int tiles_x, int tiles_y, const uint32_t* __restrict__ counters) {
     constexpr int M16 = 64 * 16, W16 = M16 + M16 / 32;
     __shared__ uint32_t s_v[W16], s_r[W16];
@@ -298,7 +296,7 @@
     const uint2 raw = reinterpret_cast<const uint2*>(ranges_raw)[tile];
     const uint32_t start = ~raw.x, n = raw.y != 0u ? raw.y - start : 0u;
     if (n <= 512u || n > 1024u) return;
-    sort_tile_wave<16, 4>(tile, start, n, slot_sorted, e_rec, wave_rowbase, point_list, qlist, qrow, qcount, s_v, s_r, lane);
+    sort_tile_wave<16, 4>(tile, start, n, rec_id, rec_row, rec_depth, wave_rowbase, point_list, qlist, qrow, qcount, s_v, s_r, lane);
 }
 
 template <int E>
@@ -338,8 +336,9 @@
 
 constexpr int WG_MAX = 4096;
 template <int E, int LE>
-__device__ __forceinline__ void sort_tile_wg(const int tile, const uint32_t start, const uint32_t n, const uint32_t* __restrict__ slot_sorted,
-                                             const uint4* __restrict__ e_rec, const uint32_t* __restrict__ wave_rowbase,
+__device__ __forceinline__ void sort_tile_wg(const int tile, const uint32_t start, const uint32_t n, const uint32_t* __restrict__ rec_id,
+                                             const uint32_t* __restrict__ rec_row, const uint32_t* __restrict__ rec_depth,
+                                             const uint32_t* __restrict__ wave_rowbase,
                                              uint32_t* __restrict__ point_list, uint2* __restrict__ qlist, uint32_t* __restrict__ qrow,
                                              uint32_t* __restrict__ qcount, uint32_t* s_v, uint32_t* s_r, uint32_t* s_x, const int tid,
                                              uint32_t* __restrict__ clk = nullptr) {
@@ -355,15 +354,12 @@
     constexpr int BATCH = E < 8 ? E : 8;
     static_for<0, E / BATCH>([&](auto bc) {
         constexpr int e0 = BATCH * decltype(bc)::value;
-        uint32_t slot[BATCH];
+        uint3 rc[BATCH];
 #pragma unroll
         for (int e = 0; e < BATCH; e++) {
             const uint32_t p = (uint32_t)((e0 + e) * 256 + tid);
-            slot[e] = p < n ? slot_sorted[start + p] : 0u;
-        }
-        uint4 rc[BATCH];
-#pragma unroll
-        for (int e = 0; e < BATCH; e++) rc[e] = (uint32_t)((e0 + e) * 256 + tid) < n ? e_rec[slot[e]] : make_uint4(0u, 0u, 0xFFFFFFFFu, 0u);
+            rc[e] = p < n ? make_uint3(rec_id[start + p], rec_row[start + p], rec_depth[start + p]) : make_uint3(0u, 0u, 0xFFFFFFFFu);
+        }
         static_for<0, BATCH>([&](auto ec) {
             constexpr int e = decltype(ec)::value;
             const uint32_t p = (uint32_t)((e0 + e) * 256 + tid);
@@ -453,8 +449,9 @@
 }
 
 constexpr int BIG_CHUNK = 4096;
-__device__ __forceinline__ void sort_tile_big(const int tile, const uint32_t start, const uint32_t n, const uint32_t* __restrict__ slot_sorted,
-                                              const uint4* __restrict__ e_rec, const uint32_t* __restrict__ wave_rowbase, uint32_t* __restrict__ point_list,
+__device__ __forceinline__ void sort_tile_big(const int tile, const uint32_t start, const uint32_t n, const uint32_t* __restrict__ rec_id,
+                                              const uint32_t* __restrict__ rec_row, const uint32_t* __restrict__ rec_depth,
+                                              const uint32_t* __restrict__ wave_rowbase, uint32_t* __restrict__ point_list,
                                               uint32_t* __restrict__ row_tmp ,
                                               uint2* __restrict__ qlist, uint32_t* __restrict__ qrow, uint32_t* __restrict__ qcount,
                                               uint32_t* s_x ) {
@@ -468,20 +465,11 @@
     constexpr int E = 16, LE = 4;
     for (uint32_t base = 0; base < n; base += BIG_CHUNK) {
         uint32_t key[E], idx[E];
-        static_for<0, E / 8>([&](auto bc) {
-            constexpr int e0 = 8 * decltype(bc)::value;
-            uint32_t slot[8];
-#pragma unroll
-            for (int e = 0; e < 8; e++) {
-                const uint32_t p = base + (uint32_t)((e0 + e) * 256 + tid);
-                slot[e] = p < n ? slot_sorted[start + p] : 0u;
-            }
-            static_for<0, 8>([&](auto ec) {
-                constexpr int e = decltype(ec)::value;
-                const uint32_t p = base + (uint32_t)((e0 + e) * 256 + tid);
-                key[e0 + e] = p < n ? e_rec[slot[e]].z : 0xFFFFFFFFu;
-                idx[e0 + e] = p;
-            });
+        static_for<0, E>([&](auto ec) {
+            constexpr int e = decltype(ec)::value;
+            const uint32_t p = base + (uint32_t)(e * 256 + tid);
+            key[e] = p < n ? rec_depth[start + p] : 0xFFFFFFFFu;
+            idx[e] = p;
         });
         network_wg<E, LE>(key, idx, tid, s_x);
 #pragma unroll
@@ -554,7 +542,8 @@
     }
     barrier();
     for (uint32_t p = tid; p < n; p += 256) {
-        const uint4 rc = e_rec[slot_sorted[start + I2[p]]];
+        const uint32_t src = start + I2[p];
+        const uint2 rc = make_uint2(rec_id[src], rec_row[src]);
         point_list[start + p] = rc.x;
         row_tmp[start + p] = (rc.y & GS2M_ROWS_BIG) != 0u ? (rc.y & ~GS2M_ROWS_BIG) : rc.y + wave_rowbase[(rc.x & GS2M_GID_MASK) >> 6];
     }
@@ -591,8 +580,8 @@
 };
 template <int MAXE>
 __global__ void __launch_bounds__(256) __attribute__((amdgpu_waves_per_eu(MAXE >= 8 ? 3 : GS2M_TS_WG_OCC, 8)))
-tile_sort_wg_kernel(const uint32_t* __restrict__ ranges_raw, uint2* __restrict__ ranges, const uint32_t* __restrict__ slot_sorted,
-                    const uint4* __restrict__ e_rec, const uint32_t* __restrict__ wave_rowbase, uint32_t* __restrict__ point_list,
+tile_sort_wg_kernel(const uint32_t* __restrict__ ranges_raw, uint2* __restrict__ ranges, const uint32_t* __restrict__ rec_id,
+                    const uint32_t* __restrict__ rec_row, const uint32_t* __restrict__ rec_depth, const uint32_t* __restrict__ wave_rowbase, uint32_t* __restrict__ point_list,
                     uint32_t* __restrict__ row_tmp, uint2* __restrict__ qlist, uint32_t* __restrict__ qrow, uint32_t* __restrict__ qcount,
                     int tiles_x, int tiles_y, uint32_t nblocks, uint32_t* __restrict__ counters, int take_mid) {
     constexpr int WORDS = WgCfg<MAXE>::kWords;
@@ -614,24 +603,39 @@
             }
             if (n > 1024u && tid == 0) counters[GS2M_CNT_SPAN_LONG] = 1u;
             if (n == 0u || n > 1024u) continue;
-            if (n <= 256u) sort_tile_wg<1, 0>(tile, start, n, slot_sorted, e_rec, wave_rowbase, point_list, qlist, qrow, qcount, s_v, s_r, s_x, tid, row_tmp);
-            else if (n <= 512u) sort_tile_wg<2, 1>(tile, start, n, slot_sorted, e_rec, wave_rowbase, point_list, qlist, qrow, qcount, s_v, s_r, s_x, tid, row_tmp);
-            else sort_tile_wg<4, 2>(tile, start, n, slot_sorted, e_rec, wave_rowbase, point_list, qlist, qrow, qcount, s_v, s_r, s_x, tid, row_tmp);
+            if (n <= 256u) sort_tile_wg<1, 0>(tile, start, n, rec_id, rec_row, rec_depth, wave_rowbase, point_list, qlist, qrow, qcount, s_v, s_r, s_x, tid, row_tmp);
+            else if (n <= 512u) sort_tile_wg<2, 1>(tile, start, n, rec_id, rec_row, rec_depth, wave_rowbase, point_list, qlist, qrow, qcount, s_v, s_r, s_x, tid, row_tmp);
+            else sort_tile_wg<4, 2>(tile, start, n, rec_id, rec_row, rec_depth, wave_rowbase, point_list, qlist, qrow, qcount, s_v, s_r, s_x, tid, row_tmp);
         } else {
             if (n <= 512u || (n <= 1024u && !take_mid)) continue;
-            if (n <= 1024u) sort_tile_wg<4, 2>(tile, start, n, slot_sorted, e_rec, wave_rowbase, point_list, qlist, qrow, qcount, s_v, s_r, s_x, tid, row_tmp);
-            else if (n <= 2048u) sort_tile_wg<8, 3>(tile, start, n, slot_sorted, e_rec, wave_rowbase, point_list, qlist, qrow, qcount, s_v, s_r, s_x, tid, row_tmp);
-            else if (n <= (uint32_t)WG_MAX) sort_tile_wg<16, 4>(tile, start, n, slot_sorted, e_rec, wave_rowbase, point_list, qlist, qrow, qcount, s_v, s_r, s_x, tid, row_tmp);
-            else sort_tile_big(tile, start, n, slot_sorted, e_rec, wave_rowbase, point_list, row_tmp, qlist, qrow, qcount, s_all);
+            if (n <= 1024u) sort_tile_wg<4, 2>(tile, start, n, rec_id, rec_row, rec_depth, wave_rowbase, point_list, qlist, qrow, qcount, s_v, s_r, s_x, tid, row_tmp);
+            else if (n <= 2048u) sort_tile_wg<8, 3>(tile, start, n, rec_id, rec_row, rec_depth, wave_rowbase, point_list, qlist, qrow, qcount, s_v, s_r, s_x, tid, row_tmp);
+            else if (n <= (uint32_t)WG_MAX) sort_tile_wg<16, 4>(tile, start, n, rec_id, rec_row, rec_depth, wave_rowbase, point_list, qlist, qrow, qcount, s_v, s_r, s_x, tid, row_tmp);
+            else sort_tile_big(tile, start, n, rec_id, rec_row, rec_depth, wave_rowbase, point_list, row_tmp, qlist, qrow, qcount, s_all);
         }
         gs2m_sync();
     }
 }
 
+}
+
+__global__ void __launch_bounds__(256) gather_records_kernel(uint32_t n, const uint32_t* __restrict__ slot_sorted, const uint4* __restrict__ e_rec,
+                                                             uint32_t* __restrict__ rec_id, uint32_t* __restrict__ rec_row, uint32_t* __restrict__ rec_depth) {
+    const uint32_t i = blockIdx.x * 256u + threadIdx.x;
+    if (i >= n) return;
+    const uint4 rc = e_rec[slot_sorted[i]];
+    rec_id[i] = rc.x;
+    rec_row[i] = rc.y;
+    rec_depth[i] = rc.z;
 }
 
 static std::atomic<int> g_ts_policy{0};
 void gs2m_set_tile_sort_policy_impl(int policy) { g_ts_policy = policy; }
+
+void gs2m_launch_gather_records(size_t n, const uint32_t* slot_sorted, const uint4* e_rec, uint32_t* const rec[3], hipStream_t s) {
+    if (n == 0) return;
+    gather_records_kernel<<<(unsigned)((n + 255) / 256), 256, 0, s>>>((uint32_t)n, slot_sorted, e_rec, rec[0], rec[1], rec[2]);
+}
 
 void gs2m_launch_tile_sort(size_t tiles, int tiles_x, int tiles_y, size_t R , const BinningState& b, const ImageState& im,
                            const GeomState& g, hipStream_t s) {
@@ -643,14 +647,14 @@
     const bool mid_own_kernel = policy != 3 && (R == SIZE_MAX || R > (size_t)400 * tiles);
     const unsigned wg_grid = grid < 2048u ? grid : 2048u;
     if (waves) {
-        tile_sort_wave_kernel<<<grid, 64, 0, s>>>(im.ranges_raw, im.ranges, b.slot_sorted, b.e_rec, g.wave_rowbase, b.point_list, b.qlist, b.qrow, im.qcount,
+        tile_sort_wave_kernel<<<grid, 64, 0, s>>>(im.ranges_raw, im.ranges, b.rec[0], b.rec[1], b.rec[2], g.wave_rowbase, b.point_list, b.qlist, b.qrow, im.qcount,
                                                   tiles_x, tiles_y, 512u, g.counters);
         if (mid_own_kernel)
-            tile_sort_wave16_kernel<<<grid, 64, 0, s>>>(im.ranges_raw, b.slot_sorted, b.e_rec, g.wave_rowbase, b.point_list, b.qlist, b.qrow, im.qcount, tiles_x, tiles_y, g.counters);
+            tile_sort_wave16_kernel<<<grid, 64, 0, s>>>(im.ranges_raw, b.rec[0], b.rec[1], b.rec[2], g.wave_rowbase, b.point_list, b.qlist, b.qrow, im.qcount, tiles_x, tiles_y, g.counters);
     } else {
-        tile_sort_wg_kernel<4><<<wg_grid, 256, 0, s>>>(im.ranges_raw, im.ranges, b.slot_sorted, b.e_rec, g.wave_rowbase, b.point_list, b.sort_valA, b.qlist, b.qrow,
+        tile_sort_wg_kernel<4><<<wg_grid, 256, 0, s>>>(im.ranges_raw, im.ranges, b.rec[0], b.rec[1], b.rec[2], g.wave_rowbase, b.point_list, b.sort_keyA, b.qlist, b.qrow,
                                                        im.qcount, tiles_x, tiles_y, grid, g.counters, 0);
     }
-    tile_sort_wg_kernel<16><<<wg_grid < 768u ? wg_grid : 768u , 256, 0, s>>>(im.ranges_raw, nullptr, b.slot_sorted, b.e_rec, g.wave_rowbase, b.point_list, b.sort_valA,
+    tile_sort_wg_kernel<16><<<wg_grid < 768u ? wg_grid : 768u , 256, 0, s>>>(im.ranges_raw, nullptr, b.rec[0], b.rec[1], b.rec[2], g.wave_rowbase, b.point_list, b.sort_keyA,
                                                                              b.qlist, b.qrow, im.qcount, tiles_x, tiles_y, grid, g.counters, waves && !mid_own_kernel ? 1 : 0);
 }
diff --git a/gs-2m_amd/gs2m_native.py b/gs-2m_amd/gs2m_native.py
--- a/gs-2m_amd/gs2m_native.py
+++ b/gs-2m_amd/gs2m_native.py
@@ -17,7 +17,7 @@
 class Layout(C.Structure):
     _fields_ = [(n, C.c_uint64) for n in (
         "geom_bytes", "rec", "tiles_touched", "depth_key", "rect", "gauss_rows", "clamped", "wave_rowbase", "counters",
-        "binning_bytes", "point_list", "tile_keys", "qlist", "qrow",
+        "binning_bytes", "point_list", "tile_keys", "qlist", "qrow", "rec_id", "rec_row", "rec_depth",
         "image_bytes", "final_T", "n_contrib", "ranges", "qcount")]
 
 
@@ -62,6 +62,7 @@
     "gs2m_debug_radix_temp_bytes": (i, [ll, i, C.POINTER(ull)]),
     "gs2m_debug_radix_plan": (i, [i, C.POINTER(i), C.POINTER(i), C.POINTER(i)]),
     "gs2m_debug_radix_sort": (i, [ll, i, p, p, p, p, p, p, p, ull, i, p, p, s]),
+    "gs2m_debug_radix_sort_rec3": (i, [ll, i, p, p, p, p, p, p, p, ull, i, p, p, s]),
     "gs2m_debug_block_scans": (i, [ll, p, p, p, p, ll, p, p, p, p, s]),
     "gs2m_debug_blend_forward": (i, [i, i, i, p, p, p, p, p, p, p, p, p, p, p, s]),
     "gs2m_debug_blend_backward": (i, [i, i, i, p, p, p, p, p, p, p, p, p, p, p, p, s]),
diff --git a/include/gs2m_raster.h b/include/gs2m_raster.h
--- a/include/gs2m_raster.h
+++ b/include/gs2m_raster.h
@@ -109,6 +109,9 @@
     uint64_t tile_keys;
     uint64_t qlist;
     uint64_t qrow;
+    uint64_t rec_id;
+    uint64_t rec_row;
+    uint64_t rec_depth;
     uint64_t image_bytes;
     uint64_t final_T;
     uint64_t n_contrib;
@@ -206,6 +209,9 @@
 int gs2m_debug_radix_sort(long long n, int total_bits, const unsigned* kin, const unsigned* vin, unsigned* kA, unsigned* vA,
                           unsigned* kB, unsigned* vB, void* temp, unsigned long long temp_bytes, int prezeroed,
                           unsigned* range_raw, const unsigned* ext_hist, void* stream);
+int gs2m_debug_radix_sort_rec3(long long n, int total_bits, const unsigned* kin, const unsigned* vin, unsigned* kA, unsigned* vA,
+                               unsigned* kB, unsigned* vB, void* temp, unsigned long long temp_bytes, int prezeroed,
+                               unsigned* range_raw, const unsigned* ext_hist, void* stream);
 int gs2m_debug_block_scans(long long n_blocks, const unsigned* block_tt, const unsigned* block_hu, unsigned* block_pref,
                            unsigned* block_hupref, long long n_waves, const unsigned* wave_rows, unsigned* wave_rowbase,
                            unsigned* counters, unsigned* landing_out, void* stream);
```

Result: no change. 857.5 views/s (median of 2 runs) (+0.2%).
